# CrystalSixone/VLN-MAGIC

Hardware: AMD Instinct MI355X
Metric: trajectory-steps/sec (whole node), MAGIC-S R2R pretrain (higher is better)
Workload: dtype bf16

## Files before the change

### include/magic_hip.h

```cpp
#ifndef MAGIC_HIP_H
#define MAGIC_HIP_H
#ifdef __cplusplus
extern "C" {
#endif

#define MAGIC_OK 0
#define MAGIC_ERR_ARG (-1)
#define MAGIC_ERR_LAUNCH (-2)
#define MAGIC_ERR_UNSUPPORTED (-3)

int magic_abi_version(void);
int magic_build_id(char* out, int len);
int magic_device_info(int* cu_count, int* clock_khz, char* arch, int arch_len);

int magic_gemm(int dtype, int layout, int batch, int nh, int M, int N, int K,
               const void* A, int lda, long long sAb, long long sAh,
               const void* B, int ldb, long long sBb, long long sBh,
               void* C, int ldc, long long sCb, long long sCh, int c_f32, int accumulate,
               const float* bias, int epilogue, const void* aux, int ldaux,
               const void* residual, int ldr, void* C2, int ldc2,
               float alpha, int splitk, float* bias_grad, void* stream);
int magic_gemm_set_big(int mode);
#define MAGIC_GEMM_FORM_PLAIN 0x1
#define MAGIC_GEMM_FORM_XCD 0x2
#define MAGIC_GEMM_FORM_KG 0x4
#define MAGIC_GEMM_FORM_WIDE 0x8
#define MAGIC_GEMM_FORM_WIDE_XCD 0x10
#define MAGIC_GEMM_FORM_GROUPED 0x20
#define MAGIC_GEMM_FORM_GROUPED_KG 0x40
#define MAGIC_GEMM_FORM_DW_ATOMIC 0x80
#define MAGIC_GEMM_FORM_DW_DET 0x100
#define MAGIC_GEMM_FORM_DW_CAT 0x200
#define MAGIC_GEMM_FORM_DW_CAT_WIDE 0x400
#define MAGIC_GEMM_FORM_LLN 0x800
#define MAGIC_GEMM_FORM_LLN_PAIR 0x1000
#define MAGIC_GEMM_PLACE_SPLIT8 0x10000
#define MAGIC_GEMM_PLACE_XCD_GROUPS 0x20000
#define MAGIC_GEMM_PLACE_XCD_ROWS 0x40000
#define MAGIC_GEMM_PLACE_PLAIN 0x80000
int magic_gemm_last_form(void);

typedef struct magic_dw_desc { const void* dY; const void* X; float* dW; float* db; int M, N, K, lda, ldb, ldc, splitk; } magic_dw_desc;
int magic_gemm_dw_ws_need(int dtype, int n, const magic_dw_desc* d, long long* floats, int* counters);
int magic_gemm_dw_grouped(int dtype, int n, const magic_dw_desc* d, float* ws, long long ws_floats, unsigned* counters, int n_counters, void* stream);
typedef struct magic_dwcat_prob { float* dW; float* db; int N, K, lda, ldb, ldc; } magic_dwcat_prob;
int magic_gemm_dw_cat(int dtype, int n_prob, const magic_dwcat_prob* probs, int n_seg, const void* const* dy_tab, const void* const* x_tab,
                      const int* m_tab, void* stream);

int magic_linear_ln(int dtype, int M, int H, int K, const void* x, int lda, const void* W, int ldb, const float* bias,
                    const void* residual, int ldr, const float* gamma, const float* beta, float eps,
                    void* out, float* rstd, const void* drop_seed, float drop_p, unsigned drop_site, void* stream);
int magic_linear_act_ln(int dtype, int M, int H, int K, const void* x, int lda, const void* W, int ldb, const float* bias, int act,
                        void* pre_out, const float* gamma, const float* beta, float eps, void* out, float* rstd, void* stream);

int magic_linear_lnbwd(int dtype, int M, int H, int K, const void* x, int lda, const void* W, int ldb,
                       const void* residual, int ldr, const void* y, const float* gamma, const float* beta, const float* rstd,
                       void* dx, void* dxm, float* dgamma, float* dbeta,
                       const void* drop_seed, float drop_p, unsigned drop_site, void* stream);

int magic_dropout(int dtype, long long rows, int cols, int ld, const void* in, void* out,
                  const void* drop_seed, float drop_p, unsigned site, void* stream);

int magic_ln_fwd(int dtype, int M, int H, const void* in0, const void* in1,
                 const void* tab0, const int* idx0, int mod0, int off0,
                 const void* tab1, const int* idx1, int mod1, int off1,
                 const void* tab2, const int* idx2, int mod2, int off2,
                 const float* gamma, const float* beta, float eps, void* out, float* rstd, int do_ln,
                 const void* drop_seed, float drop_p, unsigned site_in0, unsigned site_out, void* out_drop, void* stream);
int magic_ln_bwd(int dtype, int M, int H, const void* dy, const void* y, const float* gamma, const float* beta,
                 const float* rstd, void* dx, float* dgamma, float* dbeta,
                 const int* idx0, int mod0, int off0, float* d0, int small0,
                 const int* idx1, int mod1, int off1, float* d1, int small1,
                 const int* idx2, int mod2, int off2, float* d2, int small2,
                 int do_ln, const void* drop_seed, float drop_p, unsigned site_dy, unsigned site_dx, void* dxm, int hot0, int pg_partial,
                 void* stream);
int magic_ln_bwd_tail(int dtype, int M, int H, const float* dy32, const void* y, const float* gamma, const float* beta, const float* rstd,
                      const void* act_pre, int act, void* dx, float* dgamma, float* dbeta, void* stream);
int magic_ln_bwd_blocks(int M, int H, int has_tables);
int magic_colsum_add_v(int n, const float* const* parts, float* const* dsts, const int* nblks, const int* lens, const int* strides, void* stream);

int magic_smallk_ln_fwd(int dtype, int M, int H, int Kin, const float* x, const float* W, const float* b,
                        const float* gamma, const float* beta, float eps, void* out, float* rstd, void* stream);
typedef struct {
  int n_out, accumulate; const void* src1; const int* ptr1; const int* idx1; const float* w1;
  const void* src2; const int* ptr2; const int* idx2; const float* w2; void* out;
} magic_csr_prob;
int magic_csr_gather_multi(int dtype, int H, int n, const magic_csr_prob* d, void* stream);
typedef struct {
  int M, Kin; const float* x; const void* dy; const void* y; const float* gamma; const float* beta; const float* rstd;
  float* dW; float* db; float* dgamma; float* dbeta; float* part;
} magic_skb_prob;
int magic_smallk_ln_bwd_pair(int dtype, int H, const magic_skb_prob* d, void* stream);
typedef struct {
  int M, Kin; const float* x; const float* W; const float* b; const float* gamma; const float* beta; float eps; int pad_;
  void* A; float* rstd; void* out;
  const void* add0;
  const void* src1; const int* ptr1; const int* idx1; const float* w1;
  const void* src2; const int* ptr2; const int* idx2; const float* w2;
  const void* tab; const int* tab_idx;
} magic_node_in;
int magic_node_in_fwd(int dtype, int H, int n, const magic_node_in* d, void* stream);

typedef struct { const unsigned* seed; unsigned site; float p; } magic_drop_desc;
typedef struct magic_pano_in {
  int M, Kin; float eps; int pad_;
  const void* P0; const float* g1; const float* b1; void* A1; float* rstd1;
  const float* loc; const float* W; const float* b; const float* g2; const float* b2; void* A2; float* rstd2;
  const void* nav_tab; const int* nav_idx; const void* tok_tab;
  const float* g3; const float* b3; void* X0; float* rstd3; void* X0d; magic_drop_desc dout;
} magic_pano_in;
typedef struct magic_ln_in {
  int M, do_ln; const void* in0; const void* in1;
  const void* tab[3]; const int* idx[3]; int mod[3]; int off[3];
  const float* gamma; const float* beta; float eps; int pad_; void* out; float* rstd;
  const unsigned* drop_seed; float drop_p; unsigned site_in0, site_out, pad2_; void* out_drop;
} magic_ln_in;
int magic_embed_in_fwd(int dtype, int H, const magic_pano_in* pa, const magic_ln_in* tx, void* stream);

typedef struct magic_pano_in_bwd {
  int M, Kin, pad0_, pad1_;
  const void* dy; magic_drop_desc ddy;
  const void* X0; const float* rstd3; const float* g3; const float* b3; float* dg3; float* db3;
  const int* nav_idx; float* d_nav; float* d_tok;
  const void* A1; const float* rstd1; const float* g1; const float* b1; float* dg1; float* db1; void* dP0;
  const void* A2; const float* rstd2; const float* g2; const float* b2; float* dg2; float* db2;
  const float* loc; float* dW; float* dbl;
  float* part;
} magic_pano_in_bwd;
typedef struct magic_ln_bwd_in {
  int M, do_ln; const void* dy; const void* y; const float* gamma; const float* beta; const float* rstd; void* dx; float* dgamma; float* dbeta;
  const int* idx[3]; int mod[3]; int off[3]; float* d[3]; int small[3];
  const unsigned* drop_seed; float drop_p; unsigned site_dy, site_dx; int hot0; void* dxm;
  int partial;
} magic_ln_bwd_in;
int magic_embed_in_bwd_supported(int H, int Kin);
int magic_embed_in_bwd_blocks(int M, int H, int nb_text, int partial);
int magic_embed_in_bwd_text_blocks(int M, int H, int has_tables, int has_pgrad);
int magic_embed_in_bwd(int dtype, int H, const magic_pano_in_bwd* pa, const magic_ln_bwd_in* tx,
                       int n_cs, const float* const* cs_parts, float* const* cs_dsts, const int* cs_nblks, void* stream);
int magic_smallk_ln_bwd(int dtype, int M, int H, int Kin, const float* x, const void* dy, const void* y,
                        const float* gamma, const float* beta, const float* rstd,
                        float* dW, float* db, float* dgamma, float* dbeta, float* part, void* stream);
int magic_smallk_ln_bwd_blocks(int M, int H, int Mmax);

int magic_node_in_bwd_supported(int H, int V, int Mmax);
int magic_node_in_bwd(int dtype, int H, int Np, int V, const void* x, const float* probs, const float* wf, void* d_fused, void* d_pano,
                      float* dwf, float* dbf, const magic_csr_prob* gat, int n_skb, const magic_skb_prob* skb,
                      int t_M, const void* t_dy, const int* t_idx, float* t_dtab,
                      long long add_n, int add_count, const void* const* add_xs, void* add_y, void* stream);

int magic_softmax_fwd(int dtype, int B, int nh, int Nq, int Nk, int ldp, const float* S, void* P, float scale,
                      const unsigned char* kmask, const float* dist, const float* sprel_w, const float* sprel_b, void* stream);
int magic_softmax_bwd(int dtype, int B, int nh, int Nq, int Nk, int ldp, const void* P, const float* dP, void* dS, float scale,
                      const float* dist, float* dsprel_w, float* dsprel_b, void* stream);
int magic_head_mean_fwd(int dtype, int B, int nh, long long inner, const void* P, float* out, void* stream);
int magic_head_mean_bwd(int B, int nh, long long inner, const float* g, float* dP, int accumulate, void* stream);

int magic_attn_supported(int dtype, int Nq, int Nk, int backward);
int magic_attn_fwd(int dtype, int B, int nh, int Nq, int Nk, const void* q, int ldq, const void* k, const void* v, int ldkv,
                   void* P, int ldp, void* ctx, int H, float scale, const unsigned char* kmask, const float* dist,
                   const float* sprel_w, const float* sprel_b,
                   const void* drop_seed, float drop_p, unsigned drop_site, void* Pd, void* stream);
int magic_attn_bwd(int dtype, int B, int nh, int Nq, int Nk, const void* q, int ldq, const void* k, const void* v, int ldkv,
                   const void* P, int ldp, const void* dctx, int H, float scale, const float* dP_init,
                   void* dq, int lddq, void* dk, void* dv, int lddkv,
                   const float* dist, float* dsprel_w, float* dsprel_b,
                   const void* drop_seed, float drop_p, unsigned drop_site, void* stream);
int magic_attn_bwd_ks(int dtype, int B, int nh, int Nq, int Nk, const void* q, int ldq, const void* k, const void* v, int ldkv,
                      const void* P, int ldp, const void* o, const void* dctx, int H, float scale,
                      void* dq, int lddq, void* dk, void* dv, int lddkv, int accumulate_kv,
                      const void* drop_seed, float drop_p, unsigned drop_site, void* stream);

int magic_lndot_fwd(int dtype, int M, int H, const void* Y, const float* gamma, const float* beta, float eps,
                    const float* w2, const float* b2, float* logit, void* stream);
int magic_lndot_bwd_blocks(int M);
int magic_lndot_bwd(int dtype, int M, int H, const void* Y, const float* gamma, const float* beta, float eps,
                    const float* w2, const float* dlogit, void* dZ, float* dgamma, float* dbeta, float* dw2, float* db2,
                    float* part, void* stream);

int magic_ce_rows(int dtype, int M, int N, const void* logits, int ld, const int* labels, int ignore_index,
                  float coef, const float* row_w, float* loss_row, void* dlogits, int ldd, int accumulate,
                  float* w_out, float w_rate, void* stream);
int magic_softkl_rows(int dtype, int M, int N, const void* logits, int ld, const float* targets, int ldt, float coef,
                      const float* row_w , float* loss_row, void* dlogits, int ldd,
                      void* stream);

int magic_kd_rows(int M, int N, const float* s, const float* t, int ld, float temperature, const float* w, float norm,
                  float coef, const float* coef_dev, float* loss_row, float* ds, int accumulate, void* stream);
int magic_mse(int dtype, int g_f32, long long outer, long long inner, const void* s, long long s_stride, const void* t,
              long long t_stride, const float* w, long long rows_per_w, float norm, float coef, const float* coef_dev, float* loss, void* ds,
              long long g_stride, int accumulate, void* stream);
typedef struct {
  int g_f32; long long outer, inner; const void* s; long long s_stride; const void* t; long long t_stride;
  const float* w; long long rows_per_w; float norm, coef; const float* coef_dev; float* loss; void* ds; long long g_stride; int accumulate;
  const int* valid_dev; const float* norm_dev; long long valid_mod;
} magic_mse_desc;
int magic_mse_multi(int dtype, int n, const magic_mse_desc* d, void* stream);
int magic_kd_emb_supported(int dtype, int Hs, int Ht);
int magic_kd_emb(int dtype, int n, const magic_mse_desc* d, int Hs, int Ht, const int* M, const void* const* W, const float* const* b,
                 void* const* d_acc, void* stream);
int magic_cfp_loss(int dtype, int B, int H, const void* a0, const void* a1, const void* a2, const void* txt, float temperature, float coef,
                   float* rows, void* d0, void* d1, void* d2, void* dtxt, float* part, int* counter, void* stream);

int magic_csr_gather(int dtype, int n_out, int H, const void* src, const int* ptr, const int* idx, const float* w,
                     void* out, int accumulate, void* stream);
int magic_pano_fuse_fwd(int dtype, int N, int V, int H, const void* x, const int* lens, const float* wf, const float* bf,
                        void* fused, float* probs, const void* P, int nh, int inner, float* pmean, void* stream);
typedef struct {
  int B, K, Vp, use_gate;
  const float *g_raw, *l_raw, *fuse_raw; const unsigned char *gmask, *lmask; const int* fsrc; const unsigned char* bwmask;
  float *gl, *ll, *fl;
  const int *glab, *llab; int ignore_index; float coef;
  float *rows, *dgl, *dll, *dfl;
  const float* t_fused; float w_rate; int pad_; float* w_out;
  float T, kd_norm, kd_coef, pad2_; const float* kd_coef_dev; float* kd_rows;
} magic_sap_loss_params;
int magic_sap_fuse_loss(const void* params, int nbytes, void* stream);
int magic_pano_fuse_bwd_blocks(int N);
int magic_pano_fuse_bwd(int dtype, int N, int V, int H, const void* x, const float* probs, const float* wf, const void* dfused,
                        void* dx, float* dwf, float* dbf, void* stream);
int magic_sap_fuse_fwd(int B, int K, int Vp, const float* g_raw, const float* l_raw, const float* fuse_raw,
                       const unsigned char* gmask, const unsigned char* lmask, const int* fsrc, const unsigned char* bwmask,
                       int use_gate, float* gl, float* ll, float* fl, void* stream);
int magic_sap_fuse_bwd(int B, int K, int Vp, const float* g_raw, const float* l_raw, const float* fuse_raw,
                       const unsigned char* gmask, const unsigned char* lmask, const int* fsrc, const unsigned char* bwmask,
                       int use_gate, const float* dgl, const float* dll, const float* dfl,
                       float* dg_raw, float* dl_raw, float* dfuse_raw, void* stream);

int magic_step_rng(unsigned long long base_seed, unsigned* counter, float rw_temp, int* seed_out, float* rw_out, float* zero_me,
                   float* scale_state, float growth, float backoff, int interval, void* stream);
int magic_seed_scale(const float* scale_dev);
int magic_loss_assemble(const float* rows, int n_rows, const float* row_w, float row_scale, const float* kd_rows, int n_kd,
                        float* slots, const float* rw, float alpha, int has_kd, float* out, void* stream);

int magic_rowgate_fwd(int dtype, int M, int H, int mode, const void* x, const void* e, const float* wx, const float* we,
                      const float* b0, const float* b1, float* out_s, void* out, float* gsave, void* stream);
int magic_rowgate_bwd(int dtype, int M, int H, int mode, const void* x, const void* e, const float* wx, const float* we, const float* gsave,
                      const float* dy, const void* dout, void* dx, void* de, float* dwx, float* dwe, float* db0, float* db1, void* stream);

int magic_sumsq(long long n, const float* g, float* out, void* stream);
int magic_adamw(long long n, float* p, float* g, float* m, float* v, void* shadow, int shadow_dtype,
                float lr, float b1, float b2, float eps, float wd, float step_size,
                const float* sumsq, float max_norm, float gscale, const float* lr_ss, long long n_decay, int zero_grad,
                unsigned* overflow, float* scale_state, int* sched_step, int decay_first, void* stream);
int magic_sumsq_sched(long long n, const float* g, float* out, int* step, float lr0, int warmup, int total, float b1, float b2,
                      float* lr_ss, void* stream);
int magic_sched_step(int* step, float lr0, int warmup, int total, float b1, float b2, float* lr_ss, float* zero_me, void* stream);
int magic_cast(int dtype16, int to16, long long n, const void* x, void* y, void* stream);
int magic_add_n(int dtype, long long n, int count, const void* const* xs, void* y, void* stream);
int magic_add(int dtype, long long n, const void* x, void* y, void* stream);
int magic_dact(int dtype, int kind, long long n, const void* dy, const void* z, void* dz, void* stream);

int magic_view_gather(int dtype, int Np, int V, int D, const void* table, int n_viewpoints, const int* vp_row,
                      const int* order, void* out, void* stream);

int magic_set_f32_mfma(int mode);
int magic_get_f32_mfma(void);

typedef struct {
  const void* Wqkv; const float* bqkv; const void* Wo; const float* bo; const float* g1; const float* be1;
  const void* W1; const float* bi; const void* W2; const float* bo2; const float* g2; const float* be2;
  void *qkv, *P, *Pd, *ctx, *a, *z, *g, *out; float *rstd_a, *rstd_o;
  unsigned site_attn, site_ao, site_out, pad_;
} magic_enc_layer;
typedef struct { const void* x; const unsigned char* kmask; int nsamp, N, ldp, nlayers; magic_enc_layer L[6]; } magic_enc_seg;
typedef struct { magic_enc_seg seg[2]; int nseg; float p_attn, p_hidden, eps, scale; const unsigned* seed;
                 unsigned* sync; int sync_words, pad2_; } magic_enc_params;
int magic_encoder_supported(int dtype, int H, int I, int nh, int N, int nlayers);
int magic_encoder_params_bytes(void);
int magic_encoder_fwd(int dtype, const void* params, int nbytes, void* stream);
int magic_encoder_start_gate(int timeout_us, int recent_us, unsigned* stats, void* stream);
int magic_stream_probe(unsigned* word2, int timeout_us, void* stream_wait, void* stream_set);
int magic_encoder_health(unsigned* out, void* stream);

typedef struct {
  const void* Wqkv; const float* bqkv; const void* Wo; const float* bo; const float* g1; const float* be1;
  const void* Wq; const float* bq; const void* Wkv; const float* bkv; const void* Woc; const float* boc; const float* gc; const float* bec;
  const void* W1; const float* bi; const void* W2; const float* bo2; const float* g2; const float* be2;
  void *qkv, *P, *Pd, *ctx, *a; float* rstd_a;
  void *q, *kv, *Pc, *Pdc, *cctx, *c; float* rstd_c;
  void *z, *g, *out; float* rstd_o;
  unsigned site_attn, site_ao, site_cattn, site_co, site_out, pad_;
} magic_xenc_layer;
typedef struct {
  const void* x; const void* cx; const unsigned char* qmask; const unsigned char* cmask;
  const float* dist; const float* sprel_w; const float* sprel_b;
  int nsamp, Nq, Nk, ldps, ldpc, nlayers;
  magic_xenc_layer L[3];
} magic_xenc_seg;
typedef struct { magic_xenc_seg seg[2]; int nseg; float p_attn, p_hidden, eps, scale; const unsigned* seed;
                 unsigned* sync; int sync_words, pad2_; } magic_xenc_params;
int magic_xencoder_supported(int dtype, int H, int I, int nh, int Nq, int Nk, int nlayers);
int magic_xencoder_params_bytes(void);
int magic_xencoder_fwd(int dtype, const void* params, int nbytes, void* stream);

typedef struct {
  int M, ld_in, Np, pad_;
  const void* inp; const void* res;
  const void* Wa; const float* ba; const float* g1; const float* b1; void* y1;
  const void* W1; const float* bi; const void* W2; const float* bo2; const float* g2; const float* b2; void* y2;
  const void* Wp; const float* bp; void* proj;
  float eps; int pad2_;
} magic_chain_params;
int magic_chain_supported(int dtype, int H, int I);
int magic_pack_frag_spans(const void* src, void* dst, int n, const long long* offs, const int* rows, const int* cols, void* stream);
int magic_layout_spans(const void* src, void* dst_f, void* dst_tf, int n, const long long* offs, const int* rows, const int* cols,
                       const int* flags, void* stream);
int magic_chain_fwd(int dtype, const void* params, int nbytes, void* stream);
int magic_chain_tile_rows(int rows);

typedef struct {
  int M, kt;
  const void* dqkv_n; const void* WqkvT_n; const void* dao_n; const void* dfo_in; const void* dfod_in;
  const void* y2; const float* rstd2; const float* g2; const float* b2; float* dg2; float* db2;
  const void* z; const void* W2T; const void* W1T;
  const void* y1; const float* rstd1; const float* g1; const float* b1; float* dg1; float* db1;
  const void* WoT;
  void *dfo, *dfod, *dz, *daod, *dao, *dctx;
  unsigned site_out, site_ao;
  int mode, N, ntile, ldp;
  const void* qkv_a; const void* P_a; const void* o_a; const void* dctx_a; const float* dP_init; void* dqkv_out;
  unsigned site_attn, pad_;
  const float* dist; float* dsprel_w; float* dsprel_b;
} magic_rowbwd_seg;
typedef struct { magic_rowbwd_seg seg[2]; int nseg, blocks0; float p_hidden; int pad1; const unsigned* seed; float p_attn, scale; } magic_rowbwd_params;
int magic_rowbwd_supported(int dtype, int H, int I);
int magic_rowbwd_attn_supported(int dtype, int H, int I, int nh, int N);
int magic_rowbwd_params_bytes(void);
int magic_rowbwd(int dtype, const void* params, int nbytes, void* stream);
int magic_rowbwd_rows(long long total_rows);
int magic_colsum_add(int H, int n, const float* const* parts, float* const* dsts, const int* nblks, void* stream);
int magic_transpose_spans(const void* src, void* dst, int n, const long long* offs, const int* rows, const int* cols, void* stream);

int magic_group_begin(void);
int magic_group_end(void* stream);

#ifdef __cplusplus
}
#endif
#endif
```

### vln-magic_amd/csrc/build_id.py

```python
#!/usr/bin/env python3
import hashlib
import os
import sys

HERE = os.path.dirname(os.path.abspath(__file__))
HEADERS = ("common.hpp", "group.hpp", "enc_common.hpp", os.path.join("..", "..", "include", "magic_hip.h"))
EXTRA = ("gen_fastcall.py", "build_id.py", os.path.join("..", "host", "abi.py"), os.path.join("..", "host", "lib.py"), "hostplan.c")


def _sha(*chunks):
    h = hashlib.sha256()
    for c in chunks:
        h.update(c if isinstance(c, bytes) else c.encode())
        h.update(b"\0")
    return h.hexdigest()


def _read(name):
    with open(os.path.join(HERE, name), "rb") as f:
        return f.read()


def units():
    return sorted(f for f in os.listdir(HERE) if f.endswith(".hip"))


def flags():
    for line in _read("Makefile").decode().splitlines():
        if line.startswith("FLAGS"):
            return line.strip()
    return ""


def unit_hashes():
    hdr = [_read(h) for h in HEADERS]
    fl = flags()
    return {u: _sha(_read(u), *hdr, fl) for u in units()}


def build_id(uh=None):
    uh = uh or unit_hashes()
    return _sha(*[f"{u}:{h}" for u, h in sorted(uh.items())], *[_read(e) for e in EXTRA])[:16]


def _write_if_changed(path, text):
    try:
        with open(path) as f:
            if f.read() == text:
                return False
    except OSError:
        pass
    with open(path, "w") as f:
        f.write(text)
    return True


def write_stamp(target):
    uh = unit_hashes()
    if target == "buildid.c":
        _write_if_changed(os.path.join(HERE, "buildid.c"),
                          "/* generated by build_id.py: the id of the source set this library was built from */\n"
                          "#include <string.h>\n"
                          f'int magic_build_id(char* out, int len) {{\n  static const char id[] = "{build_id(uh)}";\n'
                          "  if (!out || len < (int)sizeof(id)) return -1;\n  memcpy(out, id, sizeof(id));\n  return 0;\n}\n")
    else:
        _write_if_changed(os.path.join(HERE, target), uh[target[:-6] + ".hip"] + "\n")


if __name__ == "__main__":
    if "--stamp" in sys.argv:
        write_stamp(sys.argv[sys.argv.index("--stamp") + 1])
    else:
        print(build_id())
```

### vln-magic_amd/csrc/graphops.hip

```cpp
#include "common.hpp"
#include <cstring>

template <typename T>
__global__ __launch_bounds__(256) void csr_gather_kernel(int n_out, int H, const T* src, const int* ptr, const int* idx, const float* w,
                                                         T* out, int accumulate) {
  const int lane = threadIdx.x & 63, n = blockIdx.x * 4 + (threadIdx.x >> 6);
  if (n >= n_out) return;
  const int e0 = ptr[n], e1 = ptr[n + 1];
  if (accumulate && e0 == e1) return;
  for (int c = lane * 2; c < H; c += 128) {
    float a = 0.f, b = 0.f;
    for (int e = e0; e < e1; ++e) {
      const float wv = w ? w[e] : 1.f;
      const T* p = src + (long long)idx[e] * H + c;
      a += wv * to_f(p[0]); b += wv * to_f(p[1]);
    }
    T* o = out + (long long)n * H + c;
    if (accumulate) { a += to_f(o[0]); b += to_f(o[1]); }
    o[0] = from_f<T>(a); o[1] = from_f<T>(b);
  }
}

#define CSRM_MAX 4
struct CsrMulti { magic_csr_prob p[CSRM_MAX]; int start[CSRM_MAX + 1]; int n, H; };
template <typename T>
__global__ __launch_bounds__(256) void csr_gather_multi_kernel(CsrMulti mm) {
  int i = 0;
  while (i + 1 < mm.n && (int)blockIdx.x >= mm.start[i + 1]) ++i;
  const magic_csr_prob& p = mm.p[i];
  const int H = mm.H, lane = threadIdx.x & 63, n = (blockIdx.x - mm.start[i]) * 4 + (threadIdx.x >> 6);
  if (n >= p.n_out) return;
  const int a0 = p.ptr1[n], a1 = p.ptr1[n + 1];
  const int b0 = p.ptr2 ? p.ptr2[n] : 0, b1 = p.ptr2 ? p.ptr2[n + 1] : 0;
  if (p.accumulate && a0 == a1 && b0 == b1) return;
  const T* s1 = (const T*)p.src1; const T* s2 = (const T*)p.src2; T* out = (T*)p.out;
  for (int c = lane * 2; c < H; c += 128) {
    T* o = out + (long long)n * H + c;
    float va = 0.f, vb = 0.f;
    if (p.accumulate) { va = to_f(o[0]); vb = to_f(o[1]); }
    if (!p.accumulate || a0 < a1) {
      float a = 0.f, b = 0.f;
      for (int e = a0; e < a1; ++e) {
        const float wv = p.w1 ? p.w1[e] : 1.f;
        const T* q = s1 + (long long)p.idx1[e] * H + c;
        a += wv * to_f(q[0]); b += wv * to_f(q[1]);
      }
      va = to_f(from_f<T>(a + va)); vb = to_f(from_f<T>(b + vb));
    }
    if (b0 < b1) {
      float a = 0.f, b = 0.f;
      for (int e = b0; e < b1; ++e) {
        const float wv = p.w2 ? p.w2[e] : 1.f;
        const T* q = s2 + (long long)p.idx2[e] * H + c;
        a += wv * to_f(q[0]); b += wv * to_f(q[1]);
      }
      va = to_f(from_f<T>(a + va)); vb = to_f(from_f<T>(b + vb));
    }
    o[0] = from_f<T>(va); o[1] = from_f<T>(vb);
  }
}

template <typename T>
__global__ __launch_bounds__(256) void pano_fuse_fwd_kernel(int N, int V, int H, const T* x, const int* lens, const float* wf, const float* bf,
                                                            T* fused, float* probs, const T* P, int nh, int inner, float* pmean) {
  __shared__ float sc[64];
  const int n = blockIdx.x, tid = threadIdx.x, lane = tid & 63, wid = tid >> 6;
  if (P) {
    const T* pb = P + (long long)n * nh * inner;
    for (int r = tid; r < inner; r += 256) {
      float s = 0.f;
      for (int h = 0; h < nh; ++h) s += to_f(pb[(long long)h * inner + r]);
      pmean[(long long)n * inner + r] = s / nh;
    }
  }
  const T* xb = x + (long long)n * V * H;
  for (int v = wid; v < V; v += 4) {
    float d = 0.f;
    for (int c = lane; c < H; c += 64) d += to_f(xb[(long long)v * H + c]) * wf[c];
    d = wave_sum(d);
    if (lane == 0) sc[v] = d + bf[0] + (v < lens[n] ? 0.f : -10000.0f);
  }
  __syncthreads();
  if (wid == 0) {
    float s = lane < V ? sc[lane] : -3.0e38f;
    const float mx = wave_max(s);
    float e = lane < V ? __expf(s - mx) : 0.f;
    const float z = wave_sum(e);
    if (lane < V) { sc[lane] = e / z; probs[(long long)n * V + lane] = e / z; }
  }
  __syncthreads();
  for (int c = tid; c < H; c += 256) {
    float a = 0.f;
    for (int v = 0; v < V; ++v) a += sc[v] * to_f(xb[(long long)v * H + c]);
    fused[(long long)n * H + c] = from_f<T>(a);
  }
}


#define PFF_VPW 10
template <typename T, int NIT>
__global__ __launch_bounds__(256) void pano_fuse_fwd_reg_kernel(int N, int V, const T* x, const int* lens, const float* wf, const float* bf,
                                                                T* fused, float* probs, const T* P, int nh, int inner, float* pmean) {
  constexpr int H = NIT * 128;
  __shared__ float sc[64];
  __shared__ float part[4][H];
  const int n = blockIdx.x, tid = threadIdx.x, lane = tid & 63, wid = tid >> 6;
  const T* xb = x + (long long)n * V * H;
  float xv[PFF_VPW][2 * NIT], wr[2 * NIT];
#pragma unroll
  for (int it = 0; it < NIT; ++it) { wr[2 * it] = wf[it * 128 + lane * 2]; wr[2 * it + 1] = wf[it * 128 + lane * 2 + 1]; }
#pragma unroll
  for (int j = 0; j < PFF_VPW; ++j) {
    const int v = wid + 4 * j;
#pragma unroll
    for (int it = 0; it < NIT; ++it) {
      xv[j][2 * it] = 0.f; xv[j][2 * it + 1] = 0.f;
      if (v < V) {
        if constexpr (sizeof(T) == 2) {
          const unsigned u = *(const unsigned*)(xb + (long long)v * H + it * 128 + lane * 2);
          T lo, hi;
          __builtin_memcpy(&lo, &u, 2); __builtin_memcpy(&hi, (const char*)&u + 2, 2);
          xv[j][2 * it] = to_f(lo); xv[j][2 * it + 1] = to_f(hi);
        } else {
          const float2 u = *(const float2*)(xb + (long long)v * H + it * 128 + lane * 2);
          xv[j][2 * it] = u.x; xv[j][2 * it + 1] = u.y;
        }
      }
    }
  }
  if (P) {
    const T* pb = P + (long long)n * nh * inner;
    for (int r = tid; r < inner; r += 256) {
      float s = 0.f;
      for (int h = 0; h < nh; ++h) s += to_f(pb[(long long)h * inner + r]);
      pmean[(long long)n * inner + r] = s / nh;
    }
  }
  const int len = lens[n];
  const float b0 = bf[0];
#pragma unroll
  for (int j = 0; j < PFF_VPW; ++j) {
    const int v = wid + 4 * j;
    float d = 0.f;
#pragma unroll
    for (int i = 0; i < 2 * NIT; ++i) d += xv[j][i] * wr[i];
    d = wave_sum(d);
    if (lane == 0 && v < V) sc[v] = d + b0 + (v < len ? 0.f : -10000.0f);
  }
  __syncthreads();
  if (wid == 0) {
    float s = lane < V ? sc[lane] : -3.0e38f;
    const float mx = wave_max(s);
    float e = lane < V ? __expf(s - mx) : 0.f;
    const float z = wave_sum(e);
    if (lane < V) { sc[lane] = e / z; probs[(long long)n * V + lane] = e / z; }
  }
  __syncthreads();
  float a[2 * NIT];
#pragma unroll
  for (int i = 0; i < 2 * NIT; ++i) a[i] = 0.f;
#pragma unroll
  for (int j = 0; j < PFF_VPW; ++j) {
    const int v = wid + 4 * j;
    const float pv = v < V ? sc[v] : 0.f;
#pragma unroll
    for (int i = 0; i < 2 * NIT; ++i) a[i] += pv * xv[j][i];
  }
#pragma unroll
  for (int it = 0; it < NIT; ++it) { part[wid][it * 128 + lane * 2] = a[2 * it]; part[wid][it * 128 + lane * 2 + 1] = a[2 * it + 1]; }
  __syncthreads();
  for (int c = tid; c < H; c += 256) fused[(long long)n * H + c] = from_f<T>((part[0][c] + part[1][c]) + (part[2][c] + part[3][c]));
}

#define PF_PB 2
template <typename T>
__global__ __launch_bounds__(256 * PF_PB) void pano_fuse_bwd_kernel(int N, int V, int H, const T* __restrict__ x, const float* __restrict__ probs,
                                                                    const float* __restrict__ wf, const T* __restrict__ dfused, T* __restrict__ dx,
                                                                    float* dwf, float* dbf) {
  __shared__ float dp[PF_PB][64], dsv[PF_PB][64], red[PF_PB * 4][768], rb[PF_PB];
  const int tid = threadIdx.x, lane = tid & 63, wave = tid >> 6, pb = wave >> 2, wid = wave & 3;
  const int n = blockIdx.x * PF_PB + pb;
  const bool live = n < N;
  const int nn = live ? n : N - 1;
  const T* xb = x + (long long)nn * V * H;
  const T* df = dfused + (long long)nn * H;
  const float* p = probs + (long long)nn * V;
  const int nit = H / 128;
  float dfr[12], wfr[12];
  for (int it = 0; it < nit; ++it) {
    const int c = it * 128 + lane * 2;
    dfr[2 * it] = to_f(df[c]); dfr[2 * it + 1] = to_f(df[c + 1]);
    wfr[2 * it] = wf[c]; wfr[2 * it + 1] = wf[c + 1];
  }
  for (int v = wid; v < V; v += 4) {
    float d = 0.f;
    for (int it = 0; it < nit; ++it) {
      const int c = it * 128 + lane * 2;
      d += to_f(xb[(long long)v * H + c]) * dfr[2 * it] + to_f(xb[(long long)v * H + c + 1]) * dfr[2 * it + 1];
    }
    d = wave_sum(d);
    if (lane == 0) dp[pb][v] = d;
  }
  __syncthreads();
  if (wid == 0) {
    float t = lane < V ? p[lane] * dp[pb][lane] : 0.f;
    const float s = wave_sum(t);
    const float d = (lane < V && live) ? p[lane] * (dp[pb][lane] - s) : 0.f;
    if (lane < V) dsv[pb][lane] = d;
    const float tot = wave_sum(d);
    if (lane == 0) rb[pb] = tot;
  }
  __syncthreads();
  float aw[12];
  for (int i = 0; i < 2 * nit; ++i) aw[i] = 0.f;
  if (live) {
    for (int v = wid; v < V; v += 4) {
      const float pv = p[v], dv = dsv[pb][v];
      for (int it = 0; it < nit; ++it) {
        const int c = it * 128 + lane * 2;
        const long long i = ((long long)n * V + v) * H + c;
        const float x0 = to_f(xb[(long long)v * H + c]), x1 = to_f(xb[(long long)v * H + c + 1]);
        aw[2 * it] += dv * x0; aw[2 * it + 1] += dv * x1;
        dx[i] = from_f<T>(to_f(dx[i]) + pv * dfr[2 * it] + dv * wfr[2 * it]);
        dx[i + 1] = from_f<T>(to_f(dx[i + 1]) + pv * dfr[2 * it + 1] + dv * wfr[2 * it + 1]);
      }
    }
  }
  for (int it = 0; it < nit; ++it) {
    const int c = it * 128 + lane * 2;
    red[wave][c] = aw[2 * it]; red[wave][c + 1] = aw[2 * it + 1];
  }
  __syncthreads();
  float* const prow = dbf ? nullptr : dwf + (long long)blockIdx.x * (H + 1);
  for (int c = tid; c < H; c += 256 * PF_PB) {
    float v = 0.f;
    for (int w = 0; w < PF_PB * 4; ++w) v += red[w][c];
    if (prow) prow[c] = v; else atomicAdd(dwf + c, v);
  }
  if (tid == 0) {
    float v = 0.f;
    for (int q = 0; q < PF_PB; ++q) v += rb[q];
    if (prow) prow[H] = v; else atomicAdd(dbf, v);
  }
}

__global__ __launch_bounds__(64) void sap_fuse_fwd_kernel(int B, int K, int Vp, const float* g_raw, const float* l_raw, const float* fuse_raw,
                                                          const unsigned char* gmask, const unsigned char* lmask, const int* fsrc,
                                                          const unsigned char* bwmask, float use_gate, float* gl, float* ll, float* fl) {
  __shared__ float sl[128];
  __shared__ float sbw;
  const int b = blockIdx.x, tid = threadIdx.x;
  const float NEG = -__builtin_inff();
  const float fw = use_gate != 0.f ? 1.f / (1.f + __expf(-fuse_raw[b])) : 0.5f;
  float bw = 0.f;
  for (int j = tid; j < Vp; j += 64) {
    const float v = lmask[b * Vp + j] ? l_raw[b * Vp + j] * (1.f - fw) : NEG;
    ll[b * Vp + j] = v; sl[j] = v;
    if (bwmask[b * Vp + j] && lmask[b * Vp + j]) bw += v;
  }
  bw = wave_sum(bw);
  if (tid == 0) sbw = bw;
  __syncthreads();
  for (int k = tid; k < K; k += 64) {
    const float v = gmask[b * K + k] ? g_raw[b * K + k] * fw : NEG;
    gl[b * K + k] = v;
    const int s = fsrc[b * K + k];
    float add = 0.f;
    if (s >= 0) add = sl[s]; else if (s == -2) add = sbw;
    fl[b * K + k] = v + add;
  }
}

using SapLossParams = magic_sap_loss_params;
__device__ __forceinline__ float sap_ce_wave(const float* x, int N, int lab, int ignore_index, float coef, float* d, int lane) {
  const bool ignored = (lab == ignore_index) || lab < 0 || lab >= N;
  const float xl = ignored ? 0.f : x[lab];
  float mx = -3.0e38f;
  for (int c = lane; c < N; c += 64) mx = fmaxf(mx, x[c]);
  mx = wave_max(mx);
  float s = 0.f;
  for (int c = lane; c < N; c += 64) s += __expf(x[c] - mx);
  s = wave_sum(s);
  const float lse = mx + __logf(s);
  if (d) {
    const float cf = ignored ? 0.f : coef;
    for (int c = lane; c < N; c += 64) d[c] = cf * (__expf(x[c] - lse) - (c == lab ? 1.f : 0.f));
  }
  return ignored ? 0.f : lse - xl;
}
__global__ __launch_bounds__(64) void sap_fuse_loss_kernel(SapLossParams p, const float* ss) {
  __shared__ float sl[128];
  if (ss) { p.coef *= ss[0]; p.kd_coef *= ss[0]; }
  __shared__ float sbw;
  const int b = blockIdx.x, lane = threadIdx.x, B = p.B, K = p.K, Vp = p.Vp;
  const float NEG = -__builtin_inff();
  const float fw = p.use_gate ? 1.f / (1.f + __expf(-p.fuse_raw[b])) : 0.5f;
  float* gl = p.gl + (long long)b * K; float* ll = p.ll + (long long)b * Vp; float* fl = p.fl + (long long)b * K;
  float bw = 0.f;
  for (int j = lane; j < Vp; j += 64) {
    const float v = p.lmask[b * Vp + j] ? p.l_raw[b * Vp + j] * (1.f - fw) : NEG;
    ll[j] = v; sl[j] = v;
    if (p.bwmask[b * Vp + j] && p.lmask[b * Vp + j]) bw += v;
  }
  bw = wave_sum(bw);
  if (lane == 0) sbw = bw;
  __syncthreads();
  for (int k = lane; k < K; k += 64) {
    const float v = p.gmask[b * K + k] ? p.g_raw[b * K + k] * fw : NEG;
    gl[k] = v;
    const int s = p.fsrc[b * K + k];
    float add = 0.f;
    if (s >= 0) add = sl[s]; else if (s == -2) add = sbw;
    fl[k] = v + add;
  }
  __syncthreads();
  const int gla = p.glab[b], lla = p.llab[b];
  const float l0 = sap_ce_wave(gl, K, gla, p.ignore_index, p.coef, p.dgl ? p.dgl + (long long)b * K : nullptr, lane);
  const float l1 = sap_ce_wave(ll, Vp, lla, p.ignore_index, p.coef, p.dll ? p.dll + (long long)b * Vp : nullptr, lane);
  float* dfl = p.dfl ? p.dfl + (long long)b * K : nullptr;
  const float l2 = sap_ce_wave(fl, K, gla, p.ignore_index, p.coef, dfl, lane);
  if (lane == 0) { p.rows[b] = l0; p.rows[B + b] = l1; p.rows[2 * B + b] = l2; }
  if (!p.t_fused) return;
  const float* t = p.t_fused + (long long)b * K;
  float wr = 1.f;
  if (p.w_out) {
    wr = __expf(-p.w_rate * sap_ce_wave(t, K, gla, p.ignore_index, 0.f, nullptr, lane));
    if (lane == 0) p.w_out[b] = wr;
  }
  if (!p.kd_rows) return;
  __syncthreads();
  float coef = p.kd_coef;
  if (p.kd_coef_dev) coef *= p.kd_coef_dev[0];
  const float invT = 1.0f / p.T;
  float sv[8], tv[8], ms = -3.0e38f, mt = -3.0e38f;
#pragma unroll
  for (int it = 0; it < 8; ++it) {
    const int c = it * 64 + lane;
    float a = -3.0e38f, q = -3.0e38f;
    if (c < K) {
      a = fl[c]; q = t[c];
      if (a == NEG) a = -1e6f;
      if (q == NEG) q = -1e6f;
      a *= invT; q *= invT;
      ms = fmaxf(ms, a); mt = fmaxf(mt, q);
    }
    sv[it] = a; tv[it] = q;
  }
  ms = wave_max(ms); mt = wave_max(mt);
  float zs = 0.f, zt = 0.f;
#pragma unroll
  for (int it = 0; it < 8; ++it) {
    const int c = it * 64 + lane;
    if (c < K) { zs += __expf(sv[it] - ms); zt += __expf(tv[it] - mt); }
  }
  zs = wave_sum(zs); zt = wave_sum(zt);
  const float ls = ms + __logf(zs), lt = mt + __logf(zt);
  float kl = 0.f;
#pragma unroll
  for (int it = 0; it < 8; ++it) {
    const int c = it * 64 + lane;
    if (c < K) {
      const float lpt = tv[it] - lt, lps = sv[it] - ls;
      const float pt = __expf(lpt), ps = __expf(lps);
      if (pt > 0.f) kl += pt * (lpt - lps);
      if (dfl) dfl[c] += coef * wr * p.T * (ps - pt) * p.kd_norm;
    }
  }
  kl = wave_sum(kl);
  if (lane == 0) p.kd_rows[b] = wr * kl * p.T * p.T * p.kd_norm;
}

__global__ __launch_bounds__(64) void sap_fuse_bwd_kernel(int B, int K, int Vp, const float* g_raw, const float* l_raw, const float* fuse_raw,
                                                          const unsigned char* gmask, const unsigned char* lmask, const int* fsrc,
                                                          const unsigned char* bwmask, float use_gate, const float* dgl, const float* dll,
                                                          const float* dfl, float* dg_raw, float* dl_raw, float* dfuse_raw) {
  __shared__ float dl[128];
  __shared__ float sbw;
  const int b = blockIdx.x, tid = threadIdx.x;
  const float fw = use_gate != 0.f ? 1.f / (1.f + __expf(-fuse_raw[b])) : 0.5f;
  for (int j = tid; j < Vp; j += 64) dl[j] = (dll && lmask[b * Vp + j]) ? dll[b * Vp + j] : 0.f;
  if (tid == 0) sbw = 0.f;
  __syncthreads();
  float dfw = 0.f;
  for (int k = tid; k < K; k += 64) {
    const bool ok = gmask[b * K + k];
    const float dg = ok ? ((dgl ? dgl[b * K + k] : 0.f) + (dfl ? dfl[b * K + k] : 0.f)) : 0.f;
    dg_raw[b * K + k] = dg * fw;
    dfw += dg * g_raw[b * K + k];
    if (dfl && ok) {
      const int s = fsrc[b * K + k];
      const float d = dfl[b * K + k];
      if (s >= 0) atomicAdd(&dl[s], d); else if (s == -2) atomicAdd(&sbw, d);
    }
  }
  __syncthreads();
  for (int j = tid; j < Vp; j += 64) {
    float d = dl[j];
    if (bwmask[b * Vp + j]) d += sbw;
    if (!lmask[b * Vp + j]) d = 0.f;
    dl_raw[b * Vp + j] = d * (1.f - fw);
    dfw -= d * l_raw[b * Vp + j];
  }
  dfw = wave_sum(dfw);
  if (tid == 0) dfuse_raw[b] = use_gate != 0.f ? dfw * fw * (1.f - fw) : 0.f;
}

extern "C" int magic_csr_gather(int dtype, int n_out, int H, const void* src, const int* ptr, const int* idx, const float* w,
                                void* out, int accumulate, void* stream) {
  if (n_out <= 0 || H <= 0 || (H & 1)) return MAGIC_ERR_ARG;
  dim3 grid((n_out + 3) / 4), block(256);
  hipStream_t st = (hipStream_t)stream;
  if (dtype == DT_BF16) hipLaunchKernelGGL(csr_gather_kernel<bf16>, grid, block, 0, st, n_out, H, (const bf16*)src, ptr, idx, w, (bf16*)out, accumulate);
  else if (dtype == DT_F16) hipLaunchKernelGGL(csr_gather_kernel<f16>, grid, block, 0, st, n_out, H, (const f16*)src, ptr, idx, w, (f16*)out, accumulate);
  else hipLaunchKernelGGL(csr_gather_kernel<float>, grid, block, 0, st, n_out, H, (const float*)src, ptr, idx, w, (float*)out, accumulate);
  return launch_status();
}

extern "C" int magic_csr_gather_multi(int dtype, int H, int n, const magic_csr_prob* d, void* stream) {
  if (n < 1 || n > CSRM_MAX || !d || H <= 0 || (H & 1)) return MAGIC_ERR_ARG;
  CsrMulti mm;
  mm.n = n; mm.H = H;
  int total = 0;
  for (int i = 0; i < n; ++i) {
    if (d[i].n_out <= 0 || !d[i].src1 || !d[i].ptr1 || !d[i].idx1 || !d[i].out) return MAGIC_ERR_ARG;
    if (d[i].ptr2 && (!d[i].src2 || !d[i].idx2)) return MAGIC_ERR_ARG;
    mm.p[i] = d[i];
    mm.start[i] = total;
    total += (d[i].n_out + 3) / 4;
  }
  for (int i = n; i <= CSRM_MAX; ++i) mm.start[i] = total;
  dim3 grid(total), block(256);
  hipStream_t st = (hipStream_t)stream;
  if (dtype == DT_BF16) hipLaunchKernelGGL(csr_gather_multi_kernel<bf16>, grid, block, 0, st, mm);
  else if (dtype == DT_F16) hipLaunchKernelGGL(csr_gather_multi_kernel<f16>, grid, block, 0, st, mm);
  else hipLaunchKernelGGL(csr_gather_multi_kernel<float>, grid, block, 0, st, mm);
  return launch_status();
}

extern "C" int magic_pano_fuse_fwd(int dtype, int N, int V, int H, const void* x, const int* lens, const float* wf, const float* bf,
                                   void* fused, float* probs, const void* P, int nh, int inner, float* pmean, void* stream) {
  if (N <= 0 || V <= 0 || V > 64 || H <= 0 || (P && (nh <= 0 || inner <= 0 || !pmean))) return MAGIC_ERR_ARG;
  dim3 grid(N), block(256);
  hipStream_t st = (hipStream_t)stream;
  static int reg_form = -1;
  if (reg_form < 0) { const char* e = getenv("MAGIC_PANO_FUSE_REG"); reg_form = e ? atoi(e) : 1; }
  if (reg_form && V <= 4 * PFF_VPW && (H == 128 || H == 256 || H == 384 || H == 768)) {
#define PFR(TY, NIT) hipLaunchKernelGGL((pano_fuse_fwd_reg_kernel<TY, NIT>), grid, block, 0, st, N, V, (const TY*)x, lens, wf, bf, (TY*)fused, probs, (const TY*)P, nh, inner, pmean)
#define PFR_T(TY) do { if (H == 128) PFR(TY, 1); else if (H == 256) PFR(TY, 2); else if (H == 384) PFR(TY, 3); else PFR(TY, 6); } while (0)
    if (dtype == DT_BF16) PFR_T(bf16); else if (dtype == DT_F16) PFR_T(f16); else PFR_T(float);
#undef PFR_T
#undef PFR
    return launch_status();
  }
  if (dtype == DT_BF16) hipLaunchKernelGGL(pano_fuse_fwd_kernel<bf16>, grid, block, 0, st, N, V, H, (const bf16*)x, lens, wf, bf, (bf16*)fused, probs, (const bf16*)P, nh, inner, pmean);
  else if (dtype == DT_F16) hipLaunchKernelGGL(pano_fuse_fwd_kernel<f16>, grid, block, 0, st, N, V, H, (const f16*)x, lens, wf, bf, (f16*)fused, probs, (const f16*)P, nh, inner, pmean);
  else hipLaunchKernelGGL(pano_fuse_fwd_kernel<float>, grid, block, 0, st, N, V, H, (const float*)x, lens, wf, bf, (float*)fused, probs, (const float*)P, nh, inner, pmean);
  return launch_status();
}

extern "C" int magic_pano_fuse_bwd_blocks(int N) { return N > 0 ? (N + PF_PB - 1) / PF_PB : MAGIC_ERR_ARG; }
extern "C" int magic_pano_fuse_bwd(int dtype, int N, int V, int H, const void* x, const float* probs, const float* wf, const void* dfused,
                                   void* dx, float* dwf, float* dbf, void* stream) {
  if (N <= 0 || V <= 0 || V > 64 || H <= 0 || H % 128 || H > 768) return MAGIC_ERR_ARG;
  dim3 grid((N + PF_PB - 1) / PF_PB), block(256 * PF_PB);
  hipStream_t st = (hipStream_t)stream;
  if (dtype == DT_BF16) hipLaunchKernelGGL(pano_fuse_bwd_kernel<bf16>, grid, block, 0, st, N, V, H, (const bf16*)x, probs, wf, (const bf16*)dfused, (bf16*)dx, dwf, dbf);
  else if (dtype == DT_F16) hipLaunchKernelGGL(pano_fuse_bwd_kernel<f16>, grid, block, 0, st, N, V, H, (const f16*)x, probs, wf, (const f16*)dfused, (f16*)dx, dwf, dbf);
  else hipLaunchKernelGGL(pano_fuse_bwd_kernel<float>, grid, block, 0, st, N, V, H, (const float*)x, probs, wf, (const float*)dfused, (float*)dx, dwf, dbf);
  return launch_status();
}

extern "C" int magic_sap_fuse_fwd(int B, int K, int Vp, const float* g_raw, const float* l_raw, const float* fuse_raw,
                                  const unsigned char* gmask, const unsigned char* lmask, const int* fsrc, const unsigned char* bwmask,
                                  int use_gate, float* gl, float* ll, float* fl, void* stream) {
  if (B <= 0 || K <= 0 || Vp <= 0 || Vp > 128) return MAGIC_ERR_ARG;
  hipLaunchKernelGGL(sap_fuse_fwd_kernel, dim3(B), dim3(64), 0, (hipStream_t)stream, B, K, Vp, g_raw, l_raw, fuse_raw, gmask, lmask, fsrc, bwmask,
                     (float)use_gate, gl, ll, fl);
  return launch_status();
}

extern "C" int magic_sap_fuse_loss(const void* params, int nbytes, void* stream) {
  if (!params || nbytes != (int)sizeof(SapLossParams)) return MAGIC_ERR_ARG;
  SapLossParams p;
  memcpy(&p, params, sizeof(p));
  if (p.B <= 0 || p.K <= 0 || p.K > 512 || p.Vp <= 0 || p.Vp > 128 || !p.g_raw || !p.l_raw || !p.fuse_raw || !p.gmask || !p.lmask || !p.fsrc || !p.bwmask ||
      !p.gl || !p.ll || !p.fl || !p.glab || !p.llab || !p.rows) return MAGIC_ERR_ARG;
  if ((p.w_out || p.kd_rows) && !p.t_fused) return MAGIC_ERR_ARG;
  if (p.kd_rows && !(p.T > 0.f)) return MAGIC_ERR_ARG;
  hipLaunchKernelGGL(sap_fuse_loss_kernel, dim3(p.B), dim3(64), 0, (hipStream_t)stream, p, seed_scale_get());
  return launch_status();
}

extern "C" int magic_sap_fuse_bwd(int B, int K, int Vp, const float* g_raw, const float* l_raw, const float* fuse_raw,
                                  const unsigned char* gmask, const unsigned char* lmask, const int* fsrc, const unsigned char* bwmask,
                                  int use_gate, const float* dgl, const float* dll, const float* dfl,
                                  float* dg_raw, float* dl_raw, float* dfuse_raw, void* stream) {
  if (B <= 0 || K <= 0 || Vp <= 0 || Vp > 128) return MAGIC_ERR_ARG;
  hipLaunchKernelGGL(sap_fuse_bwd_kernel, dim3(B), dim3(64), 0, (hipStream_t)stream, B, K, Vp, g_raw, l_raw, fuse_raw, gmask, lmask, fsrc, bwmask,
                     (float)use_gate, dgl, dll, dfl, dg_raw, dl_raw, dfuse_raw);
  return launch_status();
}

template <typename T>
__global__ __launch_bounds__(256) void view_gather_kernel(long long rows, int V, int D, const T* table, int n_vp, const int* vp_row, const int* order, T* out) {
  constexpr int VE = 16 / sizeof(T), UN = 4;
  typedef __attribute__((ext_vector_type(4))) unsigned int u4;
  const int nvec = D / VE;
  const long long total = rows * nvec, stride = (long long)gridDim.x * 256;
  u4* dst = (u4*)out;
  for (long long v0 = (long long)blockIdx.x * 256 + threadIdx.x; v0 < total; v0 += stride * UN) {
    u4 val[UN];
#pragma unroll
    for (int u = 0; u < UN; ++u) {
      const long long v = v0 + u * stride;
      val[u] = (u4){0u, 0u, 0u, 0u};
      if (v < total) {
        const long long r = v / nvec;
        const int c = (int)(v - r * nvec), sv = order[r];
        const int vr = vp_row[r / V];
        if (sv >= 0 && sv < 36 && (unsigned)vr < (unsigned)n_vp)
          val[u] = __builtin_nontemporal_load((const u4*)(table + ((long long)vr * 36 + sv) * D) + c);
      }
    }
#pragma unroll
    for (int u = 0; u < UN; ++u) {
      const long long v = v0 + u * stride;
      if (v < total) dst[v] = val[u];
    }
  }
}

extern "C" int magic_view_gather(int dtype, int Np, int V, int D, const void* table, int n_viewpoints, const int* vp_row,
                                 const int* order, void* out, void* stream) {
  if (Np <= 0 || V <= 0 || D <= 0 || n_viewpoints <= 0 || !table || !vp_row || !order || !out) return MAGIC_ERR_ARG;
  if (!dtype_ok(dtype)) return MAGIC_ERR_ARG;
  const int ve = dtype_is16(dtype) ? 8 : 4;
  if (D % ve || ((uintptr_t)table & 15) || ((uintptr_t)out & 15)) return MAGIC_ERR_ARG;
  const long long rows = (long long)Np * V;
  const long long chunks = (rows * (D / ve) + 256 * 4 - 1) / (256 * 4);
  dim3 grid((unsigned)(chunks < 1 ? 1 : chunks)), block(256);
  hipStream_t st = (hipStream_t)stream;
  if (dtype == DT_BF16) hipLaunchKernelGGL(view_gather_kernel<bf16>, grid, block, 0, st, rows, V, D, (const bf16*)table, n_viewpoints, vp_row, order, (bf16*)out);
  else if (dtype == DT_F16) hipLaunchKernelGGL(view_gather_kernel<f16>, grid, block, 0, st, rows, V, D, (const f16*)table, n_viewpoints, vp_row, order, (f16*)out);
  else hipLaunchKernelGGL(view_gather_kernel<float>, grid, block, 0, st, rows, V, D, (const float*)table, n_viewpoints, vp_row, order, (float*)out);
  return launch_status();
}
```

### vln-magic_amd/host/model_pretrain.py

```python
import os

import torch
import torch.nn as nn

from . import ops as O
from .config import cfg_get
from .ddp import refuse_torch_ddp
from .engine import Ctx, MagicNet, cls_specs, rup, trunk_specs
from .params import ParamStore
from .plan import build_plan, check_plan

MID_CUT = 2
LOCKSTEP = not os.environ.get("MAGIC_NO_LOCKSTEP")
LOCKSTEP_EAGER = bool(os.environ.get("MAGIC_LOCKSTEP_EAGER"))
DYN_TERMS = ("txt_emb", "txt_attn", "img_emb", "img_fused", "img_attn", "g_emb", "g_attn", "l_emb", "l_attn")
KD_SLOTS = ("txt_emb_loss", "txt_attn_loss", "img_emb_loss", "avg_img_emb_loss", "img_attn_loss",
            "global_emb_loss", "global_attn_loss", "local_emb_loss", "local_attn_loss", "predict_loss")


PRETRAIN_CAUSAL = ("back_txt", "back_img")


def pretrain_specs(cfg):
    H = cfg.hidden_size
    s = trunk_specs(cfg, "bert.")
    s += [("mlm_head.predictions.transform.dense.weight", (H, H), "normal"), ("mlm_head.predictions.transform.dense.bias", (H,), "zeros"),
          ("mlm_head.predictions.transform.LayerNorm.weight", (H,), "ones"), ("mlm_head.predictions.transform.LayerNorm.bias", (H,), "zeros"),
          ("mlm_head.predictions.bias", (cfg.vocab_size,), "zeros")]
    s += cls_specs("global_sap_head.", H) + cls_specs("local_sap_head.", H) + cls_specs("sap_fuse_linear.", H, 2 * H)
    for k in ("gmap", "vp", "fused", "txt"):
        s += [(f"cfp_heads.{k}.weight", (H, H), "normal"), (f"cfp_heads.{k}.bias", (H,), "zeros")]
    if "mrc" in (getattr(cfg, "pretrain_tasks", None) or ()):
        P = int(cfg_get(cfg, "image_prob_size"))
        s += [("image_classifier.net.0.weight", (H, H), "normal"), ("image_classifier.net.0.bias", (H,), "zeros"),
              ("image_classifier.net.2.weight", (H,), "ones"), ("image_classifier.net.2.bias", (H,), "zeros"),
              ("image_classifier.net.3.weight", (P, H), "normal"), ("image_classifier.net.3.bias", (P,), "zeros")]
    from .causal import causal_specs
    return s + causal_specs(cfg, "bert.", only=PRETRAIN_CAUSAL)


def _dropout_knobs(model, config):
    model.dropout = nn.Dropout(float(cfg_get(config, "hidden_dropout_prob")))
    model.attention_dropout = nn.Dropout(float(cfg_get(config, "attention_probs_dropout_prob")))


class _BackwardHook(torch.autograd.Function):

    @staticmethod
    def forward(ctx, loss_value, anchor, model):
        ctx.model = model
        return loss_value.clone()

    @staticmethod
    def backward(ctx, grad_out):
        ctx.model.backward()
        m = ctx.model
        if m.loss_scale is not None:
            m.store.grad.mul_(grad_out.to(torch.float32) * m.loss_scale[1])
        elif m.grad_scale != 1.0:
            m.store.grad.mul_(grad_out.to(torch.float32) / m.grad_scale)
        from .trainer import auto_sync
        auto_sync(ctx.model)
        return None, None, None


MLM_TAIL_FUSED = os.environ.get("MAGIC_MLM_TAIL_FUSED", "1") != "0"
MLM_DX_SPLITK = int(os.environ.get("MAGIC_MLM_DX_SPLITK", "32"))
MLM_DX_ATOMICS = os.environ.get("MAGIC_MLM_DX_ATOMICS", "0") != "0"


class GlocalTextPathCMTPreTraining(nn.Module):
    def __init__(self, config, device="cuda", compute_dtype=torch.bfloat16, seed=0):
        super().__init__()
        self.config = config
        self.device_ = torch.device(device)
        self.compute_dtype = compute_dtype
        trainable = getattr(config, "role", "student") != "teacher" or bool(getattr(config, "train_teacher", False))
        self.store = ParamStore(pretrain_specs(config), device, compute_dtype,
                                init_std=cfg_get(config, "initializer_range"), seed=seed, requires_grad=trainable)
        self.store.attach_to(self)
        self.net = MagicNet(config, self.store, "bert.")
        self.prefix, self.explicit_backward = "bert.", True
        if self.device_.type == "cuda":
            O.dw_counters(self.device_)
        from .causal import build_blocks
        self.causal_blocks = build_blocks(self, only=PRETRAIN_CAUSAL)
        _dropout_knobs(self, config)
        self._anchor = torch.zeros(1, device=self.device_, requires_grad=True)
        self._ctx = None
        self._kd_idx = torch.tensor([0, 0, 1, 1, 1, 2, 2, 3, 3, 4], device=self.device_)
        self.keep_mlm_logits = False
        self.dropout_seed = None
        self.grad_scale = 4096.0 if compute_dtype == torch.float16 else 1.0
        self.loss_scale = None
        self.register_load_state_dict_post_hook(lambda m, k: setattr(m.store, "shadow_clean", False))

    def enable_dynamic_loss_scale(self, init=None):
        if self.loss_scale is None:
            S = float(init if init is not None else self.grad_scale)
            self.loss_scale = torch.tensor([S, 1.0 / S, 0.0, 0.0], dtype=torch.float32, device=self.device_)
        return self.loss_scale

    @classmethod
    def from_pretrained(cls, pretrained_model_name_or_path=None, config=None, state_dict=None, **kw):
        model = cls(config, **kw)
        if state_dict is not None:
            own = model.state_dict()
            keep = {k: v for k, v in state_dict.items() if k in own and tuple(v.shape) == tuple(own[k].shape)}
            model.load_state_dict(keep, strict=False)
        return model

    def _par(self, fn_main, fn_aux):
        if LOCKSTEP and self.device_.type == "cuda" and (torch.cuda.is_current_stream_capturing() or LOCKSTEP_EAGER):
            from . import lib as L
            return L.lockstep(fn_main, fn_aux)
        return fn_main(), fn_aux()

    def _arm_dropout(self):
        ph, pa = float(self.dropout.p), float(self.attention_dropout.p)
        if self.training and self.store.requires_grad and torch.is_grad_enabled() and (ph > 0 or pa > 0):
            seed = getattr(self, "dropout_seed", None)
            if seed is None:
                seed = torch.randint(0, 2 ** 31 - 1, (2,), dtype=torch.int32, device=self.device_)
            self.net.set_dropout(seed, ph, pa)
        else:
            self.net.set_dropout(None)

    def mark_params_dirty(self):
        self.store.shadow_clean = False

    def _dev(self, t, dtype=None):
        t = t.to(self.device_, non_blocking=True)
        return t if dtype is None or t.dtype == dtype else t.to(dtype)

    def _inputs(self, batch, plan):
        Np, V = plan["Np"], plan["V"]
        if batch.get("view_table") is not None:
            x = batch["view_table"].gather(batch["traj_vp_row"], batch["traj_view_order"]).reshape(Np * V, -1)
        else:
            x = self._dev(batch["traj_view_img_fts"]).reshape(Np * V, -1)
        if x.dtype != self.compute_dtype:
            x = O.cast_to(x.contiguous(), self.compute_dtype)
        return Ctx(feats=x,
                   loc=self._dev(batch["traj_loc_fts"], torch.float32).reshape(Np * V, -1).contiguous(),
                   gpos=self._dev(batch["gmap_pos_fts"], torch.float32).reshape(plan["B"] * plan["K"], -1).contiguous(),
                   vpos=self._dev(batch["vp_pos_fts"], torch.float32).reshape(plan["B"] * plan["Vp"], -1).contiguous(),
                   dist=self._dev(batch["gmap_pair_dists"], torch.float32).contiguous())

    def _cls(self, prefix, X, M, lda=None):
        n, H = self.net, self.net.H
        l1 = n.lin(prefix + "net.0.weight")
        Y = O.linear_fwd(X, l1.W, l1.b, M, epilogue=2, lda=lda)
        ln = n.ln(prefix + "net.2")
        l2 = n.lin(prefix + "net.3.weight")
        logit = n.new(M, dtype=torch.float32)
        O.lndot_fwd(Y, M, H, ln.g, ln.b, n.eps, l2.Wm, l2.b, logit)
        return Y, logit

    def _cls_tail(self, prefix, Y, M):
        n = self.net
        ln, l2 = n.ln(prefix + "net.2"), n.lin(prefix + "net.3.weight")
        logit = n.new(M, dtype=torch.float32)
        O.lndot_fwd(Y, M, n.H, ln.g, ln.b, n.eps, l2.Wm, l2.b, logit)
        return logit

    def _cls_bwd(self, prefix, X, Y, dlogit, M, d_acc, lda=None):
        n, H = self.net, self.net.H
        l1, ln, l2 = n.lin(prefix + "net.0.weight"), n.ln(prefix + "net.2"), n.lin(prefix + "net.3.weight")
        dZ = n.new(M, H)
        O.lndot_bwd(Y, M, H, ln.g, ln.b, n.eps, l2.Wm, dlogit, dZ, ln.dg, ln.db, l2.dW, l2.db)
        O.linear_dw(dZ, X, l1.dW, l1.db, M, ldb=lda)
        O.linear_dx(dZ, l1.W, M, out=d_acc, residual=d_acc, ldc=lda)

    def _causal_fwd(self, c, batch, compute_loss):
        cz, plan, H = self.causal_blocks, c.plan, self.net.H
        need = {"instr_z_direction_features": "back_txt", "instr_z_landmark_features": "back_txt", "img_z_features": "back_img"}
        for k, blk in need.items():
            if batch.get(k) is not None and blk not in cz:
                from .causal import BLOCKS
                raise ValueError(f"batch carries {k!r} but config.{BLOCKS[blk]} is off -- the model has no '{blk}' block "
                                 "(pretrain_src/config/r2r_magic_model_config.json:60-66)")
        track = bool(compute_loss and self.store.requires_grad and torch.is_grad_enabled())
        c.islands = []

        def island(block, x2d, shape, z, pz):
            x0 = x2d.detach().view(shape)
            with torch.enable_grad() if track else torch.no_grad():
                if track:
                    x0.requires_grad_(True)
                y = block(x0, z, pz)
            if track:
                c.islands.append((x0, y))
            return y.detach().reshape(x2d.shape).contiguous()
        dv = lambda t: t.to(self.device_)
        if "back_txt" in cz and (batch.get("instr_z_direction_features") is not None or batch.get("instr_z_landmark_features") is not None):
            parts = [k for k in ("direction", "landmark") if batch.get(f"instr_z_{k}_features") is not None]
            z = torch.cat([dv(batch[f"instr_z_{k}_features"]) for k in parts], 1)
            pz = torch.cat([dv(batch[f"instr_z_{k}_pzs"]) for k in parts], 1)
            c.txt_out = island(cz["back_txt"], c.txt.out, (plan["B"], plan["L"], H), z, pz)
            c.island_txt = len(c.islands) - 1 if track else None
        if "back_img" in cz and batch.get("img_z_features") is not None:
            out = island(cz["back_img"], c.pano.out, (plan["Np"], plan["V"], H), dv(batch["img_z_features"]), dv(batch["img_z_pzs"]))
            c.pano_adj = Ctx(**vars(c.pano))
            c.pano_adj.out = out
            c.island_pano = len(c.islands) - 1 if track else None

    def _causal_bwd(self, c):
        for name, attr in (("island_txt", "d_txt"), ("island_pano", "d_pano")):
            i = getattr(c, name, None)
            if i is None:
                continue
            x0, y = c.islands[i]
            d = getattr(c, attr)
            torch.autograd.backward(y, d.view(y.shape).to(y.dtype))
            setattr(c, attr, x0.grad.reshape(d.shape).to(d.dtype).clone())
            x0.grad = None

    def will_fuse_encoders(self, plan):
        n = self.net
        return bool(n.enc_ok(plan["L"], self.config.num_l_layers) and n.enc_ok(plan["V"], self.config.num_pano_layers))

    def forward(self, batch, task, compute_loss=True, teacher_outputs=None, rw=None, plan=None, return_outputs=False, inputs=None, heads=True):
        if not heads and (compute_loss or not return_outputs):
            raise ValueError("heads=False returns the encoders' outputs only: compute_loss=False, return_outputs=True")
        n = self.net
        refuse_torch_ddp(self)
        self.store.sync_shadow()
        O.DEFER["queue"].clear(); O.DEFER["bytes"] = 0
        O.RBW_JOBS.clear()
        if self.store.requires_grad:
            O.defer_dw(False)
        self._arm_dropout()
        plan = plan if plan is not None else build_plan(batch, task, self.device_)
        check_plan(plan, self.config)
        inp = inputs if inputs is not None else self._inputs(batch, plan)
        B, L, K, Vp, H = plan["B"], plan["L"], plan["K"], plan["Vp"], n.H
        c = Ctx(task=task, plan=plan, inp=inp)
        fuse = self.will_fuse_encoders(plan)
        if n.embed_in_ok():
            ct, cp = n.embeds_fwd(plan, inp.feats, inp.loc)
            c.txt, c.pano = self._par(lambda: n.text_fwd(plan, defer=fuse, c=ct), lambda: n.pano_fwd(plan, inp.feats, inp.loc, defer=fuse, c=cp))
        else:
            c.txt, c.pano = self._par(lambda: n.text_fwd(plan, defer=fuse), lambda: n.pano_fwd(plan, inp.feats, inp.loc, defer=fuse))
        if fuse:
            n.encoders_fwd(c.txt, c.pano)
        c.txt_out, c.pano_adj = c.txt.out, c.pano
        if self.causal_blocks or any(batch.get(k) is not None for k in ("instr_z_direction_features", "instr_z_landmark_features", "img_z_features")):
            self._causal_fwd(c, batch, compute_loss)
        c.gin, c.vin = n.nodes_in_fwd(plan, c.pano_adj, inp.gpos if task != "mrc" else None, inp.vpos if task != "mlm" else None)
        tl, gl_, vl = plan["lens"]["txt"], plan["lens"]["gmap"], [Vp] * B
        o = dict(txt_embeds=c.txt_out, txt_attns=c.txt.P, pano_embeds=c.pano_adj.out, pano_fused_embeds=c.pano.fused,
                 img_attns=c.pano.img_attn, plan=plan, inputs=inp)
        if task == "mlm":
            l2v_args = ("global", plan, c.txt_out, L, plan["txt_mask"], tl, plan["txt_tokens"], c.gin.out, K, plan["gmap_mask"], gl_, plan["gmap_nodes"])
            c.l2v = n.cross_fwd_fused([l2v_args])[0] if n.xenc_ok(L, K) else n.cross_fwd(*l2v_args, dist=None)
            o["gmap_embeds"], o["gmap_attns"] = c.l2v.out, c.l2v.P
            if heads:
                nm = plan["n_mask"]
                c.hm_in = n.new(nm, H)
                O.csr_gather(c.l2v.out, *plan["mlm_rows"], c.hm_in, nm, H)
                t = n.lin("mlm_head.predictions.transform.dense.weight")
                c.tz = n.new(nm, H)
                tn = n.ln("mlm_head.predictions.transform.LayerNorm")
                c.hm, c.rstd_hm = n.new(nm, H), n.new(nm, dtype=torch.float32)
                if MLM_TAIL_FUSED and O.linear_ln_ok(H, H):
                    O.linear_act_ln(c.hm_in, t.W, t.b, nm, 1, c.tz, tn.g, tn.b, n.eps, c.hm, c.rstd_hm)
                else:
                    c.tg = O.linear_fwd(c.hm_in, t.W, t.b, nm, epilogue=1, pre=c.tz)
                    O.ln_fwd(nm, H, c.hm, in0=c.tg, gamma=tn.g, beta=tn.b, eps=n.eps, rstd=c.rstd_hm)
                Vv = self.config.vocab_size
                c.ldv = rup(Vv, 8)
                c.logits = n.new(nm, c.ldv)
                if c.ldv > Vv:
                    c.logits[:, Vv:].zero_()
                O.linear_fwd(c.hm, self.store.w("bert.embeddings.word_embeddings.weight"), self.store.master("mlm_head.predictions.bias"),
                             nm, out=c.logits, ldc=c.ldv)
                o["predict"] = c.logits[:, :Vv]
        elif task == "mrc":
            loc_args = ("local", plan, c.vin.out, Vp, plan["vp_mask"], vl, B * Vp, c.txt_out, L, plan["txt_mask"], tl, plan["txt_tokens"])
            c.loc = n.cross_fwd_fused([loc_args])[0] if n.xenc_ok(Vp, L) else n.cross_fwd(*loc_args)
            o.update(vp_embeds=c.loc.out, vp_attns=c.loc.P)
            if heads:
                nm = plan["n_mrc"]
                c.mx = n.new(nm, H)
                O.csr_gather(c.loc.out, *plan["mrc_rows"], c.mx, nm, H)
                l1, l2 = n.lin("image_classifier.net.0.weight"), n.lin("image_classifier.net.3.weight")
                ln = n.ln("image_classifier.net.2")
                c.mZ, c.m_rstd = n.new(nm, H), n.new(nm, dtype=torch.float32)
                if MLM_TAIL_FUSED and O.linear_ln_ok(H, H):
                    c.mY = n.new(nm, H)
                    O.linear_act_ln(c.mx, l1.W, l1.b, nm, 2, c.mY, ln.g, ln.b, n.eps, c.mZ, c.m_rstd)
                else:
                    c.mY = O.linear_fwd(c.mx, l1.W, l1.b, nm, epilogue=2)
                    O.ln_fwd(nm, H, c.mZ, in0=c.mY, gamma=ln.g, beta=ln.b, eps=n.eps, rstd=c.m_rstd)
                c.mlogits = O.linear_fwd(c.mZ, l2.W, l2.b, nm)
                o["predict"] = c.mlogits
        else:
            def _local():
                vin = c.vin
                return vin, n.cross_fwd("local", plan, vin.out, Vp, plan["vp_mask"], vl, B * Vp,
                                        c.txt_out, L, plan["txt_mask"], tl, plan["txt_tokens"])
            if n.xenc_ok(K, L) and n.xenc_ok(Vp, L):
                c.glob, c.loc = n.cross_fwd_fused([
                    ("global", plan, c.gin.out, K, plan["gmap_mask"], gl_, plan["gmap_nodes"], c.txt_out, L, plan["txt_mask"], tl, plan["txt_tokens"], inp.dist),
                    ("local", plan, c.vin.out, Vp, plan["vp_mask"], vl, B * Vp, c.txt_out, L, plan["txt_mask"], tl, plan["txt_tokens"])])
            else:
              c.glob, (c.vin, c.loc) = self._par(
                lambda: n.cross_fwd("global", plan, c.gin.out, K, plan["gmap_mask"], gl_, plan["gmap_nodes"],
                                    c.txt_out, L, plan["txt_mask"], tl, plan["txt_tokens"], dist=inp.dist), _local)
            o.update(gmap_embeds=c.glob.out, gmap_attns=c.glob.P, vp_embeds=c.loc.out, vp_attns=c.loc.P)
            if not heads:
                pass
            elif task == "sap":
                from . import lib as _lib
                use_gate = bool(cfg_get(self.config, "glocal_fuse"))
                g1, l1_ = n.lin("global_sap_head.net.0.weight"), n.lin("local_sap_head.net.0.weight")
                with _lib.group():
                    c.Yg = O.linear_fwd(c.glob.out, g1.W, g1.b, B * K, epilogue=2)
                    c.Yl = O.linear_fwd(c.loc.out, l1_.W, l1_.b, B * Vp, epilogue=2)
                    if use_gate:
                        f1 = n.lin("sap_fuse_linear.net.0.weight")
                        tmp = O.linear_fwd(c.glob.out, f1.W, None, B, lda=K * H, ldb=2 * H, K=H)
                c.g_raw = self._cls_tail("global_sap_head.", c.Yg, B * K)
                c.l_raw = self._cls_tail("local_sap_head.", c.Yl, B * Vp)
                if use_gate:
                    c.Yf = O.linear_fwd(c.loc.out, f1.W[:, H:], f1.b, B, lda=Vp * H, ldb=2 * H, K=H, residual=tmp, epilogue=0)
                    self._relu(c.Yf)
                    fln, f2 = n.ln("sap_fuse_linear.net.2"), n.lin("sap_fuse_linear.net.3.weight")
                    c.fuse_raw = n.new(B, dtype=torch.float32)
                    O.lndot_fwd(c.Yf, B, H, fln.g, fln.b, n.eps, f2.Wm, f2.b, c.fuse_raw)
                else:
                    c.fuse_raw = n.zeros(B, dtype=torch.float32)
                c.use_gate = use_gate
                c.gl, c.ll, c.fl = n.new(B, K, dtype=torch.float32), n.new(B, Vp, dtype=torch.float32), n.new(B, K, dtype=torch.float32)
                c.sap_fused = bool(compute_loss and O.SAP_LOSS_FUSED and K <= 512 and Vp <= 128)
                if not c.sap_fused:
                    O.sap_fuse_fwd(B, K, Vp, c.g_raw, c.l_raw, c.fuse_raw, plan["gmask"], plan["lmask"], plan["fsrc"], plan["bwmask"],
                                   use_gate, c.gl, c.ll, c.fl)
                o.update(global_logits=c.gl, local_logits=c.ll, fused_logits=c.fl)
            elif task == "cfp":
                c.g0, c.v0, c.t0, c.gv0 = n.new(B, H), n.new(B, H), n.new(B, H), n.new(B, H)
                O.csr_gather_multi(H, [dict(out=c.g0, n_out=B, src1=c.glob.out, csr1=plan["g0"]),
                                       dict(out=c.v0, n_out=B, src1=c.loc.out, csr1=plan["v0"]),
                                       dict(out=c.t0, n_out=B, src1=c.txt_out, csr1=plan["t0"]),
                                       dict(out=c.gv0, n_out=B, src1=c.glob.out, csr1=plan["g0"], src2=c.loc.out, csr2=plan["v0"])])
                from . import lib as _lib
                with _lib.group():
                    c.cfp = []
                    for key, src in (("gmap", c.g0), ("vp", c.v0), ("fused", c.gv0), ("txt", c.t0)):
                        hl = n.lin(f"cfp_heads.{key}.weight")
                        c.cfp.append(O.linear_fwd(src, hl.W, hl.b, B))
                o["cfp"] = tuple(c.cfp)
            else:
                raise ValueError(task)
        if not compute_loss:
            if return_outputs:
                return o
            if task == "mlm":
                return {"predict": o["predict"]}
            if task == "mrc":
                return c.mlogits, plan["mrc_targets"], None, None
            if task == "sap":
                return dict(global_logits=c.gl, local_logits=c.ll, fused_logits=c.fl,
                            global_act_labels=self._dev(batch["global_act_labels"]), local_act_labels=self._dev(batch["local_act_labels"]))
            return o["cfp"]
        self._ctx = c
        if callable(teacher_outputs):
            teacher_outputs = teacher_outputs()
        scaled = self.loss_scale is not None and self.store.requires_grad
        if scaled:
            O.seed_scale(self.loss_scale)
        try:
            out = self._losses(c, o, teacher_outputs, rw)
        finally:
            if scaled:
                O.seed_scale(None)
        out["outputs"] = o
        if self.store.requires_grad and torch.is_grad_enabled():
            out["loss"] = _BackwardHook.apply(out["loss"], self._anchor, self)
        return out

    def _relu(self, x):
        return O.dact(x, x, 2, out=x)

    def _dyn(self, c, term, fn, mod=0):
        d = c.plan.get("dyn")
        if d is None:
            return {}
        i = DYN_TERMS.index(term)
        d["fill"][term] = fn
        return dict(valid_dev=d["i"][2 * i:2 * i + 2], norm_dev=d["f"][i:i + 1], norm=1.0, valid_mod=mod)

    def _kd_emb(self, c, slot, s_t, t_t, proj, M, outer, w, coef, d_acc, dyn=None):
        c.kd_emb.append((slot, s_t, t_t, self.net.lin(f"bert.{proj}.weight"), M, outer, w, coef, d_acc, dyn))

    def _kd_attn(self, c, slot, sP, tP, Bn, Nq, Nk, ldp, nh_s, nh_t, w, coef, dyn=None):
        n = self.net
        hmin = min(nh_s, nh_t)
        dP = None
        if self.store.requires_grad:
            dP = (n.new if hmin == nh_s else n.zeros)(Bn, nh_s, Nq, ldp, dtype=torch.float32)
        q = dict(s=sP, t=tP, outer=Bn, inner=hmin * Nq * ldp, s_stride=nh_s * Nq * ldp, t_stride=nh_t * Nq * ldp, w=w, rows_per_w=1,
                 norm=1.0 / (Bn * hmin * Nq * Nk), coef=coef[0], coef_dev=coef[1], loss=c.slots[slot:slot + 1], ds=dP,
                 g_stride=nh_s * Nq * ldp)
        if dyn is not None:
            term, qk, kk = dyn
            q.update(self._dyn(c, term, lambda t, Bn=Bn, hmin=hmin, Nq=Nq, Nk=Nk, ldp=ldp, qk=qk, kk=kk:
                               (Bn, (t[qk] if qk else Nq) * ldp, 1.0 / (Bn * hmin * (t[qk] if qk else Nq) * (t[kk] if kk else Nk))), mod=Nq * ldp))
        c.kd_mse.append(q)
        return dP

    def _kd_flush(self, c):
        from . import lib as L
        n, train = self.net, self.store.requires_grad
        jobs = c.kd_emb
        fused = bool(jobs) and all(
            O.kd_emb_ok(s_t.dtype, pl.K, pl.N) and t_t.dtype == s_t.dtype and s_t.is_contiguous() and t_t.is_contiguous() and pl.W.is_contiguous()
            and not ((s_t.data_ptr() | t_t.data_ptr() | pl.W.data_ptr() | (d_acc.data_ptr() if train else 0)) & 15)
            and (not train or d_acc.is_contiguous()) for (_, s_t, t_t, pl, _, _, _, _, d_acc, _) in jobs)
        sps = [None] * len(jobs)
        if not fused:
            with L.group():
                sps = [O.linear_fwd(s_t, pl.W, pl.b, M) for (_, s_t, _, pl, M, _, _, _, _, _) in jobs]
        dss, emb = [], []
        for (slot, s_t, t_t, pl, M, outer, w, coef, d_acc, dyn), sp in zip(jobs, sps):
            Ht = pl.N
            inner = (M // outer) * Ht
            ds = n.new(M, Ht) if train else None
            dss.append(ds)
            q = dict(s=sp, t=t_t, outer=outer, inner=inner, s_stride=inner, t_stride=inner, w=w, rows_per_w=1, norm=1.0 / (M * Ht),
                     coef=coef[0], coef_dev=coef[1], loss=c.slots[slot:slot + 1], ds=ds, g_stride=inner)
            if dyn is not None:
                term, ok, ik = dyn
                rows = M // outer
                q.update(self._dyn(c, term, lambda t, outer=outer, rows=rows, Ht=Ht, ok=ok, ik=ik:
                                   ((t[ok] if ok else outer), (t[ik] if ik else rows) * Ht,
                                    1.0 / ((t[ok] if ok else outer) * (t[ik] if ik else rows) * Ht))))
            if fused:
                q.pop("valid_mod", None)
                q.update(s=s_t, M=M, W=pl.W, b=pl.b, d_acc=d_acc if train else None)
                emb.append(q)
            else:
                c.kd_mse.append(q)
        if emb:
            O.kd_emb(emb)
        if c.kd_mse:
            O.mse_multi(c.kd_mse)
        if train:
            for (slot, s_t, t_t, pl, M, outer, w, coef, d_acc, dyn), ds in zip(jobs, dss):
                O.linear_dw(ds, s_t, pl.dW, pl.db, M)
            if not fused:
                with L.group():
                    for (slot, s_t, t_t, pl, M, outer, w, coef, d_acc, dyn), ds in zip(jobs, dss):
                        O.linear_dx(ds, pl.W, M, out=d_acc, residual=d_acc)
        c.kd_emb, c.kd_mse = [], []

    def _rw_device(self, rw):
        if rw is None:
            rw = [1.0] * 5
        if torch.is_tensor(rw) and rw.is_cuda:
            return rw
        cached = getattr(self, "_rwd_cache", None)
        key = tuple(float(x) for x in rw)
        if cached is None or cached[0] != key:
            self._rwd_cache = cached = (key, torch.tensor(list(key), dtype=torch.float32).to(self.device_))
        return cached[1]

    def _losses(self, c, o, t, rw):
        n, cfg, plan, task = self.net, self.config, c.plan, c.task
        B, L, K, Vp, H = plan["B"], plan["L"], plan["K"], plan["Vp"], n.H
        train = self.store.requires_grad
        O.defer_dw(train)
        kdl = getattr(cfg, "kdl", None)
        kd = t is not None and kdl is not None
        alpha = float(kdl["kd_alpha"]) if kd else 0.0
        sc = 1.0 - alpha
        dyn = train and self.loss_scale is not None
        gs = float(self.grad_scale) if (train and not dyn) else 1.0
        scg = sc * gs
        nm_ = plan["n_mask"] if task == "mlm" else 0
        c.dx_slabs = MLM_DX_SPLITK if (nm_ and MLM_TAIL_FUSED and not MLM_DX_ATOMICS and MLM_DX_SPLITK > 1) else 0
        if c.dx_slabs:
            f32 = n.zeros(16, dtype=torch.float32)
            c.slots, c.d_hm32 = f32, n.new(c.dx_slabs * nm_, H, dtype=torch.float32)
        else:
            f32 = n.zeros(16 + nm_ * H, dtype=torch.float32)
            c.slots, c.d_hm32 = f32[:16], (f32[16:].view(nm_, H) if nm_ else None)
        if train:
            rows = [B * L, plan["Np"] * plan["V"], plan["Np"]]
            rows += {"sap": [B * K, B * Vp, B * L], "cfp": [B * K, B * Vp, B * L, B, B, B], "mlm": [B * L, B * K], "mrc": [B * Vp]}[task]
            arena = n.zeros(sum(rows) * H)
            offs = [0]
            for r in rows:
                offs.append(offs[-1] + r * H)
            pool = [arena[offs[i]:offs[i + 1]].view(rows[i], H) for i in range(len(rows))]

            def zz(*shape):
                t = pool.pop(0)
                assert tuple(t.shape) == tuple(shape), (tuple(t.shape), shape)
                return t
        else:
            zz = lambda *s: None
        c.d_txt, c.d_pano, c.d_fused = zz(B * L, H), zz(plan["Np"] * plan["V"], H), zz(plan["Np"], H)
        c.dP_txt = c.dP_pano = c.dP_g = c.dP_l = None
        c.kd_emb, c.kd_mse = [], []
        res = {}
        if task == "sap":
            c.d_gmap, c.d_vp, c.d_txt2 = zz(B * K, H), zz(B * Vp, H), zz(B * L, H)
            c.rows = n.new(3, B, dtype=torch.float32)
            c.dgl, c.dll, c.dfl = (n.new(B, K, dtype=torch.float32), n.new(B, Vp, dtype=torch.float32), n.new(B, K, dtype=torch.float32)) \
                if train else (None, None, None)
            ga, la = plan["global_act_labels"], plan["local_act_labels"]
            c.sap_w = c.kdrows = None
            if getattr(c, "sap_fused", False):
                hard = bool(kd and kdl.get("teacher_sample_hard_mining", False))
                pred = bool(kd and "predict" in kdl["kdl_tasks"])
                if hard:
                    c.sap_w = n.new(B, dtype=torch.float32)
                if pred:
                    c.kdrows = n.new(B, dtype=torch.float32)
                if kd:
                    rwd = self._rw_device(rw)
                O.sap_fuse_loss(B, K, Vp, c.g_raw, c.l_raw, c.fuse_raw, plan["gmask"], plan["lmask"], plan["fsrc"], plan["bwmask"], c.use_gate,
                                c.gl, c.ll, c.fl, ga, la, scg / B, c.rows, dgl=c.dgl, dll=c.dll, dfl=c.dfl,
                                t_fused=t["fused_logits"] if (hard or pred) else None,
                                w_rate=float(kdl["t_sample_preprocess_exp_decay"]) if hard else 0.0, w_out=c.sap_w,
                                T=float(kdl["kd_temperature"]) if kd else 1.0, kd_norm=(1.0 / B if hard else 1.0 / (B * K)),
                                kd_coef=alpha * gs, kd_coef_dev=rwd[4:5] if pred else None, kd_rows=c.kdrows)
            else:
                O.ce_rows(c.gl, B, K, K, ga, coef=scg / B, loss_row=c.rows[0], dlogits=c.dgl, ldd=K)
                O.ce_rows(c.ll, B, Vp, Vp, la, coef=scg / B, loss_row=c.rows[1], dlogits=c.dll, ldd=Vp)
                O.ce_rows(c.fl, B, K, K, ga, coef=scg / B, loss_row=c.rows[2], dlogits=c.dfl, ldd=K)
            sup_rows, sup_w, sup_scale = c.rows, None, 1.0 / B
        elif task == "mlm":
            c.d_x, c.d_gin0 = zz(B * L, H), zz(B * K, H)
            nm = plan["n_mask"]
            c.rows = n.new(nm, dtype=torch.float32)
            c.dlogits = (n.new(nm, c.ldv) if self.keep_mlm_logits else c.logits) if train else None
            roww = plan.get("mlm_row_w")
            O.ce_rows(c.logits, nm, cfg.vocab_size, c.ldv, plan["mlm_labels"], ignore_index=-1, coef=scg if roww is not None else scg / nm,
                      row_w=roww, loss_row=c.rows, dlogits=c.dlogits, ldd=c.ldv)
            if train and not self.keep_mlm_logits:
                o["predict"] = None
            sup_rows, sup_w, sup_scale = c.rows, roww, (1.0 if roww is not None else 1.0 / nm)
        elif task == "mrc":
            c.d_vp = zz(B * Vp, H)
            nm, Pn = plan["n_mrc"], c.mlogits.shape[1]
            c.rows = n.new(nm, dtype=torch.float32)
            c.dmlogits = n.new(nm, Pn) if train else None
            roww = plan.get("mrc_row_w")
            O.softkl_rows(c.mlogits, nm, Pn, Pn, plan["mrc_targets"], coef=scg if roww is not None else scg / nm, row_w=roww,
                          loss_row=c.rows, dlogits=c.dmlogits, ldd=Pn)
            sup_rows, sup_w, sup_scale = c.rows, roww, (1.0 if roww is not None else 1.0 / nm)
        else:
            c.d_gmap, c.d_vp, c.d_txt2 = zz(B * K, H), zz(B * Vp, H), zz(B * L, H)
            c.d_cls0 = (zz(B, H), zz(B, H), zz(B, H))
            temp = float(cfg_get(cfg, "cfp_temperature"))
            c.rows = n.new(6, B, dtype=torch.float32)
            txt_o = c.cfp[3]
            c.dsim, c.d_cfp = [], None
            ar = plan["arange_b"]
            lds = c.lds = rup(B, 8)
            fused = O.cfp_loss_ok(B, H)
            if fused:
                c.d_cfp = [n.new(B, H) for _ in range(4)] if train else None
                O.cfp_loss(B, H, c.cfp[:3], txt_o, temp, scg * 0.5 / B, c.rows, d_a=c.d_cfp[:3] if train else None, d_txt=c.d_cfp[3] if train else None)
            for i in (() if fused else range(3)):
                a = c.cfp[i]
                sim, simT = n.new(B, lds, dtype=torch.float32), n.new(B, lds, dtype=torch.float32)
                O.gemm(0, a, txt_o, sim, B, B, H, H, H, lds, alpha=1.0 / temp)
                O.gemm(0, txt_o, a, simT, B, B, H, H, H, lds, alpha=1.0 / temp)
                d1 = n.new(B, lds, dtype=torch.float32) if train else None
                d2 = n.new(B, lds, dtype=torch.float32) if train else None
                O.ce_rows(sim, B, B, lds, ar, coef=scg * 0.5 / B, loss_row=c.rows[2 * i], dlogits=d1, ldd=lds)
                O.ce_rows(simT, B, B, lds, ar, coef=scg * 0.5 / B, loss_row=c.rows[2 * i + 1], dlogits=d2, ldd=lds)
                c.dsim.append((d1, d2))
            c.temp = temp
            sup_rows, sup_w, sup_scale = c.rows, None, 0.5 / B
        kd_rows, rwd = None, None
        if kd:
            if rw is None:
                rw = [1.0] * 5
            rwd = self._rw_device(rw)
            rw = [(alpha * gs, rwd[i:i + 1]) for i in range(5)]
            tasks, types = kdl["kdl_tasks"], kdl["kdl_task_types"]
            emb, att = "emb" in types, "attn" in types
            T = float(kdl["kd_temperature"])
            w = None
            if kdl.get("teacher_sample_hard_mining", False) and task == "sap":
                if getattr(c, "sap_w", None) is not None:
                    w = c.sap_w
                else:
                    w = n.new(B, dtype=torch.float32)
                    O.ce_rows(t["fused_logits"], B, K, K, plan["global_act_labels"], w_out=w,
                              w_rate=float(kdl["t_sample_preprocess_exp_decay"]))
            nh_s = n.nh
            nh_t = t["txt_attns"].shape[1]
            Np, V = plan["Np"], plan["V"]
            if "txt" in tasks:
                if emb:
                    self._kd_emb(c, 0, o["txt_embeds"], t["txt_embeds"], "txt_emb_w", B * L, B, w, rw[0], c.d_txt, dyn=("txt_emb", None, "L"))
                if att:
                    c.dP_txt = self._kd_attn(c, 1, o["txt_attns"], t["txt_attns"], B, L, L, c.txt.ldp, nh_s, nh_t, w, rw[0], dyn=("txt_attn", "L", "L"))
            wp = w if (w is not None and Np == B) else None
            if "img" in tasks:
                if emb:
                    self._kd_emb(c, 2, o["pano_embeds"], t["pano_embeds"], "kdl_img_w", Np * V, Np, wp, rw[1], c.d_pano, dyn=("img_emb", "Np", None))
                    self._kd_emb(c, 3, o["pano_fused_embeds"], t["pano_fused_embeds"], "kdl_avg_img_w", Np, Np, wp, rw[1], c.d_fused, dyn=("img_fused", "Np", None))
                if att:
                    ldp = c.pano.ldp
                    g_img = n.new(Np, V, ldp, dtype=torch.float32) if train else None
                    q = dict(s=o["img_attns"], t=t["img_attns"], outer=Np, inner=V * ldp, s_stride=V * ldp, t_stride=V * ldp, w=wp, rows_per_w=1,
                             norm=1.0 / (Np * V * V), coef=rw[1][0], coef_dev=rw[1][1], loss=c.slots[4:5], ds=g_img, g_stride=V * ldp)
                    q.update(self._dyn(c, "img_attn", lambda tr, V=V, ldp=ldp: (tr["Np"], V * ldp, 1.0 / (tr["Np"] * V * V))))
                    c.kd_mse.append(q)
            if "global" in tasks and task != "mrc":
                if task == "mlm":
                    x, Pm, Nq, Nk, ldp, d_acc, qk, kk = c.l2v.out, c.l2v.P, L, K, c.l2v.ldp, c.d_x, "L", "K"
                else:
                    x, Pm, Nq, Nk, ldp, d_acc, qk, kk = c.glob.out, c.glob.P, K, L, c.glob.ldp, c.d_gmap, "K", "L"
                if emb:
                    self._kd_emb(c, 5, x, t["gmap_embeds"], "global_cross_w", B * Nq, B, w, rw[2], d_acc, dyn=("g_emb", None, qk))
                if att:
                    c.dP_g = self._kd_attn(c, 6, Pm, t["gmap_attns"], B, Nq, Nk, ldp, nh_s, nh_t, w, rw[2], dyn=("g_attn", qk, kk))
            if "local" in tasks and task != "mlm":
                if emb:
                    self._kd_emb(c, 7, c.loc.out, t["vp_embeds"], "local_cross_w", B * Vp, B, w, rw[3], c.d_vp, dyn=("l_emb", None, None))
                if att:
                    c.dP_l = self._kd_attn(c, 8, c.loc.P, t["vp_attns"], B, Vp, L, c.loc.ldp, nh_s, nh_t, w, rw[3], dyn=("l_attn", None, "L"))
            self._kd_flush(c)
            if "img" in tasks and att and train:
                c.dP_pano = n.new(Np, nh_s, V, c.pano.ldp, dtype=torch.float32)
                O.head_mean_bwd(g_img, c.dP_pano, Np, nh_s, V * c.pano.ldp)
            if "predict" in tasks and task == "sap":
                if getattr(c, "sap_fused", False):
                    kd_rows = c.kdrows
                else:
                    c.kdrows = n.new(B, dtype=torch.float32)
                    O.kd_rows(c.fl, t["fused_logits"], B, K, K, T, w=w, norm=(1.0 / B if w is not None else 1.0 / (B * K)),
                              coef=rw[4][0], coef_dev=rw[4][1], loss_row=c.kdrows, ds=c.dfl, accumulate=True)
                    kd_rows = c.kdrows
        lo = O.loss_assemble(sup_rows.reshape(-1), sup_w, sup_scale, kd_rows, c.slots, rwd, alpha, kd, n.new(16, dtype=torch.float32))
        res["supervised_loss"] = lo[0]
        if kd:
            res["kdl_terms"] = {k: lo[1 + i] for i, k in enumerate(KD_SLOTS)}
            res["kdl_loss"] = lo[11]
        res["loss"] = lo[12]
        return res

    def backward(self, on_bucket=None):
        self.backward_phase1()
        c = self._ctx
        if on_bucket is not None:
            O.flush_dw(keep_active=True)
            on_bucket(0, c)

            def cut():
                O.flush_dw(keep_active=True)
                on_bucket(1, c)
            self.backward_phase2(on_cut=cut)
            on_bucket(2, c)
        else:
            self.backward_phase2()

    @torch.no_grad()
    def backward_phase1(self):
        c = self._ctx
        assert c is not None, "backward() without a compute_loss=True forward"
        self.store.ensure_grads()
        O.defer_dw(True)
        n, plan, task = self.net, c.plan, c.task
        B, L, K, Vp, H = plan["B"], plan["L"], plan["K"], plan["Vp"], n.H
        if task == "sap":
            dg, dl, df = n.new(B, K, dtype=torch.float32), n.new(B, Vp, dtype=torch.float32), n.new(B, dtype=torch.float32)
            O.sap_fuse_bwd(B, K, Vp, c.g_raw, c.l_raw, c.fuse_raw, plan["gmask"], plan["lmask"], plan["fsrc"], plan["bwmask"],
                           c.use_gate, c.dgl, c.dll, c.dfl, dg, dl, df)
            from . import lib as _lib
            heads = []
            for prefix, X, Y, dlogit, M, d_acc in (("global_sap_head.", c.glob.out, c.Yg, dg, B * K, c.d_gmap),
                                                   ("local_sap_head.", c.loc.out, c.Yl, dl, B * Vp, c.d_vp)):
                l1, ln, l2 = n.lin(prefix + "net.0.weight"), n.ln(prefix + "net.2"), n.lin(prefix + "net.3.weight")
                dZh = n.new(M, H)
                O.lndot_bwd(Y, M, H, ln.g, ln.b, n.eps, l2.Wm, dlogit, dZh, ln.dg, ln.db, l2.dW, l2.db)
                O.linear_dw(dZh, X, l1.dW, l1.db, M)
                heads.append((dZh, l1, M, d_acc))
            with _lib.group():
                for dZh, l1, M, d_acc in heads:
                    O.linear_dx(dZh, l1.W, M, out=d_acc, residual=d_acc)
            if c.use_gate:
                f1, fln, f2 = n.lin("sap_fuse_linear.net.0.weight"), n.ln("sap_fuse_linear.net.2"), n.lin("sap_fuse_linear.net.3.weight")
                dZ = n.new(B, H)
                O.lndot_bwd(c.Yf, B, H, fln.g, fln.b, n.eps, f2.Wm, df, dZ, fln.dg, fln.db, f2.dW, f2.db)
                O.linear_dw(dZ, c.glob.out, f1.dW, f1.db, B, N=H, K=H, ldb=K * H, ldc=2 * H)
                O.linear_dw(dZ, c.loc.out, f1.dW[:, H:], None, B, N=H, K=H, ldb=Vp * H, ldc=2 * H)
                with _lib.group():
                    O.linear_dx(dZ, f1.W, B, out=c.d_gmap, residual=c.d_gmap, ldb=2 * H, ldc=K * H, N=H, K=H)
                    O.linear_dx(dZ, f1.W[:, H:], B, out=c.d_vp, residual=c.d_vp, ldb=2 * H, ldc=Vp * H, N=H, K=H)
        elif task == "cfp":
            d_outs = c.d_cfp if c.d_cfp is not None else [n.new(B, H) for _ in range(4)]
            txt_o = c.cfp[3]
            for i in (() if c.d_cfp is not None else range(3)):
                d1, d2 = c.dsim[i]
                a = c.cfp[i]
                it = 1.0 / c.temp
                lds = c.lds
                e1, e2 = self._as(d1), self._as(d2)
                O.gemm(1, e1, txt_o, d_outs[i], B, H, B, lds, H, H, alpha=it)
                O.gemm(2, e2, txt_o, d_outs[i], B, H, B, lds, H, H, alpha=it, residual=d_outs[i], ldr=H)
                if i == 0:
                    O.gemm(2, e1, a, d_outs[3], B, H, B, lds, H, H, alpha=it)
                else:
                    O.gemm(2, e1, a, d_outs[3], B, H, B, lds, H, H, alpha=it, residual=d_outs[3], ldr=H)
                O.gemm(1, e2, a, d_outs[3], B, H, B, lds, H, H, alpha=it, residual=d_outs[3], ldr=H)
            d_g0, d_v0, d_t0 = c.d_cls0
            heads = list(zip((("gmap", c.g0, (d_g0,)), ("vp", c.v0, (d_v0,)), ("fused", c.gv0, (d_g0, d_v0)), ("txt", c.t0, (d_t0,))), d_outs))
            for (key, src, dsts), d_o in heads:
                hl = n.lin(f"cfp_heads.{key}.weight")
                O.linear_dw(d_o, src, hl.dW, hl.db, B)
            from . import lib as _lib
            for sel in (("gmap", "vp", "txt"), ("fused",)):
                with _lib.group():
                    for (key, src, dsts), d_o in heads:
                        if key in sel:
                            hl = n.lin(f"cfp_heads.{key}.weight")
                            for dst in dsts:
                                O.linear_dx(d_o, hl.W, B, out=dst, residual=dst)
            O.csr_gather_multi(H, [dict(out=c.d_gmap, n_out=B * K, accumulate=True, src1=d_g0, csr1=plan["g0_T"]),
                                   dict(out=c.d_vp, n_out=B * Vp, accumulate=True, src1=d_v0, csr1=plan["v0_T"]),
                                   dict(out=c.d_txt, n_out=B * L, accumulate=True, src1=d_t0, csr1=plan["t0_T"])])
        if task == "mlm":
            nm, Vv = plan["n_mask"], self.config.vocab_size
            dlog = c.dlogits
            Wemb = self.store.w("bert.embeddings.word_embeddings.weight")
            O.linear_dw(dlog, c.hm, self.store.g("bert.embeddings.word_embeddings.weight"), self.store.g("mlm_head.predictions.bias"),
                        nm, N=Vv, K=H, lda=c.ldv)
            d_hm32 = c.d_hm32
            if c.dx_slabs:
                O.gemm(1, dlog, Wemb, d_hm32, nm, H, Vv, c.ldv, H, H, splitk=-c.dx_slabs)
            else:
                O.gemm(1, dlog, Wemb, d_hm32, nm, H, Vv, c.ldv, H, H, splitk=MLM_DX_SPLITK, accumulate=True)
            tn = n.ln("mlm_head.predictions.transform.LayerNorm")
            if MLM_TAIL_FUSED:
                d_tz = O.ln_bwd_tail(nm, H, d_hm32, c.hm, tn.g, tn.b, c.rstd_hm, c.tz, 1, n.new(nm, H), tn.dg, tn.db, nslab=max(1, c.dx_slabs))
            else:
                d_hm = O.cast_to(d_hm32, self.compute_dtype)
                d_tg = n.new(nm, H)
                O.ln_bwd(nm, H, d_hm, y=c.hm, gamma=tn.g, beta=tn.b, rstd=c.rstd_hm, dx=d_tg, dgamma=tn.dg, dbeta=tn.db)
                d_tz = O.dact(d_tg, c.tz, 1)
            t = n.lin("mlm_head.predictions.transform.dense.weight")
            O.linear_dw(d_tz, c.hm_in, t.dW, t.db, nm)
            d_hin = O.linear_dx(d_tz, t.W, nm)
            O.csr_gather(d_hin, *plan["mlm_rows_T"], c.d_x, B * L, H, accumulate=True)
            d_gin = c.d_gin0
            d_t2 = n.cross_bwd(c.l2v, c.d_x, d_gin, c.dP_g)
            if not getattr(c, "islands", None) and n.nodes_pano_ok(plan, gin=c.gin):
                n.nodes_pano_bwd(plan, c.pano, c.gin, d_gin, None, None, c.d_pano, c.d_fused, add=(c.d_txt, [d_t2]))
                c.pano_head_done = True
            else:
                O.add_(c.d_txt, d_t2)
        elif task == "mrc":
            nm = plan["n_mrc"]
            l1, ln, l2 = n.lin("image_classifier.net.0.weight"), n.ln("image_classifier.net.2"), n.lin("image_classifier.net.3.weight")
            O.linear_dw(c.dmlogits, c.mZ, l2.dW, l2.db, nm)
            dZ = O.linear_dx(c.dmlogits, l2.W, nm)
            dY = n.new(nm, H)
            O.ln_bwd(nm, H, dZ, y=c.mZ, gamma=ln.g, beta=ln.b, rstd=c.m_rstd, dx=dY, dgamma=ln.dg, dbeta=ln.db)
            dpre = O.dact(dY, c.mY, 2)
            O.linear_dw(dpre, c.mx, l1.dW, l1.db, nm)
            dmx = O.linear_dx(dpre, l1.W, nm)
            O.csr_gather(dmx, *plan["mrc_rows_T"], c.d_vp, B * Vp, H, accumulate=True)
            d_vin = n.cross_bwd(c.loc, c.d_vp, c.d_txt, c.dP_l)
            n.vp_in_bwd(c.vin, plan, d_vin, c.d_pano)
        else:
            d_txt2 = c.d_txt2
            one = not getattr(c, "islands", None) and n.nodes_pano_ok(plan, gin=c.gin, vin=c.vin)
            fold = None
            if n.rbw_ok():
                (d_gin, d_vin), fold = n.cross_stacks_bwd([(c.glob, c.d_gmap, c.d_txt, c.dP_g), (c.loc, c.d_vp, c.d_txt, c.dP_l)], defer_fold=one)
            else:
                d_gin, d_vin = self._par(lambda: n.cross_bwd(c.glob, c.d_gmap, c.d_txt, c.dP_g),
                                         lambda: n.cross_bwd(c.loc, c.d_vp, d_txt2, c.dP_l))
                if one:
                    fold = (c.d_txt, [d_txt2])
                else:
                    O.add_(c.d_txt, d_txt2)
            if one:
                n.nodes_pano_bwd(plan, c.pano, c.gin, d_gin, c.vin, d_vin, c.d_pano, c.d_fused, add=fold)
                c.pano_head_done = True
            else:
                n.nodes_in_bwd(plan, c.gin, d_gin, c.vin, d_vin, c.d_pano, c.d_fused)
        if task == "mlm" and not getattr(c, "pano_head_done", False):
            n.gmap_in_bwd(c.gin, plan, d_gin, c.d_pano, c.d_fused)

    @torch.no_grad()
    def backward_phase2(self, on_cut=None):
        c = self._ctx
        n, plan = self.net, c.plan
        fired = []
        if getattr(c, "islands", None):
            self._causal_bwd(c)

        done = getattr(c, "pano_head_done", False)

        def on_iter(k):
            if on_cut is not None and k == MID_CUT and not fired:
                fired.append(k)
                on_cut()
        if n.rbw_ok() and n.enc_ok(plan["L"], self.config.num_l_layers) and n.enc_ok(plan["V"], self.config.num_pano_layers):
            n.encoders_bwd(c.txt, c.pano, plan, c.d_txt, c.dP_txt, c.d_pano, c.d_fused, c.dP_pano, on_iter=on_iter, pano_head_done=done)
            if on_cut is not None and not fired:
                on_cut()
        elif on_cut is not None:
            self._par(lambda: n.text_bwd(c.txt, plan, c.d_txt, c.dP_txt),
                      lambda: n.pano_bwd(c.pano, plan, c.d_pano, c.d_fused, c.dP_pano, pano_head_done=done))
            on_cut()
        else:
            self._par(lambda: n.text_bwd(c.txt, plan, c.d_txt, c.dP_txt),
                      lambda: n.pano_bwd(c.pano, plan, c.d_pano, c.d_fused, c.dP_pano, pano_head_done=done))
        O.flush_dw()
        self._ctx = None

    def _as(self, d):
        return d if d.dtype == self.compute_dtype else O.cast_to(d, self.compute_dtype)
```

### vln-magic_amd/host/ops.py

```python
import ctypes as C
import os

import torch

from . import lanes
from . import lib as L

FLOPS = {"total": 0.0, "gemm": 0.0, "linear_ln": 0.0, "attn": 0.0, "enc": 0.0, "enabled": False}
BYTES = {"dw": 0.0, "dw_launches": 0}


def _count(m, n, k, batch=1, fam="gemm"):
    if FLOPS["enabled"]:
        f = 2.0 * m * n * k * batch
        FLOPS["total"] += f
        FLOPS[fam] += f


def _chk(cond, msg):
    if not cond:
        raise L.MagicHipError("shape check failed: " + msg)


def gemm(layout, A, B, C, M, N, K, lda, ldb, ldc, *, batch=1, nh=1, sA=(0, 0), sB=(0, 0), sC=(0, 0),
# ... 884 lines not shown

def head_mean_fwd(Pm, out, B, nh, inner):
    L.call("magic_head_mean_fwd", L.dt(Pm.dtype), B, nh, inner, L.P(Pm), L.P(out), L.stream())


def head_mean_bwd(g, dP, B, nh, inner, accumulate=False):
    L.call("magic_head_mean_bwd", B, nh, inner, L.P(g), L.P(dP), 1 if accumulate else 0, L.stream())


def lndot_fwd(Y, M, H, gamma, beta, eps, w2, b2, logit):
    L.call("magic_lndot_fwd", L.dt(Y.dtype), M, H, L.P(Y), L.P(gamma), L.P(beta), float(eps), L.P(w2), L.P(b2), L.P(logit), L.stream())


def lndot_bwd(Y, M, H, gamma, beta, eps, w2, dlogit, dZ, dgamma, dbeta, dw2, db2):
    part = None
    if part_ok(H):
        nblk = int(L.load().magic_lndot_bwd_blocks(int(M)))
        stride = 3 * H + 1
        part = _part_rows(nblk, stride, Y.device)
        flat = part.view(-1)
        for off, length, dst in ((0, H, dgamma), (H, H, dbeta), (2 * H, H, dw2), (3 * H, 1, db2)):
            PART_JOBS.append((flat[off:], dst.reshape(-1), nblk, length, stride))
    L.call("magic_lndot_bwd", L.dt(Y.dtype), M, H, L.P(Y), L.P(gamma), L.P(beta), float(eps), L.P(w2), L.P(dlogit), L.P(dZ),
           L.P(dgamma), L.P(dbeta), L.P(dw2), L.P(db2), L.P(part), L.stream())


def ce_rows(logits, M, N, ld, labels, *, ignore_index=-100, coef=0.0, row_w=None, loss_row=None, dlogits=None, ldd=0,
            accumulate=False, w_out=None, w_rate=0.0):
    _chk(labels.dtype == torch.int32, "labels int32")
    L.call("magic_ce_rows", L.dt(logits.dtype), M, N, L.P(logits), ld, L.P(labels), ignore_index, float(coef), L.P(row_w),
           L.P(loss_row), L.P(dlogits), ldd, 1 if accumulate else 0, L.P(w_out), float(w_rate), L.stream())


def softkl_rows(logits, M, N, ld, targets, *, coef=0.0, row_w=None, loss_row=None, dlogits=None, ldd=0):
    _chk(targets.dtype == torch.float32 and targets.stride(-1) == 1, "softkl targets fp32")
    _chk(row_w is None or (row_w.dtype == torch.float32 and row_w.numel() >= M), "softkl row_w fp32 [M]")
    L.call("magic_softkl_rows", L.dt(logits.dtype), M, N, L.P(logits), ld, L.P(targets), targets.stride(0), float(coef),
           L.P(row_w), L.P(loss_row), L.P(dlogits), ldd, L.stream())


def kd_rows(s, t, M, N, ld, temperature, *, w=None, norm=1.0, coef=0.0, coef_dev=None, loss_row=None, ds=None, accumulate=False):
    _chk(s.dtype == torch.float32 and t.dtype == torch.float32, "kd logits fp32")
    L.call("magic_kd_rows", M, N, L.P(s), L.P(t), ld, float(temperature), L.P(w), float(norm), float(coef), L.P(coef_dev), L.P(loss_row),
           L.P(ds), 1 if accumulate else 0, L.stream())


def mse(s, t, outer, inner, s_stride, t_stride, *, w=None, rows_per_w=1, norm=1.0, coef=0.0, coef_dev=None, loss=None, ds=None, g_stride=0,
        accumulate=False):
    _chk(s.dtype == t.dtype, "mse dtypes")
    g_f32 = 1 if (ds is not None and ds.dtype == torch.float32) else 0
    if s.dtype == torch.float32:
        g_f32 = 1
    L.call("magic_mse", L.dt(s.dtype), g_f32, outer, inner, L.P(s), s_stride, L.P(t), t_stride, L.P(w), rows_per_w, float(norm),
           float(coef), L.P(coef_dev), L.P(loss), L.P(ds), g_stride, 1 if accumulate else 0, L.stream())


def mse_multi(problems):
    half = [q["s"].dtype for q in problems if q["s"].dtype != torch.float32]
    dt0 = half[0] if half else torch.float32
    i = 0
    while i < len(problems):
        chunk = problems[i:i + 10]
        arr = (L.MseDesc * len(chunk))()
        for j, q in enumerate(chunk):
            s_, t_, ds = q["s"], q["t"], q.get("ds")
            in32 = s_.dtype == torch.float32
            _chk(s_.dtype == t_.dtype and (in32 or s_.dtype == dt0), "mse_multi dtypes")
            _chk(not in32 or ds is None or ds.dtype == torch.float32, "mse_multi: fp32 inputs take an fp32 gradient")
            g_f32 = (3 if dt0 != torch.float32 else 1) if in32 else (1 if (ds is not None and ds.dtype == torch.float32) else 0)
            arr[j] = L.MseDesc(g_f32, q["outer"], q["inner"], L.P(s_), q["s_stride"], L.P(t_), q["t_stride"], L.P(q.get("w")),
                               q.get("rows_per_w", 1), float(q.get("norm", 1.0)), float(q.get("coef", 0.0)), L.P(q.get("coef_dev")),
                               L.P(q.get("loss")), L.P(ds), q.get("g_stride", 0), 1 if q.get("accumulate") else 0,
                               L.P(q.get("valid_dev")), L.P(q.get("norm_dev")), int(q.get("valid_mod", 0)))
        L.call("magic_mse_multi", L.dt(dt0), len(chunk), arr, L.stream())
        i += len(chunk)


KD_FUSED = not os.environ.get("MAGIC_NO_KD_FUSED")
_KDE_OK = {}


def kd_emb_ok(dtype, Hs, Ht):
    if not KD_FUSED or dtype not in L.HALF:
        return False
    key = (L.dt(dtype), int(Hs), int(Ht))
    if key not in _KDE_OK:
        _KDE_OK[key] = bool(L.load().magic_kd_emb_supported(*key))
    return _KDE_OK[key]


def kd_emb(problems):
    i = 0
    while i < len(problems):
        chunk = problems[i:i + 8]
        n = len(chunk)
        W0 = chunk[0]["W"]
        Ht, Hs = W0.shape
        arr = (L.MseDesc * n)()
        Ms, Ws, bs, das = (C.c_int * n)(), (C.c_void_p * n)(), (C.c_void_p * n)(), (C.c_void_p * n)()
        for j, q in enumerate(chunk):
            s_, t_, W, ds, da, M = q["s"], q["t"], q["W"], q.get("ds"), q.get("d_acc"), int(q["M"])
            _chk(s_.dtype == t_.dtype == W.dtype == W0.dtype and tuple(W.shape) == (Ht, Hs) and W.stride(0) == Hs and W.stride(1) == 1, "kd_emb weights")
            _chk(q["b"].dtype == torch.float32 and q["b"].numel() >= Ht, "kd_emb bias")
            _chk(s_.is_contiguous() and t_.is_contiguous() and s_.numel() >= M * Hs and t_.numel() >= M * Ht, "kd_emb rows")
            _chk((ds is None) == (da is None), "kd_emb: ds and d_acc go together")
            _chk(ds is None or (ds.dtype == da.dtype == W.dtype and ds.is_contiguous() and da.is_contiguous() and ds.numel() >= M * Ht and da.numel() >= M * Hs),
                 "kd_emb gradients")
            inner = int(q["inner"])
            _chk(inner % Ht == 0 and int(q["outer"]) * (inner // Ht) == M, "kd_emb extents")
            arr[j] = L.MseDesc(0, q["outer"], inner, L.P(s_), (inner // Ht) * Hs, L.P(t_), inner, L.P(q.get("w")), q.get("rows_per_w", 1),
                               float(q.get("norm", 1.0)), float(q.get("coef", 0.0)), L.P(q.get("coef_dev")), L.P(q.get("loss")), L.P(ds), inner, 0,
                               L.P(q.get("valid_dev")), L.P(q.get("norm_dev")), 0)
            Ms[j], Ws[j], bs[j], das[j] = M, L.P(W), L.P(q["b"]), L.P(da)
            _count(M, Ht, Hs)
            if ds is not None:
                _count(M, Hs, Ht)
        L.call("magic_kd_emb", L.dt(W0.dtype), n, C.addressof(arr), Hs, Ht, C.addressof(Ms), C.addressof(Ws), C.addressof(bs), C.addressof(das), L.stream())
        i += n


def csr_gather(src, ptr, idx, w, out, n_out, H, accumulate=False):
    _chk(ptr.dtype == torch.int32 and idx.dtype == torch.int32 and ptr.numel() == n_out + 1, "csr arrays")
    L.call("magic_csr_gather", L.dt(src.dtype), n_out, H, L.P(src), L.P(ptr), L.P(idx), L.P(w), L.P(out), 1 if accumulate else 0,
           L.stream())


def cfp_loss_ok(B, H):
    return B <= 64 and H <= 256 and H % 8 == 0 and not os.environ.get("MAGIC_NO_FUSED_CFP")


_CFP_COUNTER = {}


def cfp_loss(B, H, a, txt, temperature, coef, rows, d_a=None, d_txt=None):
    _chk(len(a) == 3 and all(x.is_contiguous() and x.dtype == txt.dtype for x in a) and txt.is_contiguous(), "cfp_loss operands")
    d = d_a if d_a is not None else (None, None, None)
    part = cnt = None
    if d_txt is not None:
        part = torch.empty(3, B, H, dtype=torch.float32, device=txt.device)
        cnt = _CFP_COUNTER.get(txt.device)
        if cnt is None:
            cnt = _CFP_COUNTER[txt.device] = torch.zeros(1, dtype=torch.int32, device=txt.device)
    L.call("magic_cfp_loss", L.dt(txt.dtype), B, H, L.P(a[0]), L.P(a[1]), L.P(a[2]), L.P(txt), float(temperature), float(coef), L.P(rows),
           L.P(d[0]), L.P(d[1]), L.P(d[2]), L.P(d_txt), L.P(part), L.P(cnt), L.stream())


def csr_gather_multi(H, problems):
    import ctypes as C
    _chk(1 <= len(problems) <= 4, "csr_gather_multi problems")
    arr = (L.CsrProb * len(problems))()
    for j, q in enumerate(problems):
        d = arr[j]
        d.n_out, d.accumulate = int(q["n_out"]), 1 if q.get("accumulate") else 0
        d.out = L.P(q["out"])
        for i in (1, 2):
            csr = q.get(f"csr{i}")
            if csr is None:
                continue
            _chk(csr[0].dtype == torch.int32 and csr[1].dtype == torch.int32 and csr[0].numel() == d.n_out + 1, "csr arrays")
            setattr(d, f"src{i}", L.P(q[f"src{i}"])); setattr(d, f"ptr{i}", L.P(csr[0])); setattr(d, f"idx{i}", L.P(csr[1])); setattr(d, f"w{i}", L.P(csr[2]))
    L.call("magic_csr_gather_multi", L.dt(problems[0]["out"].dtype), H, len(problems), C.addressof(arr), L.stream())


def smallk_ln_bwd_pair(H, problems):
    import ctypes as C
    _chk(len(problems) == 2, "smallk_ln_bwd_pair takes two problems")
    arr = (L.SkbProb * 2)()
    Mmax = max(int(q["M"]) for q in problems)
    for j, q in enumerate(problems):
        d = arr[j]
        d.M, d.Kin = int(q["M"]), int(q["Kin"])
        for k in ("x", "dy", "y", "gamma", "beta", "rstd", "dW", "db", "dgamma", "dbeta"):
            setattr(d, k, L.P(q[k]))
        if part_ok(H):
            d.part = L.P(_skb_part(d.M, Mmax, H, d.Kin, q["dW"], q["db"], q["dgamma"], q["dbeta"], q["dy"].device))
    L.call("magic_smallk_ln_bwd_pair", L.dt(problems[0]["dy"].dtype), H, C.addressof(arr), L.stream())


NODE_IN_BWD = not os.environ.get("MAGIC_NO_NODE_IN_BWD")
_NIB_OK = {}


def node_in_bwd_ok(dtype, H, V=0, Mmax=0, Kin=(1,)):
    if not NODE_IN_BWD or dtype not in (torch.float32,) + tuple(L.HALF) or not all(1 <= int(k) <= 16 for k in Kin):
        return False
    key = (int(H), int(V), int(Mmax))
    if key not in _NIB_OK:
        _NIB_OK[key] = bool(L.load().magic_node_in_bwd_supported(*key))
    return _NIB_OK[key]


def node_in_bwd_blocks(Np=0, Ms=(), H=128):
    lib = L.load()
    Mmax = max([int(m) for m in Ms], default=0)
    return (int(lib.magic_pano_fuse_bwd_blocks(int(Np))) if Np else 0), [int(lib.magic_smallk_ln_bwd_blocks(int(m), H, Mmax)) for m in Ms]


def node_in_bwd(H, fuse=None, gathers=None, skb=(), table=None, add=None):
    _chk(fuse is not None or gathers is None, "node_in_bwd: the gathers ride in the fusion job")
    _chk(len(skb) <= 2, "node_in_bwd: at most two position-embedding problems")
    dt_ = None
    fa = [0, 0, None, None, None, None, None, None, None]
    gat = None
    if fuse is not None:
        x, dwf, dbf, N, V = fuse["x"], fuse["dwf"], fuse["dbf"], int(fuse["N"]), int(fuse["V"])
        dt_ = x.dtype
        if dwf is not None and dbf is not None and part_ok(H):
            nblk = node_in_bwd_blocks(Np=N, H=H)[0]
            pt = _part_rows(nblk, H + 1, x.device)
            flat = pt.view(-1)
            PART_JOBS.append((flat, dwf.reshape(-1), nblk, H, H + 1))
            PART_JOBS.append((flat[H:], dbf.reshape(-1), nblk, 1, H + 1))
            dwf, dbf = pt, None
        fa = [N, V, L.P(x), L.P(fuse["probs"]), L.P(fuse["wf"]), L.P(fuse["dfused"]), L.P(fuse["dx"]), L.P(dwf), L.P(dbf)]
        if gathers is not None:
            gat = (L.CsrProb * 2)()
            for j, q in enumerate(gathers):
                if q is None:
                    continue
                d = gat[j]
                d.n_out, d.accumulate, d.out = int(q["n_out"]), 1 if q.get("accumulate") else 0, L.P(q["out"])
                for i in (1, 2):
                    csr = q.get(f"csr{i}")
                    if csr is None:
                        continue
                    _chk(csr[0].dtype == torch.int32 and csr[1].dtype == torch.int32 and csr[0].numel() == d.n_out + 1, "csr arrays")
                    setattr(d, f"src{i}", L.P(q[f"src{i}"])); setattr(d, f"ptr{i}", L.P(csr[0])); setattr(d, f"idx{i}", L.P(csr[1])); setattr(d, f"w{i}", L.P(csr[2]))
    arr = None
    if skb:
        arr = (L.SkbProb * len(skb))()
        Mmax = max(int(q["M"]) for q in skb)
        for j, q in enumerate(skb):
            d = arr[j]
            d.M, d.Kin = int(q["M"]), int(q["Kin"])
            _chk(q["x"].dtype == torch.float32 and q["x"].is_contiguous(), "node_in_bwd x fp32 contiguous")
            for k in ("x", "dy", "y", "gamma", "beta", "rstd", "dW", "db", "dgamma", "dbeta"):
                setattr(d, k, L.P(q[k]))
            if part_ok(H):
                d.part = L.P(_skb_part(d.M, Mmax, H, d.Kin, q["dW"], q["db"], q["dgamma"], q["dbeta"], q["dy"].device))
        dt_ = dt_ or skb[0]["dy"].dtype
    ta = [0, None, None, None]
    if table is not None:
        _chk(table["idx"].dtype == torch.int32 and table["dtab"].dtype == torch.float32, "node_in_bwd table: int32 ids, fp32 gradient")
        ta = [int(table["M"]), L.P(table["dy"]), L.P(table["idx"]), L.P(table["dtab"])]
        dt_ = dt_ or table["dy"].dtype
    aa, xs_arr = [0, 0, None, None], None
    if add is not None:
        y, xs = add
        _chk(len(xs) >= 1 and all(t.dtype == y.dtype and t.numel() == y.numel() and t.is_contiguous() for t in xs) and y.is_contiguous(), "add_n operands")
        xs_arr = (C.c_void_p * len(xs))(*[t.data_ptr() for t in xs])
        aa = [y.numel(), len(xs), C.addressof(xs_arr), L.P(y)]
        dt_ = dt_ or y.dtype
    _chk(dt_ is not None, "node_in_bwd: no job")
    L.call("magic_node_in_bwd", L.dt(dt_), H, *fa, C.addressof(gat) if gat is not None else None, len(skb), C.addressof(arr) if arr is not None else None,
           *ta, *aa, L.stream())


def pano_fuse_fwd(x, lens, wf, bf, fused, probs, N, V, H, P=None, nh=0, inner=0, pmean=None):
    _chk(P is None or (P.dtype == x.dtype and P.is_contiguous() and pmean is not None and pmean.dtype == torch.float32), "pano_fuse head-mean operands")
    L.call("magic_pano_fuse_fwd", L.dt(x.dtype), N, V, H, L.P(x), L.P(lens), L.P(wf), L.P(bf), L.P(fused), L.P(probs),
           L.P(P), int(nh), int(inner), L.P(pmean), L.stream())


def pano_fuse_bwd(x, probs, wf, dfused, dx, dwf, dbf, N, V, H):
    if dwf is not None and dbf is not None and part_ok(H):
        nblk = int(L.load().magic_pano_fuse_bwd_blocks(int(N)))
        pt = _part_rows(nblk, H + 1, x.device)
        flat = pt.view(-1)
        PART_JOBS.append((flat, dwf.reshape(-1), nblk, H, H + 1))
        PART_JOBS.append((flat[H:], dbf.reshape(-1), nblk, 1, H + 1))
        dwf, dbf = pt, None
    L.call("magic_pano_fuse_bwd", L.dt(x.dtype), N, V, H, L.P(x), L.P(probs), L.P(wf), L.P(dfused), L.P(dx), L.P(dwf), L.P(dbf),
           L.stream())


def sap_fuse_fwd(B, K, Vp, g_raw, l_raw, fuse_raw, gmask, lmask, fsrc, bwmask, use_gate, gl, ll, fl):
    L.call("magic_sap_fuse_fwd", B, K, Vp, L.P(g_raw), L.P(l_raw), L.P(fuse_raw), L.P(gmask), L.P(lmask), L.P(fsrc), L.P(bwmask),
           1 if use_gate else 0, L.P(gl), L.P(ll), L.P(fl), L.stream())


SAP_LOSS_FUSED = not os.environ.get("MAGIC_NO_SAP_LOSS_FUSED")


def sap_fuse_loss(B, K, Vp, g_raw, l_raw, fuse_raw, gmask, lmask, fsrc, bwmask, use_gate, gl, ll, fl, glab, llab, coef, rows, *, dgl=None, dll=None,
                  dfl=None, ignore_index=-100, t_fused=None, w_rate=0.0, w_out=None, T=1.0, kd_norm=0.0, kd_coef=0.0, kd_coef_dev=None, kd_rows=None):
    import ctypes as C
    _chk(glab.dtype == torch.int32 and llab.dtype == torch.int32 and rows.dtype == torch.float32 and rows.numel() >= 3 * B, "sap_fuse_loss labels int32, rows fp32 [3, B]")
    _chk(t_fused is None or (t_fused.dtype == torch.float32 and t_fused.is_contiguous() and tuple(t_fused.shape) == (B, K)), "sap_fuse_loss teacher logits fp32 [B, K]")
    P = L.SapLossParams()
    P.B, P.K, P.Vp, P.use_gate = B, K, Vp, 1 if use_gate else 0
    for k, v in (("g_raw", g_raw), ("l_raw", l_raw), ("fuse_raw", fuse_raw), ("gmask", gmask), ("lmask", lmask), ("fsrc", fsrc), ("bwmask", bwmask),
                 ("gl", gl), ("ll", ll), ("fl", fl), ("glab", glab), ("llab", llab), ("rows", rows), ("dgl", dgl), ("dll", dll), ("dfl", dfl),
                 ("t_fused", t_fused), ("w_out", w_out), ("kd_coef_dev", kd_coef_dev), ("kd_rows", kd_rows)):
        setattr(P, k, L.P(v))
    P.ignore_index, P.coef, P.w_rate, P.T, P.kd_norm, P.kd_coef = int(ignore_index), float(coef), float(w_rate), float(T), float(kd_norm), float(kd_coef)
    L.call("magic_sap_fuse_loss", C.addressof(P), C.sizeof(P), L.stream())


def sap_fuse_bwd(B, K, Vp, g_raw, l_raw, fuse_raw, gmask, lmask, fsrc, bwmask, use_gate, dgl, dll, dfl, dg_raw, dl_raw, dfuse_raw):
    L.call("magic_sap_fuse_bwd", B, K, Vp, L.P(g_raw), L.P(l_raw), L.P(fuse_raw), L.P(gmask), L.P(lmask), L.P(fsrc), L.P(bwmask),
           1 if use_gate else 0, L.P(dgl), L.P(dll), L.P(dfl), L.P(dg_raw), L.P(dl_raw), L.P(dfuse_raw), L.stream())


def step_rng(base_seed, counter, rw_temp, seed_out=None, rw_out=None, zero_me=None, scale_state=None, growth=2.0, backoff=0.5, interval=2000):
    L.call("magic_step_rng", int(base_seed) & 0xFFFFFFFFFFFFFFFF, L.P(counter), float(rw_temp), L.P(seed_out), L.P(rw_out), L.P(zero_me),
           L.P(scale_state), float(growth), float(backoff), int(interval), L.stream())


def rowgate_fwd(mode, x, M, H, wx, *, e=None, we=None, b0=None, b1=None, out_s=None, out=None, gsave=None):
    L.call("magic_rowgate_fwd", L.dt(x.dtype), M, H, mode, L.P(x), L.P(e), L.P(wx), L.P(we), L.P(b0), L.P(b1), L.P(out_s), L.P(out), L.P(gsave), L.stream())


def rowgate_bwd(mode, x, M, H, wx, *, e=None, we=None, gsave=None, dy=None, dout=None, dx=None, de=None, dwx=None, dwe=None, db0=None, db1=None):
    L.call("magic_rowgate_bwd", L.dt(x.dtype), M, H, mode, L.P(x), L.P(e), L.P(wx), L.P(we), L.P(gsave), L.P(dy), L.P(dout), L.P(dx), L.P(de),
           L.P(dwx), L.P(dwe), L.P(db0), L.P(db1), L.stream())


def seed_scale(scale_state):
    L.call("magic_seed_scale", L.P(scale_state))


def loss_assemble(rows, row_w, row_scale, kd_rows, slots, rw, alpha, has_kd, out):
    _chk(rows.dtype == torch.float32 and rows.is_contiguous() and out.dtype == torch.float32 and out.numel() >= 13, "loss_assemble layout")
    L.call("magic_loss_assemble", L.P(rows), rows.numel(), L.P(row_w), float(row_scale), L.P(kd_rows), kd_rows.numel() if kd_rows is not None else 0,
           L.P(slots), L.P(rw), float(alpha), 1 if has_kd else 0, L.P(out), L.stream())
    return out


def sumsq(g, out):
    L.call("magic_sumsq", g.numel(), L.P(g), L.P(out), L.stream())


def sumsq_sched(g, out, step, lr0, warmup, total, b1, b2, lr_ss):
    _chk(step.numel() >= 2 and step.dtype == torch.int32, "schedule step words: int32[2] {global_step, optimizer state step}")
    L.call("magic_sumsq_sched", g.numel(), L.P(g), L.P(out), L.P(step), float(lr0), int(warmup), int(total), float(b1), float(b2), L.P(lr_ss), L.stream())


def adamw(n, p, g, m, v, shadow, lr, b1, b2, eps, wd, step_size, sumsq_buf, max_norm, gscale, lr_ss=None, n_decay=-1, zero_grad=False, overflow=None,
          scale_state=None, sched_step=None, decay_first=False):
    _chk(sched_step is None or (sched_step.numel() >= 2 and sched_step.dtype == torch.int32), "schedule step words: int32[2] {global_step, optimizer state step}")
    L.call("magic_adamw", n, L.P(p), L.P(g), L.P(m), L.P(v), L.P(shadow), L.dt(shadow.dtype) if shadow is not None else 1, float(lr), float(b1), float(b2), float(eps), float(wd),
           float(step_size), L.P(sumsq_buf), float(max_norm), float(gscale), L.P(lr_ss), int(n_decay), 1 if zero_grad else 0, L.P(overflow),
           L.P(scale_state), L.P(sched_step), 1 if decay_first else 0, L.stream())


def sched_step(step, lr0, warmup, total, b1, b2, lr_ss, zero_me=None):
    _chk(step.numel() >= 2 and step.dtype == torch.int32, "schedule step words: int32[2] {global_step, optimizer state step}")
    L.call("magic_sched_step", L.P(step), float(lr0), int(warmup), int(total), float(b1), float(b2), L.P(lr_ss), L.P(zero_me), L.stream())


def cast_to(x, dtype, out=None):
    if x.dtype == dtype:
        return x
    _chk((x.dtype == torch.float32) != (dtype == torch.float32) and (x.dtype in L.HALF or dtype in L.HALF), "cast_to: fp32 <-> 16-bit only")
    if out is None:
        out = torch.empty(x.shape, dtype=dtype, device=x.device)
    to16 = dtype in L.HALF
    L.call("magic_cast", L.dt(dtype if to16 else x.dtype), 1 if to16 else 0, x.numel(), L.P(x), L.P(out), L.stream())
    return out


def add_(y, x):
    L.call("magic_add", L.dt(y.dtype), y.numel(), L.P(x), L.P(y), L.stream())
    return y


def add_n(y, xs):
    import ctypes as C
    _chk(1 <= len(xs) <= 8 and all(x.dtype == y.dtype and x.numel() == y.numel() and x.is_contiguous() for x in xs), "add_n operands")
    arr = (C.c_void_p * len(xs))(*[x.data_ptr() for x in xs])
    L.call("magic_add_n", L.dt(y.dtype), y.numel(), len(xs), C.addressof(arr), L.P(y), L.stream())
    return y


def dact(dy, z, kind, out=None):
    if out is None:
        out = torch.empty_like(dy)
    L.call("magic_dact", L.dt(dy.dtype), kind, dy.numel(), L.P(dy), L.P(z), L.P(out), L.stream())
    return out
```

Before: 198,000.

## Fuse SAP head linear, LayerNorm-dot and loss into single forward and backward kernels

Adds a fused SAP head kernel that performs the global, local and fuse head linears with MFMA, bias and activation, LayerNorm dot and the SAP fuse loss in one launch. It replaces a sequence of about seven launches. A matching fused backward kernel is also added but is gated off by default behind an environment variable. The loss and backward bodies are moved into a shared header so the old kernels and the new fused kernels reuse the same code. The aim is to cut launch overhead and intermediate global-memory traffic for these small per-step head shapes, at the cost of a large new kernel with heavy LDS use and a shape-restricted support check.

Result: no change. 197,800 (-0.1%).

```diff
diff --git a/include/magic_hip.h b/include/magic_hip.h
--- a/include/magic_hip.h
+++ b/include/magic_hip.h
@@ -226,6 +226,14 @@
                        const unsigned char* gmask, const unsigned char* lmask, const int* fsrc, const unsigned char* bwmask,
                        int use_gate, const float* dgl, const float* dll, const float* dfl,
                        float* dg_raw, float* dl_raw, float* dfuse_raw, void* stream);
+int magic_sap_head_supported(int dtype, int H, int K, int Vp);
+int magic_sap_head_fwd(int dtype, int H, const void* gx, const void* lx, const void* const* W, const float* const* vecs, float eps,
+                       void* const* Y, const void* params, int nbytes, void* stream);
+int magic_sap_head_bwd_blocks(int B);
+int magic_sap_head_bwd(int dtype, int H, int B, int K, int Vp, int use_gate, const float* g_raw, const float* l_raw, const float* fuse_raw,
+                       const unsigned char* gmask, const unsigned char* lmask, const int* fsrc, const unsigned char* bwmask,
+                       const float* dgl, const float* dll, const float* dfl, const void* const* Y, const void* const* W,
+                       const float* const* vecs, float eps, void* const* dZ, void* d_gmap, void* d_vp, float* part, void* stream);
 
 int magic_step_rng(unsigned long long base_seed, unsigned* counter, float rw_temp, int* seed_out, float* rw_out, float* zero_me,
                    float* scale_state, float growth, float backoff, int interval, void* stream);
diff --git a/profiles/micro/sap_head_probe.py b/profiles/micro/sap_head_probe.py
--- /dev/null
+++ b/profiles/micro/sap_head_probe.py
@@ -0,0 +1,116 @@
+import os
+import statistics
+import sys
+
+import torch
+
+sys.path.insert(0, os.path.join(os.path.dirname(os.path.abspath(__file__)), "..", ".."))
+import magic_amd
+from magic_amd.host import lib as L
+from magic_amd.host import ops as O
+
+ROUNDS = int(sys.argv[1]) if len(sys.argv) > 1 else 12
+REPS = int(sys.argv[2]) if len(sys.argv) > 2 else 20
+B, K, Vp, H, DT, EPS = 48, 80, 37, 128, torch.bfloat16, 1e-12
+dev = "cuda"
+f32 = dict(dtype=torch.float32, device=dev)
+gx, lx = torch.randn(B * K, H, device=dev).to(DT), torch.randn(B * Vp, H, device=dev).to(DT)
+heads = []
+for h in range(3):
+    cols = 2 * H if h == 2 else H
+    q = dict(W=(torch.randn(H, cols, device=dev) / cols ** 0.5).to(DT), b1=0.3 * torch.randn(H, **f32), g=1 + 0.2 * torch.randn(H, **f32), be=0.3 * torch.randn(H, **f32),
+             w2=torch.randn(H, **f32) / H ** 0.5, b2=0.2 * torch.randn(1, **f32))
+    q.update(dg=torch.zeros(H, **f32), dbe=torch.zeros(H, **f32), dw2=torch.zeros(H, **f32), db2=torch.zeros(1, **f32))
+    heads.append(q)
+hg, hl, hf = heads
+gmask = (torch.rand(B, K, device=dev) < 0.6).to(torch.uint8)
+lmask = (torch.rand(B, Vp, device=dev) < 0.6).to(torch.uint8)
+gmask[:, 0] = 1
+lmask[:, 0] = 1
+fsrc = torch.randint(-2, Vp, (B, K), device=dev, dtype=torch.int32)
+bwm = (torch.rand(B, Vp, device=dev) < 0.3).to(torch.uint8)
+glab, llab = torch.zeros(B, dtype=torch.int32, device=dev), torch.zeros(B, dtype=torch.int32, device=dev)
+t_fused = 2 * torch.randn(B, K, **f32)
+t_fused[gmask == 0] = float("-inf")
+kdev = torch.ones(1, **f32)
+Yg, Yl, Yf = torch.empty(B * K, H, device=dev, dtype=DT), torch.empty(B * Vp, H, device=dev, dtype=DT), torch.empty(B, H, device=dev, dtype=DT)
+dZg, dZl, dZf = torch.empty_like(Yg), torch.empty_like(Yl), torch.empty_like(Yf)
+g_raw, l_raw, fuse_raw = torch.empty(B * K, **f32), torch.empty(B * Vp, **f32), torch.empty(B, **f32)
+gl, ll, fl = torch.empty(B, K, **f32), torch.empty(B, Vp, **f32), torch.empty(B, K, **f32)
+rows, dgl, dll, dfl = torch.empty(3, B, **f32), torch.empty(B, K, **f32), torch.empty(B, Vp, **f32), torch.empty(B, K, **f32)
+w_out, kdr = torch.empty(B, **f32), torch.empty(B, **f32)
+dg, dl, df = torch.empty(B, K, **f32), torch.empty(B, Vp, **f32), torch.empty(B, **f32)
+d_gmap, d_vp = torch.zeros(B * K, H, device=dev, dtype=DT), torch.zeros(B * Vp, H, device=dev, dtype=DT)
+fuse = (B, K, Vp, g_raw, l_raw, fuse_raw, gmask, lmask, fsrc, bwm, True)
+loss = (gl, ll, fl, glab, llab, 0.5 / B, rows)
+lkw = dict(dgl=dgl, dll=dll, dfl=dfl, t_fused=t_fused, w_rate=0.7, w_out=w_out, T=2.0, kd_norm=1.0 / B, kd_coef=0.2, kd_coef_dev=kdev, kd_rows=kdr)
+
+
+def seq_fwd():
+    with L.group():
+        O.linear_fwd(gx, hg["W"], hg["b1"], B * K, epilogue=2, out=Yg)
+        O.linear_fwd(lx, hl["W"], hl["b1"], B * Vp, epilogue=2, out=Yl)
+        tmp = O.linear_fwd(gx, hf["W"], None, B, lda=K * H, ldb=2 * H, K=H)
+    O.lndot_fwd(Yg, B * K, H, hg["g"], hg["be"], EPS, hg["w2"], hg["b2"], g_raw)
+    O.lndot_fwd(Yl, B * Vp, H, hl["g"], hl["be"], EPS, hl["w2"], hl["b2"], l_raw)
+    O.linear_fwd(lx, hf["W"][:, H:], hf["b1"], B, lda=Vp * H, ldb=2 * H, K=H, residual=tmp, epilogue=0, out=Yf)
+    O.dact(Yf, Yf, 2, out=Yf)
+    O.lndot_fwd(Yf, B, H, hf["g"], hf["be"], EPS, hf["w2"], hf["b2"], fuse_raw)
+    O.sap_fuse_loss(*fuse, *loss, **lkw)
+
+
+def seq_bwd():
+    O.sap_fuse_bwd(*fuse, dgl, dll, dfl, dg, dl, df)
+    O.lndot_bwd(Yg, B * K, H, hg["g"], hg["be"], EPS, hg["w2"], dg, dZg, hg["dg"], hg["dbe"], hg["dw2"], hg["db2"])
+    O.lndot_bwd(Yl, B * Vp, H, hl["g"], hl["be"], EPS, hl["w2"], dl, dZl, hl["dg"], hl["dbe"], hl["dw2"], hl["db2"])
+    with L.group():
+        O.linear_dx(dZg, hg["W"], B * K, out=d_gmap, residual=d_gmap)
+        O.linear_dx(dZl, hl["W"], B * Vp, out=d_vp, residual=d_vp)
+    O.lndot_bwd(Yf, B, H, hf["g"], hf["be"], EPS, hf["w2"], df, dZf, hf["dg"], hf["dbe"], hf["dw2"], hf["db2"])
+    with L.group():
+        O.linear_dx(dZf, hf["W"], B, out=d_gmap, residual=d_gmap, ldb=2 * H, ldc=K * H, N=H, K=H)
+        O.linear_dx(dZf, hf["W"][:, H:], B, out=d_vp, residual=d_vp, ldb=2 * H, ldc=Vp * H, N=H, K=H)
+
+
+def fus_fwd():
+    O.sap_head_fwd(gx, lx, heads, EPS, (Yg, Yl, Yf), *fuse, *loss, **lkw)
+
+
+def fus_bwd():
+    O.sap_head_bwd(heads, EPS, (Yg, Yl, Yf), (dZg, dZl, dZf), d_gmap, d_vp, *fuse, dgl, dll, dfl)
+
+
+def timed(fn):
+    e0, e1 = torch.cuda.Event(enable_timing=True), torch.cuda.Event(enable_timing=True)
+    O.defer_dw(True)
+    try:
+        e0.record()
+        for _ in range(REPS):
+            fn()
+        e1.record()
+        e1.synchronize()
+        O.flush_dw()
+    finally:
+        O.defer_dw(False)
+    return e0.elapsed_time(e1) * 1e3 / REPS
+
+
+forms = (("sequence forward (7 launches)", seq_fwd), ("fused forward (1 launch)", fus_fwd), ("sequence backward (6 launches)", seq_bwd), ("fused backward (1 launch)", fus_bwd))
+for _ in range(3):
+    for _, fn in forms:
+        timed(fn)
+torch.cuda.synchronize()
+res = {name: [] for name, _ in forms}
+for r in range(ROUNDS):
+    for name, fn in forms:
+        res[name].append(timed(fn))
+print(f"B {B}, K {K}, Vp {Vp}, H {H}, bf16; {ROUNDS} rounds x {REPS} back-to-back calls per form, interleaved; us per call")
+print("round  " + "  ".join(f"{name.split(' (')[0]:>17s}" for name, _ in forms))
+for r in range(ROUNDS):
+    print(f"{r:5d}  " + "  ".join(f"{res[name][r]:17.2f}" for name, _ in forms))
+med = {name: statistics.median(v) for name, v in res.items()}
+for name, _ in forms:
+    print(f"{name:32s} median {med[name]:7.2f} us  min {min(res[name]):7.2f} us")
+names = [n for n, _ in forms]
+print(f"forward: {med[names[0]] - med[names[1]]:.2f} us less per call; backward: {med[names[2]] - med[names[3]]:.2f} us less per call; "
+      f"thirteen launches {med[names[0]] + med[names[2]]:.2f} us against two {med[names[1]] + med[names[3]]:.2f} us")
diff --git a/vln-magic_amd/csrc/build_id.py b/vln-magic_amd/csrc/build_id.py
--- a/vln-magic_amd/csrc/build_id.py
+++ b/vln-magic_amd/csrc/build_id.py
@@ -4,7 +4,7 @@
 import sys
 
 HERE = os.path.dirname(os.path.abspath(__file__))
-HEADERS = ("common.hpp", "group.hpp", "enc_common.hpp", os.path.join("..", "..", "include", "magic_hip.h"))
+HEADERS = ("common.hpp", "group.hpp", "enc_common.hpp", "saploss.hpp", os.path.join("..", "..", "include", "magic_hip.h"))
 EXTRA = ("gen_fastcall.py", "build_id.py", os.path.join("..", "host", "abi.py"), os.path.join("..", "host", "lib.py"), "hostplan.c")
 
 
diff --git a/vln-magic_amd/csrc/graphops.hip b/vln-magic_amd/csrc/graphops.hip
--- a/vln-magic_amd/csrc/graphops.hip
+++ b/vln-magic_amd/csrc/graphops.hip
@@ -271,103 +271,11 @@
   }
 }
 
-using SapLossParams = magic_sap_loss_params;
-__device__ __forceinline__ float sap_ce_wave(const float* x, int N, int lab, int ignore_index, float coef, float* d, int lane) {
-  const bool ignored = (lab == ignore_index) || lab < 0 || lab >= N;
-  const float xl = ignored ? 0.f : x[lab];
-  float mx = -3.0e38f;
-  for (int c = lane; c < N; c += 64) mx = fmaxf(mx, x[c]);
-  mx = wave_max(mx);
-  float s = 0.f;
-  for (int c = lane; c < N; c += 64) s += __expf(x[c] - mx);
-  s = wave_sum(s);
-  const float lse = mx + __logf(s);
-  if (d) {
-    const float cf = ignored ? 0.f : coef;
-    for (int c = lane; c < N; c += 64) d[c] = cf * (__expf(x[c] - lse) - (c == lab ? 1.f : 0.f));
-  }
-  return ignored ? 0.f : lse - xl;
-}
+#include "saploss.hpp"
 __global__ __launch_bounds__(64) void sap_fuse_loss_kernel(SapLossParams p, const float* ss) {
   __shared__ float sl[128];
-  if (ss) { p.coef *= ss[0]; p.kd_coef *= ss[0]; }
   __shared__ float sbw;
-  const int b = blockIdx.x, lane = threadIdx.x, B = p.B, K = p.K, Vp = p.Vp;
-  const float NEG = -__builtin_inff();
-  const float fw = p.use_gate ? 1.f / (1.f + __expf(-p.fuse_raw[b])) : 0.5f;
-  float* gl = p.gl + (long long)b * K; float* ll = p.ll + (long long)b * Vp; float* fl = p.fl + (long long)b * K;
-  float bw = 0.f;
-  for (int j = lane; j < Vp; j += 64) {
-    const float v = p.lmask[b * Vp + j] ? p.l_raw[b * Vp + j] * (1.f - fw) : NEG;
-    ll[j] = v; sl[j] = v;
-    if (p.bwmask[b * Vp + j] && p.lmask[b * Vp + j]) bw += v;
-  }
-  bw = wave_sum(bw);
-  if (lane == 0) sbw = bw;
-  __syncthreads();
-  for (int k = lane; k < K; k += 64) {
-    const float v = p.gmask[b * K + k] ? p.g_raw[b * K + k] * fw : NEG;
-    gl[k] = v;
-    const int s = p.fsrc[b * K + k];
-    float add = 0.f;
-    if (s >= 0) add = sl[s]; else if (s == -2) add = sbw;
-    fl[k] = v + add;
-  }
-  __syncthreads();
-  const int gla = p.glab[b], lla = p.llab[b];
-  const float l0 = sap_ce_wave(gl, K, gla, p.ignore_index, p.coef, p.dgl ? p.dgl + (long long)b * K : nullptr, lane);
-  const float l1 = sap_ce_wave(ll, Vp, lla, p.ignore_index, p.coef, p.dll ? p.dll + (long long)b * Vp : nullptr, lane);
-  float* dfl = p.dfl ? p.dfl + (long long)b * K : nullptr;
-  const float l2 = sap_ce_wave(fl, K, gla, p.ignore_index, p.coef, dfl, lane);
-  if (lane == 0) { p.rows[b] = l0; p.rows[B + b] = l1; p.rows[2 * B + b] = l2; }
-  if (!p.t_fused) return;
-  const float* t = p.t_fused + (long long)b * K;
-  float wr = 1.f;
-  if (p.w_out) {
-    wr = __expf(-p.w_rate * sap_ce_wave(t, K, gla, p.ignore_index, 0.f, nullptr, lane));
-    if (lane == 0) p.w_out[b] = wr;
-  }
-  if (!p.kd_rows) return;
-  __syncthreads();
-  float coef = p.kd_coef;
-  if (p.kd_coef_dev) coef *= p.kd_coef_dev[0];
-  const float invT = 1.0f / p.T;
-  float sv[8], tv[8], ms = -3.0e38f, mt = -3.0e38f;
-#pragma unroll
-  for (int it = 0; it < 8; ++it) {
-    const int c = it * 64 + lane;
-    float a = -3.0e38f, q = -3.0e38f;
-    if (c < K) {
-      a = fl[c]; q = t[c];
-      if (a == NEG) a = -1e6f;
-      if (q == NEG) q = -1e6f;
-      a *= invT; q *= invT;
-      ms = fmaxf(ms, a); mt = fmaxf(mt, q);
-    }
-    sv[it] = a; tv[it] = q;
-  }
-  ms = wave_max(ms); mt = wave_max(mt);
-  float zs = 0.f, zt = 0.f;
-#pragma unroll
-  for (int it = 0; it < 8; ++it) {
-    const int c = it * 64 + lane;
-    if (c < K) { zs += __expf(sv[it] - ms); zt += __expf(tv[it] - mt); }
-  }
-  zs = wave_sum(zs); zt = wave_sum(zt);
-  const float ls = ms + __logf(zs), lt = mt + __logf(zt);
-  float kl = 0.f;
-#pragma unroll
-  for (int it = 0; it < 8; ++it) {
-    const int c = it * 64 + lane;
-    if (c < K) {
-      const float lpt = tv[it] - lt, lps = sv[it] - ls;
-      const float pt = __expf(lpt), ps = __expf(lps);
-      if (pt > 0.f) kl += pt * (lpt - lps);
-      if (dfl) dfl[c] += coef * wr * p.T * (ps - pt) * p.kd_norm;
-    }
-  }
-  kl = wave_sum(kl);
-  if (lane == 0) p.kd_rows[b] = wr * kl * p.T * p.T * p.kd_norm;
+  sap_loss_body(p, ss, blockIdx.x, threadIdx.x, true, sl, &sbw);
 }
 
 __global__ __launch_bounds__(64) void sap_fuse_bwd_kernel(int B, int K, int Vp, const float* g_raw, const float* l_raw, const float* fuse_raw,
@@ -376,33 +284,9 @@
                                                           const float* dfl, float* dg_raw, float* dl_raw, float* dfuse_raw) {
   __shared__ float dl[128];
   __shared__ float sbw;
-  const int b = blockIdx.x, tid = threadIdx.x;
-  const float fw = use_gate != 0.f ? 1.f / (1.f + __expf(-fuse_raw[b])) : 0.5f;
-  for (int j = tid; j < Vp; j += 64) dl[j] = (dll && lmask[b * Vp + j]) ? dll[b * Vp + j] : 0.f;
-  if (tid == 0) sbw = 0.f;
-  __syncthreads();
-  float dfw = 0.f;
-  for (int k = tid; k < K; k += 64) {
-    const bool ok = gmask[b * K + k];
-    const float dg = ok ? ((dgl ? dgl[b * K + k] : 0.f) + (dfl ? dfl[b * K + k] : 0.f)) : 0.f;
-    dg_raw[b * K + k] = dg * fw;
-    dfw += dg * g_raw[b * K + k];
-    if (dfl && ok) {
-      const int s = fsrc[b * K + k];
-      const float d = dfl[b * K + k];
-      if (s >= 0) atomicAdd(&dl[s], d); else if (s == -2) atomicAdd(&sbw, d);
-    }
-  }
-  __syncthreads();
-  for (int j = tid; j < Vp; j += 64) {
-    float d = dl[j];
-    if (bwmask[b * Vp + j]) d += sbw;
-    if (!lmask[b * Vp + j]) d = 0.f;
-    dl_raw[b * Vp + j] = d * (1.f - fw);
-    dfw -= d * l_raw[b * Vp + j];
-  }
-  dfw = wave_sum(dfw);
-  if (tid == 0) dfuse_raw[b] = use_gate != 0.f ? dfw * fw * (1.f - fw) : 0.f;
+  const int b = blockIdx.x;
+  sap_bwd_body(K, Vp, g_raw, l_raw, fuse_raw, gmask, lmask, fsrc, bwmask, use_gate, dgl, dll, dfl, dg_raw + b * K, dl_raw + b * Vp, dfuse_raw + b,
+               b, threadIdx.x, true, dl, &sbw);
 }
 
 extern "C" int magic_csr_gather(int dtype, int n_out, int H, const void* src, const int* ptr, const int* idx, const float* w,
diff --git a/vln-magic_amd/csrc/saphead.hip b/vln-magic_amd/csrc/saphead.hip
--- /dev/null
+++ b/vln-magic_amd/csrc/saphead.hip
@@ -0,0 +1,439 @@
+#include "saploss.hpp"
+#include <cstring>
+
+#define SH_NT 256
+#define SH_R 32
+
+struct SapHeadVec { const float *b1, *g, *be, *w2, *b2; };
+struct SapHeadFwd {
+  const void *gx, *lx; const void* W[3]; SapHeadVec v[3]; float eps; void* Y[3];
+  SapLossParams lp; const float* ss;
+};
+struct SapHeadBwd {
+  int B, K, Vp, use_gate;
+  const float *g_raw, *l_raw, *fuse_raw; const unsigned char *gmask, *lmask; const int* fsrc; const unsigned char* bwmask;
+  const float *dgl, *dll, *dfl;
+  const void* Y[3]; const void* W[3]; SapHeadVec v[3]; float eps;
+  void* dZ[3]; void *dg, *dv; float* part;
+};
+
+template <int H> static constexpr size_t sh_fwd_lds() { return (size_t)(H + SH_R) * (H + 8) * 2 + 132 * 4; }
+template <int H> static constexpr size_t sh_bwd_lds() { return (size_t)(H + SH_R) * (H + 8) * 2 + (512 + 128 + 128 + 4) * 4; }
+
+__device__ __forceinline__ void sh_ld2(const bf16* p, float& a, float& b) {
+  typedef __attribute__((ext_vector_type(2))) __bf16 bf16x2;
+  bf16x2 v = *(const bf16x2*)p; a = (float)v[0]; b = (float)v[1];
+}
+__device__ __forceinline__ void sh_ld2(const f16* p, float& a, float& b) {
+  typedef __attribute__((ext_vector_type(2))) _Float16 f16x2;
+  f16x2 v = *(const f16x2*)p; a = (float)v[0]; b = (float)v[1];
+}
+__device__ __forceinline__ void sh_st2(bf16* p, bf16* q, float a, float b) {
+  typedef __attribute__((ext_vector_type(2))) __bf16 bf16x2;
+  bf16x2 v; v[0] = (bf16)a; v[1] = (bf16)b; *(bf16x2*)p = v; *(bf16x2*)q = v;
+}
+__device__ __forceinline__ void sh_st2(f16* p, f16* q, float a, float b) {
+  typedef __attribute__((ext_vector_type(2))) _Float16 f16x2;
+  f16x2 v; v[0] = (f16)a; v[1] = (f16)b; *(f16x2*)p = v; *(f16x2*)q = v;
+}
+
+template <typename Hh, int H>
+__device__ __forceinline__ void sh_stage(Hh* sW, const Hh* __restrict__ W, const int ld, const int tid) {
+  typedef h16x8<Hh> v8;
+  constexpr int CH = H / 8;
+#pragma unroll 4
+  for (int c = tid; c < H * CH; c += SH_NT) {
+    const int row = c / CH, cv = c % CH;
+    *(v8*)(sW + row * (H + 8) + cv * 8) = *(const v8*)(W + (long long)row * ld + cv * 8);
+  }
+}
+template <typename Hh> __device__ __forceinline__ h16x8<Hh> sh_zero8() {
+  h16x8<Hh> z;
+#pragma unroll
+  for (int e = 0; e < 8; ++e) z[e] = (Hh)0.0f;
+  return z;
+}
+template <typename Hh, int H>
+__device__ __forceinline__ void sh_afrag(const Hh* p, const int lane, h16x8<Hh> (&a)[H / 32]) {
+#pragma unroll
+  for (int ks = 0; ks < H / 32; ++ks) a[ks] = p ? *(const h16x8<Hh>*)(p + ks * 32 + 8 * (lane >> 4)) : sh_zero8<Hh>();
+}
+template <typename Hh, int H, int NJ>
+__device__ __forceinline__ void sh_mma_nt(const h16x8<Hh> (&a)[H / 32], const Hh* sW, const int col0, const int lane, f32x4 (&acc)[NJ]) {
+  typedef h16x8<Hh> v8;
+#pragma unroll
+  for (int ks = 0; ks < H / 32; ++ks) {
+    v8 b[NJ];
+#pragma unroll
+    for (int j = 0; j < NJ; ++j) b[j] = *(const v8*)(sW + (col0 + j * 16 + (lane & 15)) * (H + 8) + ks * 32 + 8 * (lane >> 4));
+#pragma unroll
+    for (int j = 0; j < NJ; ++j) acc[j] = mfma16(a[ks], b[j], acc[j]);
+  }
+}
+template <typename Hh, int H, int NJ>
+__device__ __forceinline__ void sh_mma_nn(const h16x8<Hh> (&a)[H / 32], const Hh* sW, const int col0, const int lane, f32x4 (&acc)[NJ]) {
+  typedef h16x8<Hh> v8;
+  const int g4 = lane >> 4, q4 = (lane & 15) >> 2, pp = lane & 3;
+#pragma unroll
+  for (int ks = 0; ks < H / 32; ++ks) {
+    v8 b[NJ];
+#pragma unroll
+    for (int j = 0; j < NJ; ++j) b[j] = lds_tr8(sW + (ks * 32 + 8 * g4 + q4) * (H + 8) + col0 + j * 16 + 4 * pp, 4 * (H + 8));
+#pragma unroll
+    for (int j = 0; j < NJ; ++j) acc[j] = mfma16(a[ks], b[j], acc[j]);
+  }
+}
+
+template <typename Hh, int NIT>
+__device__ __forceinline__ float sh_lndot_row(const Hh* y, const SapHeadVec& v, const float eps, const int lane, float (&x)[2 * NIT]) {
+  constexpr int H = 128 * NIT;
+  float s = 0.f;
+#pragma unroll
+  for (int it = 0; it < NIT; ++it) { sh_ld2(y + it * 128 + lane * 2, x[2 * it], x[2 * it + 1]); s += x[2 * it] + x[2 * it + 1]; }
+  const float mean = wave_sum(s) / H;
+  float q = 0.f;
+#pragma unroll
+  for (int it = 0; it < NIT; ++it) { float a = x[2 * it] - mean, b = x[2 * it + 1] - mean; q += a * a + b * b; }
+  const float rstd = rsqrtf(wave_sum(q) / H + eps);
+  float d = 0.f;
+#pragma unroll
+  for (int it = 0; it < NIT; ++it) {
+    const int c = it * 128 + lane * 2;
+    d += ((x[2 * it] - mean) * rstd * v.g[c] + v.be[c]) * v.w2[c] + ((x[2 * it + 1] - mean) * rstd * v.g[c + 1] + v.be[c + 1]) * v.w2[c + 1];
+  }
+  d = wave_sum(d);
+  return d + v.b2[0];
+}
+
+template <typename Hh, int H>
+__global__ __launch_bounds__(SH_NT) void sap_head_fwd_kernel(SapHeadFwd a) {
+  extern __shared__ __attribute__((aligned(16))) unsigned char sh_smem[];
+  constexpr int NIT = H / 128, WP = H + 8, NJ = H / 32, NJG = H / 64;
+  Hh* const sW = (Hh*)sh_smem;
+  Hh* const sY = sW + H * WP;
+  float* const sl = (float*)(sY + SH_R * WP);
+  float* const sbw = sl + 128;
+  typedef h16x8<Hh> v8;
+  const int b = blockIdx.x, tid = threadIdx.x, lane = tid & 63, wid = tid >> 6, rh = wid >> 1, ch = wid & 1;
+  const int K = a.lp.K, Vp = a.lp.Vp;
+
+  for (int hd = 0; hd < 2; ++hd) {
+    const int R = hd ? Vp : K;
+    const Hh* __restrict__ X = (const Hh*)(hd ? a.lx : a.gx) + (long long)b * R * H;
+    Hh* __restrict__ Yo = (Hh*)a.Y[hd] + (long long)b * R * H;
+    float* __restrict__ raw = (float*)(hd ? a.lp.l_raw : a.lp.g_raw) + (long long)b * R;
+    const SapHeadVec& hv = a.v[hd];
+    sh_stage<Hh, H>(sW, (const Hh*)a.W[hd], H, tid);
+    float bv[NJ];
+#pragma unroll
+    for (int j = 0; j < NJ; ++j) bv[j] = hv.b1[ch * (H / 2) + j * 16 + (lane & 15)];
+    __syncthreads();
+    for (int r0 = 0; r0 < R; r0 += SH_R) {
+      {
+        const int ar = r0 + 16 * rh + (lane & 15);
+        v8 af[H / 32];
+        sh_afrag<Hh, H>(ar < R ? X + (long long)ar * H : nullptr, lane, af);
+        f32x4 acc[NJ];
+#pragma unroll
+        for (int j = 0; j < NJ; ++j) acc[j] = (f32x4){0.f, 0.f, 0.f, 0.f};
+        sh_mma_nt<Hh, H, NJ>(af, sW, ch * (H / 2), lane, acc);
+#pragma unroll
+        for (int j = 0; j < NJ; ++j)
+#pragma unroll
+          for (int r = 0; r < 4; ++r)
+            sY[(16 * rh + 4 * (lane >> 4) + r) * WP + ch * (H / 2) + j * 16 + (lane & 15)] = from_f<Hh>(fmaxf(acc[j][r] * 1.f + bv[j], 0.f));
+      }
+      __syncthreads();
+#pragma unroll 2
+      for (int i = 0; i < SH_R / 4; ++i) {
+        const int lr = wid * (SH_R / 4) + i, row = r0 + lr;
+        if (row < R) {
+          float x[2 * NIT];
+          const float d = sh_lndot_row<Hh, NIT>(sY + lr * WP, hv, a.eps, lane, x);
+#pragma unroll
+          for (int it = 0; it < NIT; ++it)
+            *(unsigned*)(Yo + (long long)row * H + it * 128 + lane * 2) = *(const unsigned*)(sY + lr * WP + it * 128 + lane * 2);
+          if (lane == 0) raw[row] = d;
+        }
+      }
+      __syncthreads();
+    }
+  }
+  float* const fuse_raw = (float*)a.lp.fuse_raw;
+  if (a.lp.use_gate) {
+    const SapHeadVec& hv = a.v[2];
+    float tmpf[NJG];
+#pragma unroll
+    for (int half = 0; half < 2; ++half) {
+      sh_stage<Hh, H>(sW, (const Hh*)a.W[2] + half * H, 2 * H, tid);
+      __syncthreads();
+      const Hh* x0 = half ? (const Hh*)a.lx + (long long)b * Vp * H : (const Hh*)a.gx + (long long)b * K * H;
+      v8 af[H / 32];
+      sh_afrag<Hh, H>((lane & 15) == 0 ? x0 : nullptr, lane, af);
+      f32x4 acc[NJG];
+#pragma unroll
+      for (int j = 0; j < NJG; ++j) acc[j] = (f32x4){0.f, 0.f, 0.f, 0.f};
+      sh_mma_nt<Hh, H, NJG>(af, sW, wid * (H / 4), lane, acc);
+      if (half == 0) {
+#pragma unroll
+        for (int j = 0; j < NJG; ++j) tmpf[j] = to_f(from_f<Hh>(acc[j][0] * 1.f + 0.f));
+      } else if (lane < 16) {
+#pragma unroll
+        for (int j = 0; j < NJG; ++j) {
+          const int col = wid * (H / 4) + j * 16 + lane;
+          float v = acc[j][0] * 1.f + hv.b1[col];
+          v += tmpf[j];
+          const float z = to_f(from_f<Hh>(v));
+          const Hh yf = from_f<Hh>(z * (z > 0.f ? 1.f : 0.f));
+          sY[col] = yf;
+          ((Hh*)a.Y[2])[(long long)b * H + col] = yf;
+        }
+      }
+      __syncthreads();
+    }
+    if (wid == 0) {
+      float x[2 * NIT];
+      const float d = sh_lndot_row<Hh, NIT>(sY, hv, a.eps, lane, x);
+      if (lane == 0) fuse_raw[b] = d;
+    }
+  } else if (tid == 0) {
+    fuse_raw[b] = 0.f;
+  }
+  __syncthreads();
+  sap_loss_body(a.lp, a.ss, b, tid, tid < 64, sl, sbw);
+}
+
+template <typename Hh, int H>
+__global__ __launch_bounds__(SH_NT) void sap_head_bwd_kernel(SapHeadBwd a) {
+  extern __shared__ __attribute__((aligned(16))) unsigned char sh_smem[];
+  constexpr int NIT = H / 128, WP = H + 8, NJ = H / 32, NJG = H / 64, PS = 3 * H + 1;
+  Hh* const sW = (Hh*)sh_smem;
+  Hh* const sZ = sW + H * WP;
+  float* const red = (float*)sZ;
+  float* const sdg = (float*)(sZ + SH_R * WP);
+  float* const sdl = sdg + 512;
+  float* const dlb = sdl + 128;
+  float* const sbw = dlb + 128;
+  float* const sdf = sbw + 1;
+  static_assert((size_t)SH_R * WP * 2 >= (size_t)(12 * H + 4) * 4, "the parameter sums fit the dZ tile");
+  typedef h16x8<Hh> v8;
+  const int b = blockIdx.x, tid = threadIdx.x, lane = tid & 63, wid = tid >> 6, rh = wid >> 1, ch = wid & 1;
+  const int K = a.K, Vp = a.Vp;
+
+  sap_bwd_body(K, Vp, a.g_raw, a.l_raw, a.fuse_raw, a.gmask, a.lmask, a.fsrc, a.bwmask, a.use_gate ? 1.f : 0.f, a.dgl, a.dll, a.dfl, sdg, sdl, sdf,
+               b, tid, tid < 64, dlb, sbw);
+  const int nhd = a.use_gate ? 3 : 2;
+  for (int hd = 0; hd < nhd; ++hd) {
+    const int R = hd == 0 ? K : hd == 1 ? Vp : 1;
+    const long long row0 = (long long)b * R;
+    const Hh* __restrict__ Y = (const Hh*)a.Y[hd] + row0 * H;
+    Hh* __restrict__ dZ = (Hh*)a.dZ[hd] + row0 * H;
+    const float* dlog = hd == 0 ? sdg : hd == 1 ? sdl : sdf;
+    const SapHeadVec& hv = a.v[hd];
+    if (hd < 2) sh_stage<Hh, H>(sW, (const Hh*)a.W[hd], H, tid);
+    float ag[2 * NIT], ab[2 * NIT], aw[2 * NIT], adb = 0.f;
+#pragma unroll
+    for (int i = 0; i < 2 * NIT; ++i) { ag[i] = 0.f; ab[i] = 0.f; aw[i] = 0.f; }
+    __syncthreads();
+    for (int r0 = 0; r0 < R; r0 += SH_R) {
+#pragma unroll 2
+      for (int i = 0; i < SH_R / 4; ++i) {
+        const int lr = wid * (SH_R / 4) + i, row = r0 + lr;
+        Hh* zt = sZ + lr * WP;
+        if (row < R) {
+          float x[2 * NIT];
+          float s = 0.f;
+#pragma unroll
+          for (int it = 0; it < NIT; ++it) { sh_ld2(Y + (long long)row * H + it * 128 + lane * 2, x[2 * it], x[2 * it + 1]); s += x[2 * it] + x[2 * it + 1]; }
+          const float mean = wave_sum(s) / H;
+          float q = 0.f;
+#pragma unroll
+          for (int it = 0; it < NIT; ++it) { float u = x[2 * it] - mean, w = x[2 * it + 1] - mean; q += u * u + w * w; }
+          const float rstd = rsqrtf(wave_sum(q) / H + a.eps);
+          const float dl = dlog[row];
+          adb += dl;
+          float g[2 * NIT], xh[2 * NIT];
+          float s1 = 0.f, s2 = 0.f;
+#pragma unroll
+          for (int it = 0; it < NIT; ++it) {
+#pragma unroll
+            for (int e = 0; e < 2; ++e) {
+              const int c = it * 128 + lane * 2 + e, k = 2 * it + e;
+              xh[k] = (x[k] - mean) * rstd;
+              const float dln = dl * hv.w2[c];
+              aw[k] += dl * (xh[k] * hv.g[c] + hv.be[c]);
+              ag[k] += dln * xh[k]; ab[k] += dln;
+              g[k] = dln * hv.g[c];
+              s1 += g[k]; s2 += g[k] * xh[k];
+            }
+          }
+          const float m1 = wave_sum(s1) / H, m2 = wave_sum(s2) / H;
+#pragma unroll
+          for (int it = 0; it < NIT; ++it) {
+            const float da = x[2 * it] > 0.f ? rstd * (g[2 * it] - m1 - xh[2 * it] * m2) : 0.f;
+            const float dbv = x[2 * it + 1] > 0.f ? rstd * (g[2 * it + 1] - m1 - xh[2 * it + 1] * m2) : 0.f;
+            sh_st2(dZ + (long long)row * H + it * 128 + lane * 2, zt + it * 128 + lane * 2, da, dbv);
+          }
+        } else {
+#pragma unroll
+          for (int it = 0; it < NIT; ++it) *(unsigned*)(zt + it * 128 + lane * 2) = 0u;
+        }
+      }
+      __syncthreads();
+      if (hd < 2) {
+        Hh* __restrict__ D = (Hh*)(hd ? a.dv : a.dg) + row0 * H;
+        v8 af[H / 32];
+        sh_afrag<Hh, H>(sZ + (16 * rh + (lane & 15)) * WP, lane, af);
+        float rs[NJ][4];
+#pragma unroll
+        for (int j = 0; j < NJ; ++j)
+#pragma unroll
+          for (int r = 0; r < 4; ++r) {
+            const int row = r0 + 16 * rh + 4 * (lane >> 4) + r;
+            rs[j][r] = row < R ? to_f(D[(long long)row * H + ch * (H / 2) + j * 16 + (lane & 15)]) : 0.f;
+          }
+        f32x4 acc[NJ];
+#pragma unroll
+        for (int j = 0; j < NJ; ++j) acc[j] = (f32x4){0.f, 0.f, 0.f, 0.f};
+        sh_mma_nn<Hh, H, NJ>(af, sW, ch * (H / 2), lane, acc);
+#pragma unroll
+        for (int j = 0; j < NJ; ++j)
+#pragma unroll
+          for (int r = 0; r < 4; ++r) {
+            const int row = r0 + 16 * rh + 4 * (lane >> 4) + r;
+            if (row < R) D[(long long)row * H + ch * (H / 2) + j * 16 + (lane & 15)] = from_f<Hh>((acc[j][r] * 1.f + 0.f) + rs[j][r]);
+          }
+        __syncthreads();
+      }
+    }
+    v8 zf[H / 32];
+    if (hd == 2) {
+      sh_afrag<Hh, H>((lane & 15) == 0 ? sZ : nullptr, lane, zf);
+      __syncthreads();
+    }
+#pragma unroll
+    for (int it = 0; it < NIT; ++it) {
+      const int c = it * 128 + lane * 2;
+      red[(0 * 4 + wid) * H + c] = ag[2 * it]; red[(0 * 4 + wid) * H + c + 1] = ag[2 * it + 1];
+      red[(1 * 4 + wid) * H + c] = ab[2 * it]; red[(1 * 4 + wid) * H + c + 1] = ab[2 * it + 1];
+      red[(2 * 4 + wid) * H + c] = aw[2 * it]; red[(2 * 4 + wid) * H + c + 1] = aw[2 * it + 1];
+    }
+    if (lane == 0) red[12 * H + wid] = adb;
+    __syncthreads();
+    {
+      float* prow = a.part + ((long long)hd * a.B + b) * PS;
+      for (int c = tid; c < H; c += SH_NT) {
+        prow[c] = red[c] + red[H + c] + red[2 * H + c] + red[3 * H + c];
+        prow[H + c] = red[4 * H + c] + red[5 * H + c] + red[6 * H + c] + red[7 * H + c];
+        prow[2 * H + c] = red[8 * H + c] + red[9 * H + c] + red[10 * H + c] + red[11 * H + c];
+      }
+      if (tid == 0) prow[3 * H] = red[12 * H] + red[12 * H + 1] + red[12 * H + 2] + red[12 * H + 3];
+    }
+    if (hd == 2) {
+#pragma unroll
+      for (int half = 0; half < 2; ++half) {
+        __syncthreads();
+        sh_stage<Hh, H>(sW, (const Hh*)a.W[2] + half * H, 2 * H, tid);
+        __syncthreads();
+        f32x4 acc[NJG];
+#pragma unroll
+        for (int j = 0; j < NJG; ++j) acc[j] = (f32x4){0.f, 0.f, 0.f, 0.f};
+        sh_mma_nn<Hh, H, NJG>(zf, sW, wid * (H / 4), lane, acc);
+        if (lane < 16) {
+          Hh* D = half ? (Hh*)a.dv + (long long)b * Vp * H : (Hh*)a.dg + (long long)b * K * H;
+#pragma unroll
+          for (int j = 0; j < NJG; ++j) {
+            const int col = wid * (H / 4) + j * 16 + lane;
+            D[col] = from_f<Hh>((acc[j][0] * 1.f + 0.f) + to_f(D[col]));
+          }
+        }
+      }
+    }
+  }
+}
+
+static inline bool sh_vec_ok(const float* const* v, int n) {
+  for (int i = 0; i < n; ++i) if (!v[i]) return false;
+  return true;
+}
+static inline void sh_vecs(SapHeadVec (&o)[3], const float* const* v, int nh) {
+  for (int h = 0; h < 3; ++h) {
+    if (h < nh) o[h] = SapHeadVec{v[5 * h], v[5 * h + 1], v[5 * h + 2], v[5 * h + 3], v[5 * h + 4]};
+    else o[h] = SapHeadVec{nullptr, nullptr, nullptr, nullptr, nullptr};
+  }
+}
+static inline bool sh_al16(const void* p) { return ((uintptr_t)p & 15) == 0; }
+template <typename K> static void sh_attr(K k, size_t bytes) { (void)hipFuncSetAttribute((const void*)k, hipFuncAttributeMaxDynamicSharedMemorySize, (int)bytes); }
+
+extern "C" int magic_sap_head_supported(int dtype, int H, int K, int Vp) {
+  return (dtype_is16(dtype) && (H == 128 || H == 256) && K >= 1 && K <= 512 && Vp >= 1 && Vp <= 128) ? 1 : 0;
+}
+
+extern "C" int magic_sap_head_fwd(int dtype, int H, const void* gx, const void* lx, const void* const* W, const float* const* vecs, float eps,
+                                  void* const* Y, const void* params, int nbytes, void* stream) {
+  if (!params || nbytes != (int)sizeof(SapLossParams) || !gx || !lx || !W || !vecs || !Y) return MAGIC_ERR_ARG;
+  SapHeadFwd a;
+  memcpy(&a.lp, params, sizeof(a.lp));
+  const SapLossParams& p = a.lp;
+  if (p.B <= 0 || !magic_sap_head_supported(dtype, H, p.K, p.Vp)) return MAGIC_ERR_ARG;
+  if (!p.g_raw || !p.l_raw || !p.fuse_raw || !p.gmask || !p.lmask || !p.fsrc || !p.bwmask || !p.gl || !p.ll || !p.fl) return MAGIC_ERR_ARG;
+  if (p.glab) {
+    if (!p.llab || !p.rows) return MAGIC_ERR_ARG;
+    if ((p.w_out || p.kd_rows) && !p.t_fused) return MAGIC_ERR_ARG;
+    if (p.kd_rows && !(p.T > 0.f)) return MAGIC_ERR_ARG;
+  } else if (p.llab || p.rows || p.dgl || p.dll || p.dfl || p.t_fused || p.w_out || p.kd_rows) {
+    return MAGIC_ERR_ARG;
+  }
+  const int nh = p.use_gate ? 3 : 2;
+  if (!sh_vec_ok(vecs, 5 * nh)) return MAGIC_ERR_ARG;
+  for (int h = 0; h < nh; ++h) if (!W[h] || !Y[h] || !sh_al16(W[h]) || !sh_al16(Y[h])) return MAGIC_ERR_ARG;
+  if (!sh_al16(gx) || !sh_al16(lx)) return MAGIC_ERR_ARG;
+  a.gx = gx; a.lx = lx; a.eps = eps; a.ss = seed_scale_get();
+  for (int h = 0; h < 3; ++h) { a.W[h] = h < nh ? W[h] : nullptr; a.Y[h] = h < nh ? Y[h] : nullptr; }
+  sh_vecs(a.v, vecs, nh);
+  static bool attr = false;
+  if (!attr) {
+    sh_attr(sap_head_fwd_kernel<bf16, 128>, sh_fwd_lds<128>()); sh_attr(sap_head_fwd_kernel<f16, 128>, sh_fwd_lds<128>());
+    sh_attr(sap_head_fwd_kernel<bf16, 256>, sh_fwd_lds<256>()); sh_attr(sap_head_fwd_kernel<f16, 256>, sh_fwd_lds<256>());
+    attr = true;
+  }
+  dim3 grid(p.B), block(SH_NT);
+  hipStream_t st = (hipStream_t)stream;
+#define SHF(TY, HH) hipLaunchKernelGGL((sap_head_fwd_kernel<TY, HH>), grid, block, sh_fwd_lds<HH>(), st, a)
+  if (dtype == DT_BF16) { if (H == 128) SHF(bf16, 128); else SHF(bf16, 256); }
+  else { if (H == 128) SHF(f16, 128); else SHF(f16, 256); }
+#undef SHF
+  return launch_status();
+}
+
+extern "C" int magic_sap_head_bwd_blocks(int B) { return B > 0 ? B : MAGIC_ERR_ARG; }
+extern "C" int magic_sap_head_bwd(int dtype, int H, int B, int K, int Vp, int use_gate, const float* g_raw, const float* l_raw, const float* fuse_raw,
+                                  const unsigned char* gmask, const unsigned char* lmask, const int* fsrc, const unsigned char* bwmask,
+                                  const float* dgl, const float* dll, const float* dfl, const void* const* Y, const void* const* W,
+                                  const float* const* vecs, float eps, void* const* dZ, void* d_gmap, void* d_vp, float* part, void* stream) {
+  if (B <= 0 || !magic_sap_head_supported(dtype, H, K, Vp)) return MAGIC_ERR_ARG;
+  if (!g_raw || !l_raw || !fuse_raw || !gmask || !lmask || !fsrc || !bwmask || !Y || !W || !vecs || !dZ || !d_gmap || !d_vp || !part) return MAGIC_ERR_ARG;
+  const int nh = use_gate ? 3 : 2;
+  if (!sh_vec_ok(vecs, 5 * nh)) return MAGIC_ERR_ARG;
+  for (int h = 0; h < nh; ++h) if (!W[h] || !Y[h] || !dZ[h] || !sh_al16(W[h]) || !sh_al16(Y[h]) || !sh_al16(dZ[h])) return MAGIC_ERR_ARG;
+  if (!sh_al16(d_gmap) || !sh_al16(d_vp)) return MAGIC_ERR_ARG;
+  SapHeadBwd a;
+  a.B = B; a.K = K; a.Vp = Vp; a.use_gate = use_gate ? 1 : 0;
+  a.g_raw = g_raw; a.l_raw = l_raw; a.fuse_raw = fuse_raw; a.gmask = gmask; a.lmask = lmask; a.fsrc = fsrc; a.bwmask = bwmask;
+  a.dgl = dgl; a.dll = dll; a.dfl = dfl; a.eps = eps; a.dg = d_gmap; a.dv = d_vp; a.part = part;
+  for (int h = 0; h < 3; ++h) { a.W[h] = h < nh ? W[h] : nullptr; a.Y[h] = h < nh ? Y[h] : nullptr; a.dZ[h] = h < nh ? dZ[h] : nullptr; }
+  sh_vecs(a.v, vecs, nh);
+  static bool attr = false;
+  if (!attr) {
+    sh_attr(sap_head_bwd_kernel<bf16, 128>, sh_bwd_lds<128>()); sh_attr(sap_head_bwd_kernel<f16, 128>, sh_bwd_lds<128>());
+    sh_attr(sap_head_bwd_kernel<bf16, 256>, sh_bwd_lds<256>()); sh_attr(sap_head_bwd_kernel<f16, 256>, sh_bwd_lds<256>());
+    attr = true;
+  }
+  dim3 grid(B), block(SH_NT);
+  hipStream_t st = (hipStream_t)stream;
+#define SHB(TY, HH) hipLaunchKernelGGL((sap_head_bwd_kernel<TY, HH>), grid, block, sh_bwd_lds<HH>(), st, a)
+  if (dtype == DT_BF16) { if (H == 128) SHB(bf16, 128); else SHB(bf16, 256); }
+  else { if (H == 128) SHB(f16, 128); else SHB(f16, 256); }
+#undef SHB
+  return launch_status();
+}
diff --git a/vln-magic_amd/csrc/saploss.hpp b/vln-magic_amd/csrc/saploss.hpp
--- /dev/null
+++ b/vln-magic_amd/csrc/saploss.hpp
@@ -0,0 +1,146 @@
+#pragma once
+#include "common.hpp"
+
+using SapLossParams = magic_sap_loss_params;
+__device__ __forceinline__ float sap_ce_wave(const float* x, int N, int lab, int ignore_index, float coef, float* d, int lane) {
+  const bool ignored = (lab == ignore_index) || lab < 0 || lab >= N;
+  const float xl = ignored ? 0.f : x[lab];
+  float mx = -3.0e38f;
+  for (int c = lane; c < N; c += 64) mx = fmaxf(mx, x[c]);
+  mx = wave_max(mx);
+  float s = 0.f;
+  for (int c = lane; c < N; c += 64) s += __expf(x[c] - mx);
+  s = wave_sum(s);
+  const float lse = mx + __logf(s);
+  if (d) {
+    const float cf = ignored ? 0.f : coef;
+    for (int c = lane; c < N; c += 64) d[c] = cf * (__expf(x[c] - lse) - (c == lab ? 1.f : 0.f));
+  }
+  return ignored ? 0.f : lse - xl;
+}
+
+__device__ __forceinline__ void sap_loss_body(SapLossParams p, const float* ss, const int b, const int lane, const bool on, float* sl, float* sbw) {
+  if (ss) { p.coef *= ss[0]; p.kd_coef *= ss[0]; }
+  const int B = p.B, K = p.K, Vp = p.Vp;
+  const float NEG = -__builtin_inff();
+  const float fw = p.use_gate ? 1.f / (1.f + __expf(-p.fuse_raw[b])) : 0.5f;
+  float* gl = p.gl + (long long)b * K; float* ll = p.ll + (long long)b * Vp; float* fl = p.fl + (long long)b * K;
+  if (on) {
+    float bw = 0.f;
+    for (int j = lane; j < Vp; j += 64) {
+      const float v = p.lmask[b * Vp + j] ? p.l_raw[b * Vp + j] * (1.f - fw) : NEG;
+      ll[j] = v; sl[j] = v;
+      if (p.bwmask[b * Vp + j] && p.lmask[b * Vp + j]) bw += v;
+    }
+    bw = wave_sum(bw);
+    if (lane == 0) *sbw = bw;
+  }
+  __syncthreads();
+  if (on) {
+    for (int k = lane; k < K; k += 64) {
+      const float v = p.gmask[b * K + k] ? p.g_raw[b * K + k] * fw : NEG;
+      gl[k] = v;
+      const int s = p.fsrc[b * K + k];
+      float add = 0.f;
+      if (s >= 0) add = sl[s]; else if (s == -2) add = *sbw;
+      fl[k] = v + add;
+    }
+  }
+  if (!p.glab) return;
+  __syncthreads();
+  const int gla = p.glab[b], lla = p.llab[b];
+  float* dfl = p.dfl ? p.dfl + (long long)b * K : nullptr;
+  if (on) {
+    const float l0 = sap_ce_wave(gl, K, gla, p.ignore_index, p.coef, p.dgl ? p.dgl + (long long)b * K : nullptr, lane);
+    const float l1 = sap_ce_wave(ll, Vp, lla, p.ignore_index, p.coef, p.dll ? p.dll + (long long)b * Vp : nullptr, lane);
+    const float l2 = sap_ce_wave(fl, K, gla, p.ignore_index, p.coef, dfl, lane);
+    if (lane == 0) { p.rows[b] = l0; p.rows[B + b] = l1; p.rows[2 * B + b] = l2; }
+  }
+  if (!p.t_fused) return;
+  const float* t = p.t_fused + (long long)b * K;
+  float wr = 1.f;
+  if (on && p.w_out) {
+    wr = __expf(-p.w_rate * sap_ce_wave(t, K, gla, p.ignore_index, 0.f, nullptr, lane));
+    if (lane == 0) p.w_out[b] = wr;
+  }
+  if (!p.kd_rows) return;
+  __syncthreads();
+  if (!on) return;
+  float coef = p.kd_coef;
+  if (p.kd_coef_dev) coef *= p.kd_coef_dev[0];
+  const float invT = 1.0f / p.T;
+  float sv[8], tv[8], ms = -3.0e38f, mt = -3.0e38f;
+#pragma unroll
+  for (int it = 0; it < 8; ++it) {
+    const int c = it * 64 + lane;
+    float a = -3.0e38f, q = -3.0e38f;
+    if (c < K) {
+      a = fl[c]; q = t[c];
+      if (a == NEG) a = -1e6f;
+      if (q == NEG) q = -1e6f;
+      a *= invT; q *= invT;
+      ms = fmaxf(ms, a); mt = fmaxf(mt, q);
+    }
+    sv[it] = a; tv[it] = q;
+  }
+  ms = wave_max(ms); mt = wave_max(mt);
+  float zs = 0.f, zt = 0.f;
+#pragma unroll
+  for (int it = 0; it < 8; ++it) {
+    const int c = it * 64 + lane;
+    if (c < K) { zs += __expf(sv[it] - ms); zt += __expf(tv[it] - mt); }
+  }
+  zs = wave_sum(zs); zt = wave_sum(zt);
+  const float ls = ms + __logf(zs), lt = mt + __logf(zt);
+  float kl = 0.f;
+#pragma unroll
+  for (int it = 0; it < 8; ++it) {
+    const int c = it * 64 + lane;
+    if (c < K) {
+      const float lpt = tv[it] - lt, lps = sv[it] - ls;
+      const float pt = __expf(lpt), ps = __expf(lps);
+      if (pt > 0.f) kl += pt * (lpt - lps);
+      if (dfl) dfl[c] += coef * wr * p.T * (ps - pt) * p.kd_norm;
+    }
+  }
+  kl = wave_sum(kl);
+  if (lane == 0) p.kd_rows[b] = wr * kl * p.T * p.T * p.kd_norm;
+}
+
+__device__ __forceinline__ void sap_bwd_body(const int K, const int Vp, const float* g_raw, const float* l_raw, const float* fuse_raw,
+                                             const unsigned char* gmask, const unsigned char* lmask, const int* fsrc, const unsigned char* bwmask,
+                                             const float use_gate, const float* dgl, const float* dll, const float* dfl, float* dg, float* dl_out, float* df,
+                                             const int b, const int tid, const bool on, float* dl, float* sbw) {
+  const float fw = use_gate != 0.f ? 1.f / (1.f + __expf(-fuse_raw[b])) : 0.5f;
+  if (on) {
+    for (int j = tid; j < Vp; j += 64) dl[j] = (dll && lmask[b * Vp + j]) ? dll[b * Vp + j] : 0.f;
+    if (tid == 0) *sbw = 0.f;
+  }
+  __syncthreads();
+  float dfw = 0.f;
+  if (on) {
+    for (int k = tid; k < K; k += 64) {
+      const bool ok = gmask[b * K + k];
+      const float d = ok ? ((dgl ? dgl[b * K + k] : 0.f) + (dfl ? dfl[b * K + k] : 0.f)) : 0.f;
+      dg[k] = d * fw;
+      dfw += d * g_raw[b * K + k];
+      if (dfl && ok) {
+        const int s = fsrc[b * K + k];
+        const float dd = dfl[b * K + k];
+        if (s >= 0) atomicAdd(&dl[s], dd); else if (s == -2) atomicAdd(sbw, dd);
+      }
+    }
+  }
+  __syncthreads();
+  if (on) {
+    for (int j = tid; j < Vp; j += 64) {
+      float d = dl[j];
+      if (bwmask[b * Vp + j]) d += *sbw;
+      if (!lmask[b * Vp + j]) d = 0.f;
+      dl_out[j] = d * (1.f - fw);
+      dfw -= d * l_raw[b * Vp + j];
+    }
+    dfw = wave_sum(dfw);
+    if (tid == 0) *df = use_gate != 0.f ? dfw * fw * (1.f - fw) : 0.f;
+  }
+}
diff --git a/vln-magic_amd/host/model_pretrain.py b/vln-magic_amd/host/model_pretrain.py
--- a/vln-magic_amd/host/model_pretrain.py
+++ b/vln-magic_amd/host/model_pretrain.py
@@ -67,6 +67,7 @@
 MLM_TAIL_FUSED = os.environ.get("MAGIC_MLM_TAIL_FUSED", "1") != "0"
 MLM_DX_SPLITK = int(os.environ.get("MAGIC_MLM_DX_SPLITK", "32"))
 MLM_DX_ATOMICS = os.environ.get("MAGIC_MLM_DX_ATOMICS", "0") != "0"
+TEACHER_SAP_HEAD = os.environ.get("MAGIC_TEACHER_SAP_HEAD", "0") != "0"
 
 
 class GlocalTextPathCMTPreTraining(nn.Module):
@@ -314,29 +315,38 @@
             elif task == "sap":
                 from . import lib as _lib
                 use_gate = bool(cfg_get(self.config, "glocal_fuse"))
-                g1, l1_ = n.lin("global_sap_head.net.0.weight"), n.lin("local_sap_head.net.0.weight")
-                with _lib.group():
-                    c.Yg = O.linear_fwd(c.glob.out, g1.W, g1.b, B * K, epilogue=2)
-                    c.Yl = O.linear_fwd(c.loc.out, l1_.W, l1_.b, B * Vp, epilogue=2)
-                    if use_gate:
-                        f1 = n.lin("sap_fuse_linear.net.0.weight")
-                        tmp = O.linear_fwd(c.glob.out, f1.W, None, B, lda=K * H, ldb=2 * H, K=H)
-                c.g_raw = self._cls_tail("global_sap_head.", c.Yg, B * K)
-                c.l_raw = self._cls_tail("local_sap_head.", c.Yl, B * Vp)
-                if use_gate:
-                    c.Yf = O.linear_fwd(c.loc.out, f1.W[:, H:], f1.b, B, lda=Vp * H, ldb=2 * H, K=H, residual=tmp, epilogue=0)
-                    self._relu(c.Yf)
-                    fln, f2 = n.ln("sap_fuse_linear.net.2"), n.lin("sap_fuse_linear.net.3.weight")
-                    c.fuse_raw = n.new(B, dtype=torch.float32)
-                    O.lndot_fwd(c.Yf, B, H, fln.g, fln.b, n.eps, f2.Wm, f2.b, c.fuse_raw)
-                else:
-                    c.fuse_raw = n.zeros(B, dtype=torch.float32)
                 c.use_gate = use_gate
                 c.gl, c.ll, c.fl = n.new(B, K, dtype=torch.float32), n.new(B, Vp, dtype=torch.float32), n.new(B, K, dtype=torch.float32)
-                c.sap_fused = bool(compute_loss and O.SAP_LOSS_FUSED and K <= 512 and Vp <= 128)
-                if not c.sap_fused:
-                    O.sap_fuse_fwd(B, K, Vp, c.g_raw, c.l_raw, c.fuse_raw, plan["gmask"], plan["lmask"], plan["fsrc"], plan["bwmask"],
-                                   use_gate, c.gl, c.ll, c.fl)
+                c.sap_head = bool(O.sap_head_ok(n.dtype, H, K, Vp) and (compute_loss or TEACHER_SAP_HEAD))
+                if c.sap_head:
+                    c.Yg, c.Yl, c.Yf = n.new(B * K, H), n.new(B * Vp, H), (n.new(B, H) if use_gate else None)
+                    c.g_raw, c.l_raw, c.fuse_raw = n.new(B * K, dtype=torch.float32), n.new(B * Vp, dtype=torch.float32), n.new(B, dtype=torch.float32)
+                    c.sap_fused = bool(compute_loss)
+                    if not compute_loss:
+                        O.sap_head_fwd(c.glob.out, c.loc.out, self._sap_heads(), n.eps, (c.Yg, c.Yl, c.Yf), B, K, Vp, c.g_raw, c.l_raw, c.fuse_raw,
+                                       plan["gmask"], plan["lmask"], plan["fsrc"], plan["bwmask"], use_gate, c.gl, c.ll, c.fl)
+                else:
+                    g1, l1_ = n.lin("global_sap_head.net.0.weight"), n.lin("local_sap_head.net.0.weight")
+                    with _lib.group():
+                        c.Yg = O.linear_fwd(c.glob.out, g1.W, g1.b, B * K, epilogue=2)
+                        c.Yl = O.linear_fwd(c.loc.out, l1_.W, l1_.b, B * Vp, epilogue=2)
+                        if use_gate:
+                            f1 = n.lin("sap_fuse_linear.net.0.weight")
+                            tmp = O.linear_fwd(c.glob.out, f1.W, None, B, lda=K * H, ldb=2 * H, K=H)
+                    c.g_raw = self._cls_tail("global_sap_head.", c.Yg, B * K)
+                    c.l_raw = self._cls_tail("local_sap_head.", c.Yl, B * Vp)
+                    if use_gate:
+                        c.Yf = O.linear_fwd(c.loc.out, f1.W[:, H:], f1.b, B, lda=Vp * H, ldb=2 * H, K=H, residual=tmp, epilogue=0)
+                        self._relu(c.Yf)
+                        fln, f2 = n.ln("sap_fuse_linear.net.2"), n.lin("sap_fuse_linear.net.3.weight")
+                        c.fuse_raw = n.new(B, dtype=torch.float32)
+                        O.lndot_fwd(c.Yf, B, H, fln.g, fln.b, n.eps, f2.Wm, f2.b, c.fuse_raw)
+                    else:
+                        c.fuse_raw = n.zeros(B, dtype=torch.float32)
+                    c.sap_fused = bool(compute_loss and O.SAP_LOSS_FUSED and K <= 512 and Vp <= 128)
+                    if not c.sap_fused:
+                        O.sap_fuse_fwd(B, K, Vp, c.g_raw, c.l_raw, c.fuse_raw, plan["gmask"], plan["lmask"], plan["fsrc"], plan["bwmask"],
+                                       use_gate, c.gl, c.ll, c.fl)
                 o.update(global_logits=c.gl, local_logits=c.ll, fused_logits=c.fl)
             elif task == "cfp":
                 c.g0, c.v0, c.t0, c.gv0 = n.new(B, H), n.new(B, H), n.new(B, H), n.new(B, H)
@@ -521,12 +531,16 @@
                     c.kdrows = n.new(B, dtype=torch.float32)
                 if kd:
                     rwd = self._rw_device(rw)
-                O.sap_fuse_loss(B, K, Vp, c.g_raw, c.l_raw, c.fuse_raw, plan["gmask"], plan["lmask"], plan["fsrc"], plan["bwmask"], c.use_gate,
-                                c.gl, c.ll, c.fl, ga, la, scg / B, c.rows, dgl=c.dgl, dll=c.dll, dfl=c.dfl,
-                                t_fused=t["fused_logits"] if (hard or pred) else None,
-                                w_rate=float(kdl["t_sample_preprocess_exp_decay"]) if hard else 0.0, w_out=c.sap_w,
-                                T=float(kdl["kd_temperature"]) if kd else 1.0, kd_norm=(1.0 / B if hard else 1.0 / (B * K)),
-                                kd_coef=alpha * gs, kd_coef_dev=rwd[4:5] if pred else None, kd_rows=c.kdrows)
+                lkw = dict(dgl=c.dgl, dll=c.dll, dfl=c.dfl, t_fused=t["fused_logits"] if (hard or pred) else None,
+                           w_rate=float(kdl["t_sample_preprocess_exp_decay"]) if hard else 0.0, w_out=c.sap_w,
+                           T=float(kdl["kd_temperature"]) if kd else 1.0, kd_norm=(1.0 / B if hard else 1.0 / (B * K)),
+                           kd_coef=alpha * gs, kd_coef_dev=rwd[4:5] if pred else None, kd_rows=c.kdrows)
+                fargs = (B, K, Vp, c.g_raw, c.l_raw, c.fuse_raw, plan["gmask"], plan["lmask"], plan["fsrc"], plan["bwmask"], c.use_gate,
+                         c.gl, c.ll, c.fl, ga, la, scg / B, c.rows)
+                if getattr(c, "sap_head", False):
+                    O.sap_head_fwd(c.glob.out, c.loc.out, self._sap_heads(), n.eps, (c.Yg, c.Yl, c.Yf), *fargs, **lkw)
+                else:
+                    O.sap_fuse_loss(*fargs, **lkw)
             else:
                 O.ce_rows(c.gl, B, K, K, ga, coef=scg / B, loss_row=c.rows[0], dlogits=c.dgl, ldd=K)
                 O.ce_rows(c.ll, B, Vp, Vp, la, coef=scg / B, loss_row=c.rows[1], dlogits=c.dll, ldd=Vp)
@@ -663,6 +677,44 @@
         else:
             self.backward_phase2()
 
+    def _sap_heads(self, grads=False):
+        n, out = self.net, []
+        for prefix in ("global_sap_head.", "local_sap_head.", "sap_fuse_linear."):
+            l1, ln, l2 = n.lin(prefix + "net.0.weight"), n.ln(prefix + "net.2"), n.lin(prefix + "net.3.weight")
+            q = dict(W=l1.W, b1=l1.b, g=ln.g, be=ln.b, w2=l2.Wm, b2=l2.b)
+            if grads:
+                q.update(dg=ln.dg, dbe=ln.db, dw2=l2.dW, db2=l2.db)
+            out.append(q)
+        return out
+
+    def _sap_heads_bwd_seq(self, c):
+        n, plan = self.net, c.plan
+        B, K, Vp, H = plan["B"], plan["K"], plan["Vp"], n.H
+        dg, dl, df = n.new(B, K, dtype=torch.float32), n.new(B, Vp, dtype=torch.float32), n.new(B, dtype=torch.float32)
+        O.sap_fuse_bwd(B, K, Vp, c.g_raw, c.l_raw, c.fuse_raw, plan["gmask"], plan["lmask"], plan["fsrc"], plan["bwmask"],
+                       c.use_gate, c.dgl, c.dll, c.dfl, dg, dl, df)
+        from . import lib as _lib
+        heads = []
+        for prefix, X, Y, dlogit, M, d_acc in (("global_sap_head.", c.glob.out, c.Yg, dg, B * K, c.d_gmap),
+                                               ("local_sap_head.", c.loc.out, c.Yl, dl, B * Vp, c.d_vp)):
+            l1, ln, l2 = n.lin(prefix + "net.0.weight"), n.ln(prefix + "net.2"), n.lin(prefix + "net.3.weight")
+            dZh = n.new(M, H)
+            O.lndot_bwd(Y, M, H, ln.g, ln.b, n.eps, l2.Wm, dlogit, dZh, ln.dg, ln.db, l2.dW, l2.db)
+            O.linear_dw(dZh, X, l1.dW, l1.db, M)
+            heads.append((dZh, l1, M, d_acc))
+        with _lib.group():
+            for dZh, l1, M, d_acc in heads:
+                O.linear_dx(dZh, l1.W, M, out=d_acc, residual=d_acc)
+        if c.use_gate:
+            f1, fln, f2 = n.lin("sap_fuse_linear.net.0.weight"), n.ln("sap_fuse_linear.net.2"), n.lin("sap_fuse_linear.net.3.weight")
+            dZ = n.new(B, H)
+            O.lndot_bwd(c.Yf, B, H, fln.g, fln.b, n.eps, f2.Wm, df, dZ, fln.dg, fln.db, f2.dW, f2.db)
+            O.linear_dw(dZ, c.glob.out, f1.dW, f1.db, B, N=H, K=H, ldb=K * H, ldc=2 * H)
+            O.linear_dw(dZ, c.loc.out, f1.dW[:, H:], None, B, N=H, K=H, ldb=Vp * H, ldc=2 * H)
+            with _lib.group():
+                O.linear_dx(dZ, f1.W, B, out=c.d_gmap, residual=c.d_gmap, ldb=2 * H, ldc=K * H, N=H, K=H)
+                O.linear_dx(dZ, f1.W[:, H:], B, out=c.d_vp, residual=c.d_vp, ldb=2 * H, ldc=Vp * H, N=H, K=H)
+
     @torch.no_grad()
     def backward_phase1(self):
         c = self._ctx
@@ -672,30 +724,20 @@
         n, plan, task = self.net, c.plan, c.task
         B, L, K, Vp, H = plan["B"], plan["L"], plan["K"], plan["Vp"], n.H
         if task == "sap":
-            dg, dl, df = n.new(B, K, dtype=torch.float32), n.new(B, Vp, dtype=torch.float32), n.new(B, dtype=torch.float32)
-            O.sap_fuse_bwd(B, K, Vp, c.g_raw, c.l_raw, c.fuse_raw, plan["gmask"], plan["lmask"], plan["fsrc"], plan["bwmask"],
-                           c.use_gate, c.dgl, c.dll, c.dfl, dg, dl, df)
-            from . import lib as _lib
-            heads = []
-            for prefix, X, Y, dlogit, M, d_acc in (("global_sap_head.", c.glob.out, c.Yg, dg, B * K, c.d_gmap),
-                                                   ("local_sap_head.", c.loc.out, c.Yl, dl, B * Vp, c.d_vp)):
-                l1, ln, l2 = n.lin(prefix + "net.0.weight"), n.ln(prefix + "net.2"), n.lin(prefix + "net.3.weight")
-                dZh = n.new(M, H)
-                O.lndot_bwd(Y, M, H, ln.g, ln.b, n.eps, l2.Wm, dlogit, dZh, ln.dg, ln.db, l2.dW, l2.db)
-                O.linear_dw(dZh, X, l1.dW, l1.db, M)
-                heads.append((dZh, l1, M, d_acc))
-            with _lib.group():
-                for dZh, l1, M, d_acc in heads:
-                    O.linear_dx(dZh, l1.W, M, out=d_acc, residual=d_acc)
-            if c.use_gate:
-                f1, fln, f2 = n.lin("sap_fuse_linear.net.0.weight"), n.ln("sap_fuse_linear.net.2"), n.lin("sap_fuse_linear.net.3.weight")
-                dZ = n.new(B, H)
-                O.lndot_bwd(c.Yf, B, H, fln.g, fln.b, n.eps, f2.Wm, df, dZ, fln.dg, fln.db, f2.dW, f2.db)
-                O.linear_dw(dZ, c.glob.out, f1.dW, f1.db, B, N=H, K=H, ldb=K * H, ldc=2 * H)
-                O.linear_dw(dZ, c.loc.out, f1.dW[:, H:], None, B, N=H, K=H, ldb=Vp * H, ldc=2 * H)
-                with _lib.group():
-                    O.linear_dx(dZ, f1.W, B, out=c.d_gmap, residual=c.d_gmap, ldb=2 * H, ldc=K * H, N=H, K=H)
-                    O.linear_dx(dZ, f1.W[:, H:], B, out=c.d_vp, residual=c.d_vp, ldb=2 * H, ldc=Vp * H, N=H, K=H)
+            if getattr(c, "sap_head", False) and O.SAP_HEAD_BWD_FUSED and O.part_ok(H):
+                heads = self._sap_heads(grads=True)
+                dZg, dZl, dZf = n.new(B * K, H), n.new(B * Vp, H), (n.new(B, H) if c.use_gate else None)
+                O.sap_head_bwd(heads, n.eps, (c.Yg, c.Yl, c.Yf), (dZg, dZl, dZf), c.d_gmap, c.d_vp, B, K, Vp, c.g_raw, c.l_raw, c.fuse_raw,
+                               plan["gmask"], plan["lmask"], plan["fsrc"], plan["bwmask"], c.use_gate, c.dgl, c.dll, c.dfl)
+                g1, l1_ = n.lin("global_sap_head.net.0.weight"), n.lin("local_sap_head.net.0.weight")
+                O.linear_dw(dZg, c.glob.out, g1.dW, g1.db, B * K)
+                O.linear_dw(dZl, c.loc.out, l1_.dW, l1_.db, B * Vp)
+                if c.use_gate:
+                    f1 = n.lin("sap_fuse_linear.net.0.weight")
+                    O.linear_dw(dZf, c.glob.out, f1.dW, f1.db, B, N=H, K=H, ldb=K * H, ldc=2 * H)
+                    O.linear_dw(dZf, c.loc.out, f1.dW[:, H:], None, B, N=H, K=H, ldb=Vp * H, ldc=2 * H)
+            else:
+                self._sap_heads_bwd_seq(c)
         elif task == "cfp":
             d_outs = c.d_cfp if c.d_cfp is not None else [n.new(B, H) for _ in range(4)]
             txt_o = c.cfp[3]
diff --git a/vln-magic_amd/host/ops.py b/vln-magic_amd/host/ops.py
--- a/vln-magic_amd/host/ops.py
+++ b/vln-magic_amd/host/ops.py
@@ -1210,6 +1210,94 @@
            1 if use_gate else 0, L.P(dgl), L.P(dll), L.P(dfl), L.P(dg_raw), L.P(dl_raw), L.P(dfuse_raw), L.stream())
 
 
+SAP_HEAD_FUSED = not os.environ.get("MAGIC_NO_SAP_HEAD_FUSED")
+SAP_HEAD_BWD_FUSED = os.environ.get("MAGIC_SAP_HEAD_BWD", "0") != "0"
+_SAPH_OK = {}
+
+
+def sap_head_ok(dtype, H, K, Vp):
+    if not (SAP_HEAD_FUSED and SAP_LOSS_FUSED) or dtype not in L.HALF:
+        return False
+    key = (L.dt(dtype), int(H), int(K), int(Vp))
+    if key not in _SAPH_OK:
+        _SAPH_OK[key] = bool(L.load().magic_sap_head_supported(*key))
+    return _SAPH_OK[key]
+
+
+def _sap_head_arrays(heads, use_gate, *extra):
+    import ctypes as C
+    nh = 3 if use_gate else 2
+    Ws, vecs = (C.c_void_p * 3)(), (C.c_void_p * 15)()
+    outs = [(C.c_void_p * 3)() for _ in extra]
+    for h in range(nh):
+        q = heads[h]
+        W = q["W"]
+        _chk(W.stride(1) == 1 and W.stride(0) == W.shape[1] and W.shape[1] == (2 if h == 2 else 1) * W.shape[0], "sap_head weights")
+        Ws[h] = L.P(W)
+        for i, k in enumerate(("b1", "g", "be", "w2", "b2")):
+            _chk(q[k].dtype == torch.float32, "sap_head vectors fp32")
+            vecs[5 * h + i] = L.P(q[k])
+        for o, e in zip(outs, extra):
+            _chk(e[h].dtype == W.dtype and e[h].is_contiguous(), "sap_head row tensors")
+            o[h] = L.P(e[h])
+    return (Ws, vecs, *outs)
+
+
+def sap_head_fwd(gx, lx, heads, eps, Y, B, K, Vp, g_raw, l_raw, fuse_raw, gmask, lmask, fsrc, bwmask, use_gate, gl, ll, fl, glab=None, llab=None,
+                 coef=0.0, rows=None, *, dgl=None, dll=None, dfl=None, ignore_index=-100, t_fused=None, w_rate=0.0, w_out=None, T=1.0, kd_norm=0.0,
+                 kd_coef=0.0, kd_coef_dev=None, kd_rows=None):
+    import ctypes as C
+    H = gx.shape[-1]
+    _chk(gx.dtype == lx.dtype and gx.is_contiguous() and lx.is_contiguous() and gx.numel() == B * K * H and lx.numel() == B * Vp * H, "sap_head_fwd inputs")
+    _chk(g_raw.numel() >= B * K and l_raw.numel() >= B * Vp and fuse_raw.numel() >= B, "sap_head_fwd raw logits")
+    _chk(Y[0].numel() >= B * K * H and Y[1].numel() >= B * Vp * H and (not use_gate or Y[2].numel() >= B * H), "sap_head_fwd Y")
+    if glab is not None:
+        _chk(glab.dtype == torch.int32 and llab.dtype == torch.int32 and rows.dtype == torch.float32 and rows.numel() >= 3 * B, "sap_head_fwd labels int32, rows fp32 [3, B]")
+    _chk(t_fused is None or (t_fused.dtype == torch.float32 and t_fused.is_contiguous() and tuple(t_fused.shape) == (B, K)), "sap_head_fwd teacher logits fp32 [B, K]")
+    Ws, vecs, Ys = _sap_head_arrays(heads, use_gate, Y)
+    P = L.SapLossParams()
+    P.B, P.K, P.Vp, P.use_gate = B, K, Vp, 1 if use_gate else 0
+    for k, v in (("g_raw", g_raw), ("l_raw", l_raw), ("fuse_raw", fuse_raw), ("gmask", gmask), ("lmask", lmask), ("fsrc", fsrc), ("bwmask", bwmask),
+                 ("gl", gl), ("ll", ll), ("fl", fl), ("glab", glab), ("llab", llab), ("rows", rows), ("dgl", dgl), ("dll", dll), ("dfl", dfl),
+                 ("t_fused", t_fused), ("w_out", w_out), ("kd_coef_dev", kd_coef_dev), ("kd_rows", kd_rows)):
+        setattr(P, k, L.P(v))
+    P.ignore_index, P.coef, P.w_rate, P.T, P.kd_norm, P.kd_coef = int(ignore_index), float(coef), float(w_rate), float(T), float(kd_norm), float(kd_coef)
+    _count(B * K, H, H)
+    _count(B * Vp, H, H)
+    if use_gate:
+        _count(B, H, H)
+        _count(B, H, H)
+    L.call("magic_sap_head_fwd", L.dt(gx.dtype), H, L.P(gx), L.P(lx), C.addressof(Ws), C.addressof(vecs), float(eps), C.addressof(Ys),
+           C.addressof(P), C.sizeof(P), L.stream())
+
+
+def sap_head_bwd(heads, eps, Y, dZ, d_gmap, d_vp, B, K, Vp, g_raw, l_raw, fuse_raw, gmask, lmask, fsrc, bwmask, use_gate, dgl, dll, dfl):
+    import ctypes as C
+    H = d_gmap.shape[-1]
+    _chk(part_ok(H), "sap_head_bwd needs the partial-row parameter gradients (deferred weight-gradient scope)")
+    _chk(d_gmap.is_contiguous() and d_vp.is_contiguous() and d_gmap.numel() == B * K * H and d_vp.numel() == B * Vp * H, "sap_head_bwd d_gmap / d_vp")
+    _chk(dZ[0].numel() >= B * K * H and dZ[1].numel() >= B * Vp * H and (not use_gate or dZ[2].numel() >= B * H), "sap_head_bwd dZ")
+    Ws, vecs, Ys, dZs = _sap_head_arrays(heads, use_gate, Y, dZ)
+    nblk = int(L.load().magic_sap_head_bwd_blocks(int(B)))
+    _chk(nblk > 0, "magic_sap_head_bwd_blocks")
+    stride = 3 * H + 1
+    nh = 3 if use_gate else 2
+    part = _part_rows(nh * nblk, stride, d_gmap.device)
+    flat = part.view(-1)
+    for h in range(nh):
+        q = heads[h]
+        for off, length, dst in ((0, H, q["dg"]), (H, H, q["dbe"]), (2 * H, H, q["dw2"]), (3 * H, 1, q["db2"])):
+            PART_JOBS.append((flat[h * nblk * stride + off:], dst.reshape(-1), nblk, length, stride))
+    _count(B * K, H, H)
+    _count(B * Vp, H, H)
+    if use_gate:
+        _count(B, H, H)
+        _count(B, H, H)
+    L.call("magic_sap_head_bwd", L.dt(d_gmap.dtype), H, B, K, Vp, 1 if use_gate else 0, L.P(g_raw), L.P(l_raw), L.P(fuse_raw), L.P(gmask), L.P(lmask),
+           L.P(fsrc), L.P(bwmask), L.P(dgl), L.P(dll), L.P(dfl), C.addressof(Ys), C.addressof(Ws), C.addressof(vecs), float(eps), C.addressof(dZs),
+           L.P(d_gmap), L.P(d_vp), L.P(part), L.stream())
+
+
 def step_rng(base_seed, counter, rw_temp, seed_out=None, rw_out=None, zero_me=None, scale_state=None, growth=2.0, backoff=0.5, interval=2000):
     L.call("magic_step_rng", int(base_seed) & 0xFFFFFFFFFFFFFFFF, L.P(counter), float(rw_temp), L.P(seed_out), L.P(rw_out), L.P(zero_me),
            L.P(scale_state), float(growth), float(backoff), int(interval), L.stream())
```
